# shanjiayao/PTT

Hardware: AMD Instinct MI355X
Metric: tracklet frames/sec (hot path: PointNet++ SA stack + Point-Track-Transformer blocks) (higher is better)
Workload: dtype f32

## Files before the change

include/ptt_hip.h:

```cpp
#ifndef PTT_HIP_H
#define PTT_HIP_H

#include <stddef.h>
#include <stdint.h>

#ifdef __cplusplus
extern "C" {
#endif

#define PTT_ABI_VERSION 30

enum {
    PTT_OK = 0,
    PTT_EINVAL = -1,
    PTT_EUNSUPPORTED = -2,
    PTT_ELAUNCH = -3,
    PTT_EWORKSPACE = -4
};

typedef void* ptt_stream_t;

int ptt_version(void);
const char* ptt_error_name(int code);
const char* ptt_last_error_string(void);

int ptt_fps_f32(const float* xyz, int B, int N, int npoint, int32_t* idx_out,
                ptt_stream_t stream);
int ptt_fps_ws_f32(const float* xyz, int B, int N, int npoint, int32_t* idx_out, float* workspace,
                   size_t workspace_elems, ptt_stream_t stream);

int ptt_ffps_f32(const float* xyz, const float* feat, int64_t feat_sb, int64_t feat_sc, int64_t feat_sn,
                 int B, int N, int C, int npoint, int32_t* idx_out, ptt_stream_t stream);

int ptt_gather_f32(const float* feat, const int32_t* idx, int B, int C, int N, int M,
                   float* out, ptt_stream_t stream);
int ptt_gather_grad_f32(const float* grad_out, const int32_t* idx, int B, int C, int N,
                        int M, float* grad_feat, ptt_stream_t stream);

int ptt_select_centres_f32(const float* xyz, const int32_t* idx, int B, int N, int M, float* new_xyz,
                           int64_t* idx64_out, ptt_stream_t stream);

int ptt_ball_query_f32(const float* new_xyz, const float* xyz, int B, int M, int N,
                       float radius, int nsample, int32_t* idx_out, ptt_stream_t stream);

int ptt_centres_ball_query_f32(const float* xyz, const int32_t* sel, int B, int N, int M, float radius, int nsample,
                               float* new_xyz, int64_t* idx64_out, int32_t* idx_out, ptt_stream_t stream);

int ptt_group_f32(const float* feat, const int32_t* idx, int B, int C, int N, int M,
                  int ns, float* out, ptt_stream_t stream);
int ptt_group_grad_f32(const float* grad_out, const int32_t* idx, int B, int C, int N,
                       int M, int ns, float* grad_feat, ptt_stream_t stream);

size_t ptt_scatter_add_det_workspace(int B, int N, int E);
int ptt_scatter_add_det_f32(const float* src, const int32_t* idx, int B, int C, int N, int E, float* out,
                            void* workspace, size_t workspace_bytes, ptt_stream_t stream);

int ptt_knn_f32(const float* xyz, int B, int N, int k, int32_t* idx_out,
                ptt_stream_t stream);
int ptt_knn_rel_f32(const float* xyz, int B, int N, int k, int32_t* idx_out, float* rel_out,
                    ptt_stream_t stream);

size_t ptt_packed_weight_elems(int Cout, int K);
int ptt_pack_weight_f32(const float* W, int Cout, int K, float* packed,
                        ptt_stream_t stream);
int ptt_pack_weight_rot_f32(const float* W, int Cout, int K, int rot, float* packed,
                            ptt_stream_t stream);

int ptt_linear_f32(const float* X, int rows, int K, int ldx, const float* Wpacked, int Cout,
                   const float* scale, const float* shift, int relu, const float* residual,
                   int ldr, float* out, int ldo, ptt_stream_t stream);

#define PTT_SA_MAX_LAYERS 4

typedef struct ptt_sa_layer {
    const float* Wpacked;
    const float* scale;
    const float* shift;
    int Cin;
    int Cout;
    int relu;
} ptt_sa_layer;

int ptt_rows_mlp_f32(const float* X, int rows, int K, int ldx, const ptt_sa_layer* layers, int n_layers,
                     const float* residual, int ldr, float* out, int ldo, ptt_stream_t stream);

size_t ptt_ball_query_grid_workspace(int B, int N);
int ptt_ball_query_grid_f32(const float* new_xyz, const float* xyz, int B, int M, int N, float radius, int nsample,
                            int32_t* idx_out, void* workspace, size_t workspace_bytes, ptt_stream_t stream);
int ptt_centres_ball_query_grid_f32(const float* xyz, const int32_t* sel, int B, int N, int M, float radius, int nsample,
                                    float* new_xyz, int64_t* idx64_out, int32_t* idx_out, void* workspace, size_t workspace_bytes,
                                    ptt_stream_t stream);
int ptt_fps_ball_knn_f32(const float* xyz, int B, int N, int M, float radius, int nsample, int k, int32_t* inds,
                         int64_t* inds64, float* new_xyz, int32_t* idx, int32_t* knn, float* rel, ptt_stream_t stream);
#define PTT_POINT_JOBS_MAX 4
typedef struct ptt_point_job {
    const float* xyz; const int32_t* centre_sel; const int32_t* point_sel;
    float* new_xyz; int64_t* idx64_out; int32_t* idx_out; float* rel_out;
    int32_t kind, sel_ld, B, Nraw, Npts, M, nsample;
    float radius;
} ptt_point_job;
int ptt_point_jobs_f32(const ptt_point_job* jobs, int n_jobs, ptt_stream_t stream);

#define PTT_ROW_JOBS_MAX 4
typedef struct ptt_row_job {
    const float* X; const float* X2;
    const float* Xmax;
    const float* Wpacked; const float* scale; const float* shift;
    const float* res; const float* res2;
    float* out; float* out2; float* raw;
    const float* rel; const float* w1;
    const float* qkv; const int32_t* knn; const float* pos;
    int32_t rows, K, K1, ldx, ldx2, Cout;
    int32_t act, res_split, ldr, ldr2, out_split, out_col0, ldo, ldo2, ldraw;
    int32_t prologue, epilogue, ldq, q_off, k_off, v_off, ldp, N;
    float sm_scale;
    int32_t col_tiles;
    const int32_t* idx; const float* xyz; const float* centres; const float* wx;
    float radius;
    int32_t ns, M, normalize_xyz, pro_relu;
} ptt_row_job;
int ptt_row_jobs_f32(const ptt_row_job* jobs, int n_jobs, ptt_stream_t stream);

typedef struct ptt_sa_desc {
    const float* xyz;
    const float* new_xyz;
    const int32_t* idx;
    const float* feat;
    int64_t feat_sb, feat_sc, feat_sn;
    float* out;
    int64_t out_sb, out_sc, out_sm;
    int B, N, M, nsample, C;
    float radius;
    int use_xyz;
    int normalize_xyz;
    int n_layers;
    ptt_sa_layer layers[PTT_SA_MAX_LAYERS];
    const float* l0_point_term;
    const float* l0_xyz_weight;
    int l0_channels;
    int l0_relu;
    void* compact_ws;
    size_t compact_ws_bytes;
} ptt_sa_desc;

int ptt_sa_fused_fwd_f32(const ptt_sa_desc* d, ptt_stream_t stream);
size_t ptt_sa_compact_workspace(int B, int M);

typedef struct ptt_xcorr_desc {
    const float* cos_t;
    const float* P;
    const float* w_sim;
    const float* scale0;
    const float* shift0;
    float* out;
    int64_t out_sb, out_sc, out_sn;
    float* sim_out;
    int B, Ns, Nt, C0;
    int n_layers;
    ptt_sa_layer layers[PTT_SA_MAX_LAYERS];
    int32_t split; int64_t out_sh;
    const float* search_feat; const float* templ_feat;
    int64_t s_sb, s_sn, t_sb, t_sn;
    int C; float eps;
} ptt_xcorr_desc;

int ptt_xcorr_fused_fwd_f32(const ptt_xcorr_desc* d, ptt_stream_t stream);

int ptt_cosine_map_f32(const float* search_feat, int64_t s_sb, int64_t s_sn, int64_t s_sc, const float* templ_feat,
                       int64_t t_sb, int64_t t_sn, int64_t t_sc, int B, int Ns, int Nt, int C, float eps,
                       float* cos_t, ptt_stream_t stream);

typedef struct ptt_attn_desc {
    const float* xyz;
    const float* rel;
    const int32_t* knn;
    const float* qkv;
    const float* Wd1p;
    const float* Wd2p;
    const float* bd2;
    const float* Wg1p;
    const float* bg1;
    const float* Wg2p;
    const float* bg2;
    float* res;
    float* attn;
    int B, N, k, D;
    const int32_t* order;
    int heads;
} ptt_attn_desc;

int ptt_pt_attn_pair_f32(const ptt_attn_desc* d, ptt_stream_t stream);
int ptt_spatial_order_f32(const float* xyz, int B, int N, int32_t* order, ptt_stream_t stream);

typedef struct ptt_crop_job {
    const float* points;
    int64_t ld;
    double lo1[3], hi1[3];
    double trans[3];
    double rot[9];
    double lo2[3], hi2[3];
    float* out;
    int32_t* count;
    int32_t n_points;
    int32_t capacity;
    uint8_t* label_out;
    double ltrans[3];
    double lrot[9];
    double llo[3], lhi[3];
    int32_t append;
    int32_t reserved;
} ptt_crop_job;

int ptt_crop_compact_f32(const ptt_crop_job* jobs_device, int n_jobs, ptt_stream_t stream);
#define PTT_CROP_JOBS_BY_VALUE_MAX 8
int ptt_crop_compact_host_f32(const ptt_crop_job* jobs_host, int n_jobs, ptt_stream_t stream);

#define PTT_SCAN_CROP_CHUNK 1024
size_t ptt_crop_scan_workspace(int n_jobs, int max_points);
int ptt_crop_scan_f32(const ptt_crop_job* jobs_device, int n_jobs, int max_points, void* ws, size_t ws_bytes, ptt_stream_t stream);

#define PTT_MAX_SEGMENTS 4
typedef struct ptt_regularize_job {
    const float* seg[PTT_MAX_SEGMENTS];
    const int32_t* seg_count[PTT_MAX_SEGMENTS];
    int32_t seg_capacity[PTT_MAX_SEGMENTS];
    float* out;
    int32_t* info;
    int32_t n_seg;
    int32_t input_size;
} ptt_regularize_job;

int ptt_regularize_f32(const ptt_regularize_job* jobs_device, int n_jobs, const uint32_t* draws, int n_draws,
                       ptt_stream_t stream);
int ptt_crop_regularize_f32(const ptt_crop_job* crop_jobs, const ptt_regularize_job* reg_jobs_device, int n_jobs,
                            const uint32_t* draws, int n_draws, ptt_stream_t stream);

int ptt_mt19937_fill(uint32_t seed, uint32_t* out_host, int n);

typedef struct ptt_track_box {
    double center[3];
    double wlh[3];
    double quat[4];
} ptt_track_box;

int ptt_track_crop_bounds(const ptt_track_box* boxes, int n, double offset, double scale, const double* extra2,
                          ptt_crop_job* jobs_host, int job_stride);
int ptt_track_box_by_offset(ptt_track_box* boxes, int n, float* offsets, int offset_stride, int use_z,
                            const int32_t* active, int64_t* rng_pos);
int ptt_track_select_update(const float* proposals_host, int P, const int32_t* info_host, ptt_track_box* boxes, int n, int use_z,
                            const int32_t* active, int64_t* rng_pos, float* est_out);

int ptt_select_box_f32(const float* pred_box_data, int B, int P, float* out, int32_t* idx_out, ptt_stream_t stream);

#define PTT_REF_CAMERA 0
#define PTT_REF_LIDAR 1
int ptt_box_overlap_f64(const double* gt, const double* pred, int n, int ref_coord, int dims, double* overlap, double* accuracy,
                        ptt_stream_t stream);

#define PTT_TRAIN_MAX_CANDS 1024
typedef struct ptt_train_cand {
    const float* search;
    const uint8_t* label;
    const float* first;
    const float* prev;
    const int32_t* counts;
    float reg[4];
    uint32_t index;
    uint32_t epoch;
    int32_t capacity;
    int32_t reserved;
} ptt_train_cand;

typedef struct ptt_train_batch_desc {
    float* search_points;
    float* template_points;
    float* cls_label;
    float* reg_label;
    int32_t* src_out;
    int32_t* idx_search_out;
    int32_t* idx_template_out;
    int32_t* info;
    int64_t* totals;
    int32_t B, n_cand;
    int32_t search_size, template_size;
    int32_t min_points;
    uint32_t seed_lo, seed_hi;
    int32_t reserved;
} ptt_train_batch_desc;

int ptt_train_batch_f32(const ptt_train_cand* cands_device, const ptt_train_batch_desc* desc_host, ptt_stream_t stream);
int ptt_philox4x32_10(const uint32_t* counter4, const uint32_t* key2, uint32_t* out4);

size_t ptt_bn_stats_workspace(int R, int C);
int ptt_bn_stats_f32(const float* X, int R, int C, int ldx, float eps, float* mean, float* var, float* invstd,
                     void* workspace, size_t workspace_bytes, ptt_stream_t stream);
int ptt_bn_apply_f32(const float* Z, int ldz, const float* mean, const float* invstd, const float* gamma,
                     const float* beta, int R, int C, int relu, float* X, int ldx, ptt_stream_t stream);
int ptt_bn_bwd_f32(const float* G, int ldg, const float* Act, int lda, const float* Z, int ldz, const float* mean,
                   const float* invstd, const float* gamma, int R, int C, int relu, float* dZ, int ldd,
                   float* dgamma, float* dbeta, void* workspace, size_t workspace_bytes, const float* act_scale,
                   const float* act_shift, ptt_stream_t stream);
int ptt_bn_sums_f64(const float* X, int R, int C, int ldx, double* sums, void* workspace, size_t workspace_bytes,
                    ptt_stream_t stream);
int ptt_bn_finish_f64(const double* sums, int C, float eps, float* mean, float* var, float* invstd,
                      ptt_stream_t stream);
int ptt_bn_bwd_sums_f64(const float* G, int ldg, const float* Act, int lda, const float* Z, int ldz, const float* mean,
                        const float* invstd, int R, int C, double* sums, void* workspace, size_t workspace_bytes,
                        const float* act_scale, const float* act_shift, ptt_stream_t stream);
int ptt_bn_bwd_apply_f32(const float* G, int ldg, const float* Act, int lda, const float* Z, int ldz, const float* mean,
                         const float* invstd, const float* gamma, const float* sum_dy, const float* sum_dy_xhat,
                         const double* count, int R, int C, float* dZ, int ldd, const float* act_scale, const float* act_shift,
                         ptt_stream_t stream);
int ptt_pool_rows_f32(const float* X, int ldx, int G, int ns, int C, float* out, int ldo, int32_t* arg,
                      const float* act_scale, const float* act_shift, ptt_stream_t stream);
int ptt_pool_rows_bwd_f32(const float* dOut, int ldo, const int32_t* arg, int G, int ns, int C, float* dX, int ldx,
                          ptt_stream_t stream);
int ptt_pt_pair_input_f32(const float* q, const float* kf, const int32_t* knn, const float* pos, int B, int N, int k, int D,
                          float* t, ptt_stream_t stream);
int ptt_pt_attn_train_fwd_f32(const float* a, const float* vf, const int32_t* knn, const float* pos, int B, int N, int k, int D,
                              float scale, float* attn, float* res, ptt_stream_t stream);
int ptt_pt_attn_train_bwd_f32(const float* attn, const float* vf, const int32_t* knn, const float* pos, const float* dres, int B,
                              int N, int k, int D, float scale, float* da, float* dvp, ptt_stream_t stream);

int ptt_pt_pair_input_ld_f32(const float* q, int ldq, const float* kf, int ldk, const int32_t* knn, const float* pos, int B, int N,
                             int k, int D, float* t, ptt_stream_t stream);
int ptt_pt_attn_fwd_ld_f32(const float* a, const float* vf, int ldv, const int32_t* knn, const float* pos, int B, int N, int k, int D,
                           float scale, float* attn, float* res, ptt_stream_t stream);

int ptt_gather_rows_f32(const float* src, const int32_t* idx, int B, int N, int E, int C, float* out, ptt_stream_t stream);
int ptt_scatter_csr_i32(const int32_t* idx, int B, int N, int E, int32_t* order, int32_t* start, ptt_stream_t stream);
int ptt_scatter_rows_csr_f32(const float* g, const int32_t* order, const int32_t* start, int B, int N, int E, int C,
                             float* out, ptt_stream_t stream);
int ptt_rows_gemm_pool_supported(int rows, int K, int N, int ldx, int ns);
int ptt_rows_gemm_pool_f32(const float* X, int rows, int K, int ldx, const float* in_scale, const float* in_shift,
                           const float* Wpacked, int N, float* out, int ldo, double* stats, size_t stats_elems, int ns,
                           float* pmax, float* pmin, int32_t* amax, int32_t* amin, ptt_stream_t stream);
int ptt_pool_select_f32(const float* pmax, const float* pmin, const int32_t* amax, const int32_t* amin, const float* act_scale,
                        const float* act_shift, int G, int C, float* out, int32_t* arg, ptt_stream_t stream);
size_t ptt_colsum_workspace(int R, int C);
int ptt_colsum_f32(const float* X, int R, int C, int ldx, float* out, void* workspace, size_t workspace_bytes, ptt_stream_t stream);
size_t ptt_linear_wgrad_workspace(int R, int Cout, int Cin);
int ptt_linear_wgrad_f32(const float* dZ, int ldz, const float* X, int ldx, int R, int Cout, int Cin, float* dW,
                         int accumulate, void* workspace, size_t workspace_bytes, const float* x_scale, const float* x_shift,
                         ptt_stream_t stream);
int ptt_linear_act_in_f32(const float* X, int rows, int K, int ldx, const float* in_scale, const float* in_shift,
                          const float* Wpacked, int Cout, float* out, int ldo, ptt_stream_t stream);

int ptt_pack_weight_strided_f32(const float* W, int Cout, int K, int64_t stride_out, int64_t stride_k, int batch,
                                int64_t stride_batch, float* packed, ptt_stream_t stream);
int ptt_linear_batched_f32(const float* X, int rows, int K, int ldx, int64_t x_batch_stride, const float* Wpacked,
                           int64_t w_batch_stride, int Cout, const float* scale, const float* shift, int relu,
                           const float* residual, int ldr, int64_t r_batch_stride, float* out, int ldo,
                           int64_t o_batch_stride, int batch, ptt_stream_t stream);
int ptt_softmax_rows_f32(float* X, int64_t rows, int n, int ld, float scale, ptt_stream_t stream);
int ptt_layernorm_f32(const float* x, int rows, int C, int ldx, const float* weight, const float* bias, float eps,
                      const float* residual, int ldr, float* out, int ldo, ptt_stream_t stream);

int ptt_rows_gemm_supported(int rows, int K, int N, int ldx, int ldo);
int ptt_rows_gemm_stat_chunks(int rows, int K, int N);
int ptt_rows_gemm_f32(const float* X, int rows, int K, int ldx, const float* in_scale, const float* in_shift,
                      const float* Wpacked, int N, const float* bias, int relu, const float* residual, int ldr,
                      float* out, int ldo, double* stats, size_t stats_elems, ptt_stream_t stream);
int ptt_rows_gemm_masked_f32(const float* X, int rows, int K, int ldx, const float* Wpacked, int N, const float* mask, int ldm,
                             float* out, int ldo, double* stats, size_t stats_elems, ptt_stream_t stream);
int ptt_rows_gemm_bnbwd_f32(const float* X, int rows, int K, int ldx, const float* Wpacked, int N, const float* Z, int ldz,
                            const float* mean, const float* invstd, const float* act_scale, const float* act_shift, float* out,
                            int ldo, double* sums_partial, size_t partial_elems, ptt_stream_t stream);
int ptt_bn_bwd_from_partials_f32(const double* partial, int chunks, const float* G, int ldg, const float* Z, int ldz, const float* mean,
                                 const float* invstd, const float* gamma, int R, int C, float* dZ, int ldd, float* dgamma, float* dbeta,
                                 const float* act_scale, const float* act_shift, ptt_stream_t stream);
int ptt_bn_bwd_sums_partials_f64(const double* partial, int chunks, int C, double* sums, ptt_stream_t stream);
typedef struct ptt_bn_bwd_input {
    const float* g; int ldg;
    const int32_t* arg; int ns;
    const float* z; int ldz;
    const float* k1; const float* c0; const float* c1; const float* mean;
    const float* act_a; const float* act_b;
    float* dz_out; int ldd;
} ptt_bn_bwd_input;
int ptt_bn_bwd_consts_f32(const double* partial, int chunks, const float* mean, const float* invstd, const float* gamma, int R, int C,
                          float* dgamma, float* dbeta, float* k1, float* c0, float* c1, ptt_stream_t stream);
int ptt_bn_bwd_pooled_consts_f32(const float* dPooled, int ldp, const int32_t* arg, int ns, const float* Z, int ldz, const float* mean,
                                 const float* invstd, const float* gamma, int R, int C, float* dgamma, float* dbeta, float* k1,
                                 float* c0, float* c1, void* workspace, size_t workspace_bytes, const float* act_scale,
                                 const float* act_shift, ptt_stream_t stream);
int ptt_rows_gemm_bnbwd_fused_supported(int rows, int K, int N, int ns);
int ptt_rows_gemm_bnbwd_fused_f32(const ptt_bn_bwd_input* in, int rows, int K, const float* Wpacked, int N, const float* Z, int ldz,
                                  const float* mean, const float* invstd, const float* act_scale, const float* act_shift, float* out,
                                  int ldo, double* sums_partial, size_t partial_elems, ptt_stream_t stream);
int ptt_bn_finish_partials_f32(const double* partial, int chunks, int C, int R, float eps, float* mean, float* var, float* invstd,
                               ptt_stream_t stream);
int ptt_bn_sums_partials_f64(const double* partial, int chunks, int C, int R, double* sums, ptt_stream_t stream);
int ptt_bn_bwd_pooled_f32(const float* dPooled, int ldp, const int32_t* arg, int ns, const float* Z, int ldz, const float* mean,
                          const float* invstd, const float* gamma, int R, int C, float* dZ, int ldd, float* dgamma, float* dbeta,
                          void* workspace, size_t workspace_bytes, const float* act_scale, const float* act_shift, ptt_stream_t stream);
int ptt_bn_bwd_pooled_sums_f64(const float* dPooled, int ldp, const int32_t* arg, int ns, const float* Z, int ldz, const float* mean,
                               const float* invstd, int R, int C, double* sums, void* workspace, size_t workspace_bytes,
                               const float* act_scale, const float* act_shift, ptt_stream_t stream);
int ptt_bn_bwd_pooled_apply_f32(const float* dPooled, int ldp, const int32_t* arg, int ns, const float* Z, int ldz, const float* mean,
                                const float* invstd, const float* gamma, const float* sum_dy, const float* sum_dy_xhat,
                                const double* count, int R, int C, float* dZ, int ldd, const float* act_scale,
                                const float* act_shift, ptt_stream_t stream);
int ptt_bn_update_running_f32(const float* mean, const float* var, const double* count, float momentum, int C, float* running_mean,
                              float* running_var, int64_t* num_batches_tracked, ptt_stream_t stream);
int ptt_xcorr_z0_f32(const float* P, const float* cos_t, const float* w_sim, int B, int n2, int n1, int C, float* z0, ptt_stream_t stream);
int ptt_xcorr_z0_stat_chunks(int B, int n2, int n1, int C);
int ptt_xcorr_z0_stats_f32(const float* P, const float* cos_t, const float* w_sim, int B, int n2, int n1, int C, float* z0,
                           double* stats_partial, size_t partial_elems, ptt_stream_t stream);
size_t ptt_xcorr_z0_bwd_workspace(int B, int n1, int C);
int ptt_xcorr_z0_bnbwd_f32(const double* partial, int chunks, const float* G, const float* P, const float* cos_t, const float* w_sim,
                           const float* mean, const float* invstd, const float* gamma, const float* act_scale, const float* act_shift,
                           int B, int n2, int n1, int C, float* dP, float* dcos, float* dw, float* dgamma, float* dbeta, void* workspace,
                           size_t workspace_bytes, ptt_stream_t stream);
int ptt_xcorr_z0_bwd_f32(const float* dz0, const float* cos_t, const float* w_sim, int B, int n2, int n1, int C, float* dP, float* dcos,
                         float* dw, void* workspace, size_t workspace_bytes, ptt_stream_t stream);
int ptt_sa_z0_rows_f32(const float* xyz, const float* new_xyz, const int32_t* idx, const float* term, const float* wx, int ldw, int B,
                       int N, int M, int ns, int C, float radius, int normalize_xyz, float* z0, float* rel_rows, ptt_stream_t stream);
int ptt_sa_z0_rows_stat_chunks(int B, int M, int ns, int C);
int ptt_sa_z0_rows_stats_f32(const float* xyz, const float* new_xyz, const int32_t* idx, const float* term, const float* wx, int ldw, int B,
                             int N, int M, int ns, int C, float radius, int normalize_xyz, float* z0, float* rel_rows,
                             double* stats_partial, size_t partial_elems, ptt_stream_t stream);
typedef struct ptt_bn_train_tail {
    const float* gamma; const float* beta;
    float* act_a; float* act_b;
    float* running_mean; float* running_var;
    int64_t* num_batches_tracked;
    float momentum;
} ptt_bn_train_tail;
int ptt_bn_stats_train_f32(const float* X, int R, int C, int ldx, float eps, float* mean, float* var, float* invstd,
                           void* workspace, size_t workspace_bytes, const ptt_bn_train_tail* tail, ptt_stream_t stream);
int ptt_bn_finish_partials_train_f32(const double* partial, int chunks, int C, int R, float eps, float* mean, float* var,
                                     float* invstd, const ptt_bn_train_tail* tail, ptt_stream_t stream);
typedef struct ptt_pack_job {
    const float* W;
    int64_t out_offset, stride_out, stride_k;
    int32_t Cout, K;
} ptt_pack_job;
int ptt_pack_weights_f32(const ptt_pack_job* jobs_device, int n_jobs, float* arena, ptt_stream_t stream);
size_t ptt_linear_wgrad2_workspace(int R, int Cout, int Cin);
int ptt_linear_wgrad2_f32(const float* dZ, int ldz, const float* X, int ldx, int R, int Cout, int Cin, float* dW,
                          int accumulate, void* workspace, size_t workspace_bytes, const float* x_scale, const float* x_shift,
                          ptt_stream_t stream);

typedef struct ptt_track_loss_desc {
    const float* seed_cls;
// ... 81 lines not shown
```

ptt_amd/_lib.py:

```python
import ctypes
import os
import re
from ctypes import Structure, c_char_p, c_double, c_float, c_int, c_int32, c_int64, c_longlong, c_size_t, c_uint32, c_void_p

from .build import HEADER as HEADER_PATH, LIB as LIB_PATH


def _strip_comments(text):
    return re.sub(r"/\*.*?\*/|//[^\n]*", " ", text, flags=re.S)


def parse_defines(text):
    return {n: int(v) for n, v in re.findall(r"^[ \t]*#[ \t]*define[ \t]+(PTT_\w+)[ \t]+(-?\d+)[ \t]*$", _strip_comments(text), re.M)}


CTYPES = {"int": c_int, "int32_t": c_int32, "uint32_t": c_uint32, "int64_t": c_int64, "long long": c_longlong, "size_t": c_size_t,
          "float": c_float, "double": c_double, "ptt_stream_t": c_void_p}


def _ctype(decl, name, is_return=False):
    words = decl.replace("*", " * ").split()
    if not is_return and len(words) > 1 and words[-1] != "*":
        words.pop()
    if "*" in words:
        if not is_return:
            return c_void_p
        if words == ["const", "char", "*"]:
            return c_char_p
    base = " ".join(w for w in words if w != "const")
    if base not in CTYPES:
        raise RuntimeError("ptt_amd: %s of %s in include/ptt_hip.h has the type '%s', which ptt_amd/_lib.py does not map to ctypes"
                           % ("the return value" if is_return else "parameter '%s'" % decl.strip(), name, base))
    return CTYPES[base]


def parse_prototypes(text):
    text = re.sub(r"^[ \t]*#.*$", " ", _strip_comments(text), flags=re.M).replace('extern "C" {', " ")
    text = re.sub(r"\{[^{}]*\}", " ", text)
    protos = {}
    for stmt in text.split(";"):
        stmt = " ".join(stmt.split()).lstrip("} ")
        if not stmt or stmt.split()[0] in ("typedef", "enum", "struct"):
            continue
        m = re.fullmatch(r"(.+?)\b(\w+) ?\((.*)\)", stmt)
        if m is None:
            raise RuntimeError("ptt_amd: cannot read '%s' in include/ptt_hip.h as a function prototype" % stmt)
        ret, name, params = m.groups()
        params = [] if params.strip() == "void" else params.split(",")
        protos[name] = (_ctype(ret, name, is_return=True), [_ctype(p, name) for p in params])
    return protos


def _read_header():
    if not os.path.exists(HEADER_PATH):
        raise RuntimeError("ptt_amd: %s is missing — the Python binding takes every prototype and constant of the C ABI from it" % HEADER_PATH)
    with open(HEADER_PATH) as fh:
        return fh.read()


_header = _read_header()
PROTOTYPES = parse_prototypes(_header)
EXPORTS = list(PROTOTYPES)
DEFINES = parse_defines(_header)
ABI_VERSION = DEFINES["PTT_ABI_VERSION"]
PTT_SA_MAX_LAYERS = DEFINES["PTT_SA_MAX_LAYERS"]
PTT_MAX_SEGMENTS = DEFINES["PTT_MAX_SEGMENTS"]
PTT_CROP_JOBS_BY_VALUE_MAX = DEFINES["PTT_CROP_JOBS_BY_VALUE_MAX"]
PTT_TRAIN_MAX_CANDS = DEFINES["PTT_TRAIN_MAX_CANDS"]


class CropJob(Structure):
    _fields_ = [("points", c_void_p), ("ld", c_int64),
                ("lo1", c_double * 3), ("hi1", c_double * 3), ("trans", c_double * 3), ("rot", c_double * 9),
                ("lo2", c_double * 3), ("hi2", c_double * 3),
                ("out", c_void_p), ("count", c_void_p), ("n_points", c_int32), ("capacity", c_int32),
                ("label_out", c_void_p), ("ltrans", c_double * 3), ("lrot", c_double * 9), ("llo", c_double * 3), ("lhi", c_double * 3),
                ("append", c_int32), ("reserved", c_int32)]


class RegularizeJob(Structure):
    _fields_ = [("seg", c_void_p * PTT_MAX_SEGMENTS), ("seg_count", c_void_p * PTT_MAX_SEGMENTS),
                ("seg_capacity", c_int32 * PTT_MAX_SEGMENTS), ("out", c_void_p), ("info", c_void_p),
                ("n_seg", c_int32), ("input_size", c_int32)]


class TrackBox(Structure):
    _fields_ = [("center", c_double * 3), ("wlh", c_double * 3), ("quat", c_double * 4)]


class TrainCand(Structure):
    _fields_ = [("search", c_void_p), ("label", c_void_p), ("first", c_void_p), ("prev", c_void_p), ("counts", c_void_p),
                ("reg", c_float * 4), ("index", c_uint32), ("epoch", c_uint32), ("capacity", c_int32), ("reserved", c_int32)]


class TrainBatchDesc(Structure):
    _fields_ = [("search_points", c_void_p), ("template_points", c_void_p), ("cls_label", c_void_p), ("reg_label", c_void_p),
                ("src_out", c_void_p), ("idx_search_out", c_void_p), ("idx_template_out", c_void_p), ("info", c_void_p), ("totals", c_void_p),
                ("B", c_int32), ("n_cand", c_int32), ("search_size", c_int32), ("template_size", c_int32), ("min_points", c_int32),
                ("seed_lo", c_uint32), ("seed_hi", c_uint32), ("reserved", c_int32)]


class BnTrainTail(Structure):
    _fields_ = [("gamma", c_void_p), ("beta", c_void_p), ("act_a", c_void_p), ("act_b", c_void_p),
                ("running_mean", c_void_p), ("running_var", c_void_p), ("num_batches_tracked", c_void_p), ("momentum", c_float)]


class BnBwdInput(Structure):
    _fields_ = [("g", c_void_p), ("ldg", c_int), ("arg", c_void_p), ("ns", c_int), ("z", c_void_p), ("ldz", c_int),
                ("k1", c_void_p), ("c0", c_void_p), ("c1", c_void_p), ("mean", c_void_p), ("act_a", c_void_p), ("act_b", c_void_p),
                ("dz_out", c_void_p), ("ldd", c_int)]


class PackJob(Structure):
    _fields_ = [("W", c_void_p), ("out_offset", c_int64), ("stride_out", c_int64), ("stride_k", c_int64),
                ("Cout", c_int32), ("K", c_int32)]


class RowJob(Structure):
    _fields_ = [("X", c_void_p), ("X2", c_void_p), ("Xmax", c_void_p), ("Wpacked", c_void_p), ("scale", c_void_p), ("shift", c_void_p),
                ("res", c_void_p), ("res2", c_void_p), ("out", c_void_p), ("out2", c_void_p), ("raw", c_void_p),
                ("rel", c_void_p), ("w1", c_void_p), ("qkv", c_void_p), ("knn", c_void_p), ("pos", c_void_p),
                ("rows", c_int32), ("K", c_int32), ("K1", c_int32), ("ldx", c_int32), ("ldx2", c_int32), ("Cout", c_int32),
                ("act", c_int32), ("res_split", c_int32), ("ldr", c_int32), ("ldr2", c_int32), ("out_split", c_int32),
                ("out_col0", c_int32), ("ldo", c_int32), ("ldo2", c_int32), ("ldraw", c_int32),
                ("prologue", c_int32), ("epilogue", c_int32), ("ldq", c_int32), ("q_off", c_int32), ("k_off", c_int32),
                ("v_off", c_int32), ("ldp", c_int32), ("N", c_int32), ("sm_scale", c_float), ("col_tiles", c_int32),
                ("idx", c_void_p), ("xyz", c_void_p), ("centres", c_void_p), ("wx", c_void_p), ("radius", c_float),
                ("ns", c_int32), ("M", c_int32), ("normalize_xyz", c_int32), ("pro_relu", c_int32)]


class PointJob(Structure):
    _fields_ = [("xyz", c_void_p), ("centre_sel", c_void_p), ("point_sel", c_void_p), ("new_xyz", c_void_p), ("idx64_out", c_void_p),
                ("idx_out", c_void_p), ("rel_out", c_void_p), ("kind", c_int32), ("sel_ld", c_int32), ("B", c_int32),
                ("Nraw", c_int32), ("Npts", c_int32), ("M", c_int32), ("nsample", c_int32), ("radius", c_float)]


class TrackLossDesc(Structure):
    _fields_ = [("seed_cls", c_void_p), ("cls_label", c_void_p), ("search_inds", c_void_p), ("votes", c_void_p), ("reg_label", c_void_p),
                ("box_data", c_void_p), ("centres", c_void_p), ("pos_weight_seed", c_void_p), ("pos_weight_box", c_void_p),
                ("B", c_int32), ("N", c_int32), ("Ns", c_int32), ("M", c_int32), ("ld_reg", c_int32),
                ("w_seed_cls", c_float), ("w_seed_reg", c_float), ("w_box_cls", c_float), ("w_box_reg", c_float)]


class AdamTensor(Structure):
    _fields_ = [("param", c_void_p), ("grad", c_void_p), ("exp_avg", c_void_p), ("exp_avg_sq", c_void_p), ("n", c_int64)]


class GradJob(Structure):
    _fields_ = [("partial", c_void_p), ("nchunks", c_int32), ("reserved", c_int32)]


class GradSegment(Structure):
    _fields_ = [("dst", c_int64), ("n", c_int32), ("cols", c_int32), ("ld", c_int32), ("job0", c_int32), ("njobs", c_int32), ("out", c_int32),
                ("vec", c_int32), ("reserved", c_int32)]


class AdamHyper(Structure):
    _fields_ = [("beta1", c_float), ("beta2", c_float), ("one_minus_beta1", c_float), ("one_minus_beta2", c_float), ("eps", c_float), ("step_size", c_float), ("bias2_sqrt", c_float),
                ("weight_decay", c_float), ("max_norm", c_float), ("write_clipped", c_int32)]


class SaLayer(Structure):
    _fields_ = [("Wpacked", c_void_p), ("scale", c_void_p), ("shift", c_void_p),
                ("Cin", c_int), ("Cout", c_int), ("relu", c_int)]


class SaDesc(Structure):
    _fields_ = [("xyz", c_void_p), ("new_xyz", c_void_p), ("idx", c_void_p), ("feat", c_void_p),
                ("feat_sb", c_int64), ("feat_sc", c_int64), ("feat_sn", c_int64),
                ("out", c_void_p), ("out_sb", c_int64), ("out_sc", c_int64), ("out_sm", c_int64),
                ("B", c_int), ("N", c_int), ("M", c_int), ("nsample", c_int), ("C", c_int),
                ("radius", c_float), ("use_xyz", c_int), ("normalize_xyz", c_int), ("n_layers", c_int),
                ("layers", SaLayer * PTT_SA_MAX_LAYERS),
                ("l0_point_term", c_void_p), ("l0_xyz_weight", c_void_p), ("l0_channels", c_int), ("l0_relu", c_int),
                ("compact_ws", c_void_p), ("compact_ws_bytes", c_size_t)]


class XcorrDesc(Structure):
    _fields_ = [("cos_t", c_void_p), ("P", c_void_p), ("w_sim", c_void_p), ("scale0", c_void_p), ("shift0", c_void_p),
                ("out", c_void_p), ("out_sb", c_int64), ("out_sc", c_int64), ("out_sn", c_int64),
                ("sim_out", c_void_p),
                ("B", c_int), ("Ns", c_int), ("Nt", c_int), ("C0", c_int),
                ("n_layers", c_int), ("layers", SaLayer * PTT_SA_MAX_LAYERS),
                ("split", c_int32), ("out_sh", c_int64), ("search_feat", c_void_p), ("templ_feat", c_void_p),
                ("s_sb", c_int64), ("s_sn", c_int64), ("t_sb", c_int64), ("t_sn", c_int64), ("C", c_int), ("eps", c_float)]


class AttnDesc(Structure):
    _fields_ = [("xyz", c_void_p), ("rel", c_void_p), ("knn", c_void_p), ("qkv", c_void_p),
                ("Wd1p", c_void_p), ("Wd2p", c_void_p), ("bd2", c_void_p),
                ("Wg1p", c_void_p), ("bg1", c_void_p), ("Wg2p", c_void_p), ("bg2", c_void_p),
                ("res", c_void_p), ("attn", c_void_p),
                ("B", c_int), ("N", c_int), ("k", c_int), ("D", c_int), ("order", c_void_p), ("heads", c_int)]


_lib = None


def lib():
    global _lib
    if _lib is None:
        if not os.path.exists(LIB_PATH):
            raise RuntimeError(
                "ptt_amd: %s is missing — build it with `python -m ptt_amd.build` "
                "(hipcc --offload-arch=gfx950); there is no CPU fallback" % LIB_PATH)
        import torch
        try:
            loaded = ctypes.CDLL(LIB_PATH)
        except OSError as e:
            raise RuntimeError("ptt_amd: cannot load %s: %s" % (LIB_PATH, e))
        for name, (restype, argtypes) in PROTOTYPES.items():
            fn = getattr(loaded, name)
            fn.restype, fn.argtypes = restype, argtypes
        if loaded.ptt_version() != ABI_VERSION:
            raise RuntimeError("ptt_amd: %s has ABI version %d, this package expects %d — rebuild it with "
                               "`python -m ptt_amd.build`" % (LIB_PATH, loaded.ptt_version(), ABI_VERSION))
        _lib = loaded
    return _lib


def check(rc, what):
    if rc != 0:
        l = lib()
        raise RuntimeError("%s failed: %s (%s)" % (what, l.ptt_error_name(rc).decode(),
                                                   l.ptt_last_error_string().decode()))
```

ptt_amd/csrc/mfma_ops.hip:

```cpp
#include <math.h>
#include <stdlib.h>
#include <string.h>
#include "common.h"
#include "mfma_common.h"

#ifndef PTT_PAIR_PF
#define PTT_PAIR_PF 1
#endif
#ifndef PTT_GATHER_BATCH
#define PTT_GATHER_BATCH 16
#endif
#ifndef PTT_SA_WAVES
#define PTT_SA_WAVES 2
#endif

namespace ptt {

#ifdef PTT_DEV
#define PTT_STAMP(i) do { if (p.dbg && threadIdx.x == 0 && blockIdx.x < 4096) p.dbg[blockIdx.x * 8 + (i)] = __builtin_readcyclecounter(); } while (0)
#else
#define PTT_STAMP(i) do { } while (0)
#endif

__device__ __forceinline__ void stagger_second_slot(int first_wave_blocks, int quanta) {
// ... 950 lines not shown
        if (it > 0) store_pooled(prev);
        if (!(PTT_SAS_EXP & 1)) lds_barrier();

        {
            const float* arow = Q + (lane & 31) * SAS_LDK + 4 * half;
            f32x4 a0[2], a1[2], bc[2][2], bn[2][2];
#define SAS_A2(A, KB)                                                                           \
            {                                                                                   \
                A[0] = *reinterpret_cast<const f32x4*>(arow + (KB) * 8);                        \
                A[1] = *reinterpret_cast<const f32x4*>(arow + 32 * SAS_LDK + (KB) * 8);         \
            }
#pragma unroll
            for (int k = 0; k < 2; ++k) { bc[k][0] = pre2[k][0]; bc[k][1] = pre2[k][1]; }
            SAS_A2(a0, 0)
            f32x4 mc = *reinterpret_cast<const f32x4*>(meta + (w * 16 + sub) * 4), mn = mc;
#pragma unroll
            for (int i = 0; i < 8; ++i) {
                if (i < 7) {
#pragma unroll
                    for (int k = 0; k < 2; ++k) {
                        bn[k][0] = weight_load(wr2, wvoff, (2 * i + 2 + k) * WK2);
                        bn[k][1] = weight_load(wr2, wvoff, (2 * i + 2 + k) * WK2 + 4 * 1024);
                    }
                } else {
                    pre1[0] = weight_load(wr1, wvoff, 0);
                    pre1[1] = weight_load(wr1, wvoff, WK1);
                }
                SAS_A2(a1, 2 * i + 1)
                f32x4 v = wx0;
                if (!(PTT_SAS_EXP & 2)) v = weight_load(rf, __builtin_bit_cast(int, mc[0]) + q * 16, 0);
                __builtin_amdgcn_sched_barrier(0);
                if (i == 0) {
#pragma unroll
                    for (int u = 0; u < 2; ++u)
#pragma unroll
                        for (int rt = 0; rt < 2; ++rt)
                            acc[rt][u] = __builtin_amdgcn_mfma_f32_32x32x2f32(a0[rt][0], bc[0][u][0], zero16, 0, 0, 0);
#pragma unroll
                    for (int j = 1; j < 4; ++j)
#pragma unroll
                        for (int u = 0; u < 2; ++u)
#pragma unroll
                            for (int rt = 0; rt < 2; ++rt)
                                acc[rt][u] = __builtin_amdgcn_mfma_f32_32x32x2f32(a0[rt][j], bc[0][u][j], acc[rt][u], 0, 0, 0);
                } else {
                    gemm_mfma_block<2, 2, 2>(a0, bc[0], acc);
                }
                __builtin_amdgcn_sched_barrier(0);
                if (i < 7) {
                    SAS_A2(a0, 2 * i + 2)
                    mn = *reinterpret_cast<const f32x4*>(meta + (w * 16 + 2 * (i + 1) + sub) * 4);
                }
                __builtin_amdgcn_sched_barrier(0);
                gemm_mfma_block<2, 2, 2>(a1, bc[1], acc);
                if (!(PTT_SAS_EXP & 2)) sas_pair_store(P, w, i, sub, q, v, mc, wx0, wx1, wx2, floor0);
#if PTT_SAS_INTERLEAVE
#pragma unroll
                for (int k = 0; k < 16; ++k) {
                    __builtin_amdgcn_sched_group_barrier(0x008, 1, 0);
                    __builtin_amdgcn_sched_group_barrier(0x002, 1, 0);
                }
                __builtin_amdgcn_sched_group_barrier(0x200, 1, 0);
#endif
                __builtin_amdgcn_sched_barrier(0);
                mc = mn;
#pragma unroll
                for (int k = 0; k < 2; ++k) { bc[k][0] = bn[k][0]; bc[k][1] = bn[k][1]; }
            }
#undef SAS_A2
        }
        prev = first;
        if (more) { first.advance(2, M); own = own_next; }
    }
#pragma unroll
    for (int i = 0; i < 4; ++i) pv[i >> 1][i & 1] = sas_pool(acc[i >> 1][i & 1], (i & 1) ? sh2b : sh2a, L2.relu);
    store_pooled(prev);
}

struct XcorrParams {
    const float* P; const float* wsim; const float* scale0; const float* shift0;
    float* sim_out;
    const float* cos_t;
    int C0, Nt;
    SaParams sa;
    const float* sfeat; const float* tfeat; long long s_sb, s_sn, t_sb, t_sn; int C; float eps;
    long long out_sh;
};

struct CosParams {
    const float* sfeat; const float* tfeat; float* cos_t;
    long long s_sb, s_sn, s_sc, t_sb, t_sn, t_sc;
    int B, Ns, Nt, C;
    float eps;
};
__global__ __launch_bounds__(256) void cos_map_kernel(CosParams q) {
    const int lane = threadIdx.x & 63;
    const int j = blockIdx.x * 4 + (threadIdx.x >> 6);
    if (j >= q.B * q.Ns) return;
    const int b = j / q.Ns, jj = j - b * q.Ns;
    const float* s = q.sfeat + (long long)b * q.s_sb + (long long)jj * q.s_sn;
    for (int i0 = 0; i0 < q.Nt; i0 += 64) {
        const int i = i0 + lane;
        const float* a = q.tfeat + (long long)b * q.t_sb + (long long)(i < q.Nt ? i : q.Nt - 1) * q.t_sn;
        float dot = 0.f, na = 0.f, ns = 0.f;
        if (q.t_sc == 1 && q.s_sc == 1 && (q.C & 3) == 0 && ((q.t_sn | q.t_sb | q.s_sn | q.s_sb) & 3) == 0 &&
            ((reinterpret_cast<uintptr_t>(q.tfeat) | reinterpret_cast<uintptr_t>(q.sfeat)) & 15) == 0) {
            for (int c = 0; c < q.C; c += 4) {
                const f32x4 av = *reinterpret_cast<const f32x4*>(a + c), sv = *reinterpret_cast<const f32x4*>(s + c);
#pragma unroll
                for (int k = 0; k < 4; ++k) { dot += av[k] * sv[k]; na += av[k] * av[k]; ns += sv[k] * sv[k]; }
            }
        } else {
            for (int c = 0; c < q.C; ++c) {
                const float av = a[(long long)c * q.t_sc], sv = s[(long long)c * q.s_sc];
                dot += av * sv; na += av * av; ns += sv * sv;
            }
        }
        if (i < q.Nt) q.cos_t[((long long)b * q.Ns + jj) * q.Nt + i] = dot / (fmaxf(sqrtf(na), q.eps) * fmaxf(sqrtf(ns), q.eps));
    }
}

template <int RT, bool SPLIT>
__global__ __launch_bounds__(256, 2) void xcorr_fused_kernel(XcorrParams q) {
    constexpr int ROWS = 32 * RT;
    extern __shared__ __attribute__((aligned(16))) float smem[];
    const SaParams& p = q.sa;
    float* Xs = smem;
    float* simv = smem + ROWS * p.ldk;
    const int t = threadIdx.x, lane = t & 63, w = t >> 6, half = lane >> 5;
    const int npts = p.B * p.M;
    const int j = SPLIT ? (int)blockIdx.x % npts : logical_block();
    const int hsel = SPLIT ? (int)blockIdx.x / npts : 0;
    const int b = j / p.M, jj = j - b * p.M;
    stagger_second_slot(p.first_wave, p.stagger);
    SaPre pre;
    pre.w[0] = pre.w[1] = f32x4{0.f, 0.f, 0.f, 0.f};
    float run[2] = {-__builtin_inff(), -__builtin_inff()};
    const int nlast = p.n_layers - 1;
    const SaLayerDev& LL = p.L[nlast];

    const int ibeg = SPLIT ? hsel * (q.Nt >> 1) : 0, iend = SPLIT ? ibeg + (q.Nt >> 1) : q.Nt;
    for (int i0 = ibeg; i0 < iend; i0 += ROWS) {
        prefetch_first_block(p.L[0].Wp, p.L[0].scale, p.L[0].shift, p.L[0].NT, w, lane, pre);
        if (i0 != ibeg) __syncthreads();
        if constexpr (SPLIT) {
            const int i = t >> 3, sub = t & 7;
            const float* a = q.tfeat + (long long)b * q.t_sb + (long long)(i0 + i) * q.t_sn;
            const float* sv_ = q.sfeat + (long long)b * q.s_sb + (long long)jj * q.s_sn;
            float dot = 0.f, na = 0.f, ns = 0.f;
            for (int c = sub * 4; c < q.C; c += 32) {
                const f32x4 av = *reinterpret_cast<const f32x4*>(a + c), sv = *reinterpret_cast<const f32x4*>(sv_ + c);
#pragma unroll
                for (int k = 0; k < 4; ++k) { dot += av[k] * sv[k]; na += av[k] * av[k]; ns += sv[k] * sv[k]; }
            }
#pragma unroll
            for (int m = 1; m < 8; m <<= 1) { dot += __shfl_xor(dot, m, 64); na += __shfl_xor(na, m, 64); ns += __shfl_xor(ns, m, 64); }
            if (sub == 0) simv[i] = dot / (fmaxf(sqrtf(na), q.eps) * fmaxf(sqrtf(ns), q.eps));
        } else {
            if (t < ROWS) {
                const float cs = q.cos_t[(unsigned)((b * p.M + jj) * q.Nt + i0 + t)];
                simv[t] = cs;
                if (q.sim_out) q.sim_out[(unsigned)((b * q.Nt + i0 + t) * p.M + jj)] = cs;
            }
        }
        __syncthreads();

        const int nq = q.C0 >> 2;
        if (!q.scale0 && !q.shift0 && (q.C0 & 3) == 0 && (256 % nq) == 0) {
            typedef float f32x2 __attribute__((ext_vector_type(2)));
            const int c4 = t % nq, step = 256 / nq;
            const f32x4 w4 = *reinterpret_cast<const f32x4*>(q.wsim + c4 * 4);
            const float* prow = q.P + ((size_t)(b * q.Nt + i0) * q.C0 + c4 * 4);
            for (int i = t / nq; i < ROWS; i += step) {
                const f32x4 pv = *reinterpret_cast<const f32x4*>(prow + (unsigned)(i * q.C0));
                const float cs = simv[i];
                const f32x2 c2 = {cs, cs};
                f32x2 lo = __builtin_elementwise_fma(f32x2{w4[0], w4[1]}, c2, f32x2{pv[0], pv[1]});
                f32x2 hi = __builtin_elementwise_fma(f32x2{w4[2], w4[3]}, c2, f32x2{pv[2], pv[3]});
                *reinterpret_cast<f32x4*>(Xs + i * p.ldk + c4 * 4) =
                    f32x4{fmaxf(lo[0], 0.f), fmaxf(lo[1], 0.f), fmaxf(hi[0], 0.f), fmaxf(hi[1], 0.f)};
            }
        } else {
            for (int c = t; c < q.C0; c += 256) {
                const float wsim = q.wsim[c], sc = q.scale0 ? q.scale0[c] : 1.f, sh = q.shift0 ? q.shift0[c] : 0.f;
                const float* pr = q.P + ((long long)b * q.Nt + i0) * q.C0 + c;
#pragma unroll 8
                for (int i = 0; i < ROWS; ++i) {
                    const float v = (pr[(long long)i * q.C0] + wsim * simv[i]) * sc + sh;
                    Xs[i * p.ldk + c] = fmaxf(v, 0.f);
                }
            }
        }
        __syncthreads();

        for (int l = 0; l < nlast; ++l) {
            const SaLayerDev& L = p.L[l];
            const int ctw = (L.NT + 3) >> 2;
            if (ctw <= 1) sa_layer<32 * RT, 1, RT>(p, L, false, Xs, lane, w, j, 1, pre, &p.L[l + 1]);
            else sa_layer<32 * RT, 2, RT>(p, L, false, Xs, lane, w, j, 1, pre, &p.L[l + 1]);
        }
        {
            const bool affine = LL.scale != nullptr;
            f32x16 acc[RT][2];
#pragma unroll
            for (int rt = 0; rt < RT; ++rt)
#pragma unroll
                for (int u = 0; u < 2; ++u)
#pragma unroll
                    for (int r = 0; r < 16; ++r) acc[rt][u][r] = pre.sh[u];
            int nvalid = 0;
#pragma unroll
            for (int u = 0; u < 2; ++u)
                if (w + 4 * u < LL.NT) nvalid = u + 1;
            gemm_tiles<RT, 2, 0>(Xs, p.ldk, LL.nkb, reinterpret_cast<const f32x4*>(LL.Wp), LL.NT, w, nvalid, lane, acc, pre.w);
#pragma unroll
            for (int u = 0; u < 2; ++u) {
                if (u >= nvalid) break;
                const int col = (w + 4 * u) * 32 + (lane & 31);
                float sc = 1.f, sh = 0.f;
                if (affine) { sc = LL.scale[col]; sh = LL.shift ? LL.shift[col] : 0.f; }
#pragma unroll
                for (int rt = 0; rt < RT; ++rt) {
                    float m = affine ? acc[rt][u][0] * sc + sh : acc[rt][u][0];
#pragma unroll
                    for (int r = 1; r < 16; ++r) m = fmaxf(m, affine ? acc[rt][u][r] * sc + sh : acc[rt][u][r]);
                    run[u] = fmaxf(run[u], max_halves(m));
                }
            }
        }
    }
    if (half == 0) {
#pragma unroll
        for (int u = 0; u < 2; ++u) {
            if (w + 4 * u >= LL.NT) break;
            const int col = (w + 4 * u) * 32 + (lane & 31);
            p.out[(SPLIT ? hsel * q.out_sh : 0) + b * p.osb + col * p.osc + jj * p.osm] = LL.relu ? fmaxf(run[u], 0.f) : run[u];
        }
    }
}

template <int NS, int CT, bool AFFINE, int RT>
__device__ __forceinline__ void sa_wave_layer(const SaParams& p, const SaLayerDev& L, bool last, float* Xw, int lane,
                                              int centre0, int ncentres) {
    f32x16 acc[RT][CT];
#pragma unroll
    for (int u = 0; u < CT; ++u) {
        const float s0 = (!AFFINE && L.shift) ? L.shift[u * 32 + (lane & 31)] : 0.f;
#pragma unroll
        for (int rt = 0; rt < RT; ++rt)
#pragma unroll
            for (int r = 0; r < 16; ++r) acc[rt][u][r] = s0;
    }
    gemm_core<RT, CT, CT, 1>(Xw, p.ldk, L.nkb, reinterpret_cast<const f32x4*>(L.Wp), L.NT, 0, lane, acc);
    __builtin_amdgcn_wave_barrier();
    const int half = lane >> 5;
#pragma unroll
    for (int u = 0; u < CT; ++u) {
        const int col = u * 32 + (lane & 31);
        float sc = 1.f, sv = 0.f;
        if constexpr (AFFINE) { sc = L.scale[col]; sv = L.shift ? L.shift[col] : 0.f; }
#pragma unroll
        for (int rt = 0; rt < RT; ++rt) {
            float y[16];
#pragma unroll
            for (int r = 0; r < 16; ++r) y[r] = AFFINE ? acc[rt][u][r] * sc + sv : acc[rt][u][r];
            if (!last) {
#pragma unroll
                for (int r = 0; r < 16; ++r)
                    Xw[(rt * 32 + tile_row(r, half)) * p.ldk + col] = L.relu ? fmaxf(y[r], 0.f) : y[r];
            } else if (NS == 32) {
                float m = y[0];
#pragma unroll
                for (int r = 1; r < 16; ++r) m = fmaxf(m, y[r]);
                m = max_halves(m);
                if (L.relu) m = fmaxf(m, 0.f);
                if (half == 0 && rt < ncentres) {
                    const int c = centre0 + rt; const int b = c / p.M, mm = c - b * p.M;
                    p.out[b * p.osb + col * p.osc + mm * p.osm] = m;
                }
            } else {
                float m0 = y[0], m1 = y[8];
#pragma unroll
                for (int r = 1; r < 8; ++r) { m0 = fmaxf(m0, y[r]); m1 = fmaxf(m1, y[8 + r]); }
                m0 = max_halves(m0);
                m1 = max_halves(m1);
                if (L.relu) { m0 = fmaxf(m0, 0.f); m1 = fmaxf(m1, 0.f); }
                if (half == 0) {
                    if (2 * rt < ncentres) {
                        const int c = centre0 + 2 * rt; const int b = c / p.M, mm = c - b * p.M;
                        p.out[b * p.osb + col * p.osc + mm * p.osm] = m0;
                    }
                    if (2 * rt + 1 < ncentres) {
                        const int c = centre0 + 2 * rt + 1; const int b = c / p.M, mm = c - b * p.M;
                        p.out[b * p.osb + col * p.osc + mm * p.osm] = m1;
                    }
                }
            }
        }
    }
    __builtin_amdgcn_wave_barrier();
}

constexpr int SAC_HDR = 16;
struct SacTable {
    int32_t* ws; int T;
    __host__ __device__ int32_t* ndist() const { return ws + SAC_HDR; }
    __host__ __device__ int32_t* list(int k) const { return ws + SAC_HDR + (size_t)(1 + k) * T; }
    __host__ __device__ int32_t* rows(int k) const { return ws + SAC_HDR + 5 * (size_t)T + (size_t)((4 << k) - 4) * T; }
    static size_t words(size_t T) { return SAC_HDR + 65 * T; }
};
constexpr int SAC_PASSES = 4;

__global__ __launch_bounds__(64) void sa_compact_zero_kernel(int32_t* ws) {
    if (threadIdx.x < 4) ws[threadIdx.x] = 0;
}

template <bool XYZ>
__global__ __launch_bounds__(256) void sa_compact_kernel(const float* __restrict__ xyz, const int32_t* __restrict__ idx, int N, int M,
                                                         SacTable tab) {
    __shared__ int s_cnt[4], s_base[4], s_cls[32], s_pos[32], s_nd[32];
    __shared__ int s_row[32][32];
    const int t = threadIdx.x, lane = t & 63, half = lane >> 5, s = lane & 31, w = t >> 6;
    const int g0 = blockIdx.x * 32, T = tab.T;
    if (t < 4) s_cnt[t] = 0;
    __syncthreads();
    int iv[SAC_PASSES];
    uint32_t x[SAC_PASSES], y[SAC_PASSES], z[SAC_PASSES];
#pragma unroll
    for (int q = 0; q < SAC_PASSES; ++q) iv[q] = idx[(size_t)min(g0 + q * 8 + w * 2 + half, T - 1) * 32 + s];
    if constexpr (XYZ) {
#pragma unroll
        for (int q = 0; q < SAC_PASSES; ++q) {
            const int b = min(g0 + q * 8 + w * 2 + half, T - 1) / M;
            const uint32_t* pt = reinterpret_cast<const uint32_t*>(xyz) + ((size_t)b * N + iv[q]) * 3;
            x[q] = pt[0]; y[q] = pt[1]; z[q] = pt[2];
        }
    }
#pragma unroll
    for (int q = 0; q < SAC_PASSES; ++q) {
        const int lc = q * 8 + w * 2 + half;
        const int i0a = __builtin_amdgcn_readlane(iv[q], 0), i0b = __builtin_amdgcn_readlane(iv[q], 32);
        const int i0 = half ? i0b : i0a;
        const bool real = s == 0 || iv[q] != i0;
        int dup = 0;
        if constexpr (XYZ) {
            const unsigned long long rm = __ballot(real);
            const int J = 31 - __builtin_clz((uint32_t)rm | (uint32_t)(rm >> 32));
            for (int j = 0; j < J; ++j) {
                const uint32_t xa = __builtin_amdgcn_readlane(x[q], j), xb = __builtin_amdgcn_readlane(x[q], 32 + j);
                const uint32_t ya = __builtin_amdgcn_readlane(y[q], j), yb = __builtin_amdgcn_readlane(y[q], 32 + j);
                const uint32_t za = __builtin_amdgcn_readlane(z[q], j), zb = __builtin_amdgcn_readlane(z[q], 32 + j);
                dup |= (int)(j < s) & (int)(x[q] == (half ? xb : xa)) & (int)(y[q] == (half ? yb : ya)) & (int)(z[q] == (half ? zb : za));
            }
        }
        const bool keep = real && !dup;
        const unsigned long long km = __ballot(keep);
        const uint32_t m = half ? (uint32_t)(km >> 32) : (uint32_t)km;
        const int nd = __popc(m);
        if (keep) s_row[lc][__popc(m & ((1u << s) - 1u))] = iv[q];
        if (s == 0) {
            const int k = nd <= 4 ? 0 : nd <= 8 ? 1 : nd <= 16 ? 2 : 3;
            const bool valid = g0 + lc < T;
            s_cls[lc] = valid ? k : -1;
            s_nd[lc] = nd;
            s_pos[lc] = valid ? atomicAdd(&s_cnt[k], 1) : 0;
            if (valid) tab.ndist()[g0 + lc] = nd;
        }
    }
    __syncthreads();
    if (t < 4) s_base[t] = s_cnt[t] ? atomicAdd(&tab.ws[t], s_cnt[t]) : 0;
    __syncthreads();
    for (int e = t; e < 32 * 32; e += 256) {
        const int lc = e >> 5, j = e & 31, k = s_cls[lc];
        if (k < 0 || j >= (4 << k)) continue;
        const int q = s_base[k] + s_pos[lc];
        tab.rows(k)[(size_t)q * (4 << k) + j] = s_row[lc][j < s_nd[lc] ? j : 0];
        if (j == 0) tab.list(k)[q] = g0 + lc;
    }
}

#ifndef PTT_SAL_WGS
#define PTT_SAL_WGS 1
#endif
#ifndef PTT_SAL_WAVES
#define PTT_SAL_WAVES 12
#endif

template <int ROWS>
struct SacTileT {
    static constexpr int LG = ROWS == 32 ? 3 : 4;
    static_assert(ROWS == 32 || ROWS == 64, "32- or 64-row tiles");
    int k, first, n;
    __device__ __forceinline__ static void count(const int32_t* ws, int total, int (&cnt)[4], int (&tiles)[4]) {
#pragma unroll
        for (int k = 0; k < 4; ++k) {
            cnt[k] = min(max(ws[k], 0), total);
            tiles[k] = (k ? tiles[k - 1] : 0) + ((cnt[k] + ((1 << LG) >> k) - 1) >> (LG - k));
        }
    }
    __device__ __forceinline__ void at(int j, const int (&tiles)[4], const int (&cnt)[4]) {
        k = j < tiles[0] ? 0 : j < tiles[1] ? 1 : j < tiles[2] ? 2 : 3;
        const int j0 = k == 0 ? 0 : k == 1 ? tiles[0] : k == 2 ? tiles[1] : tiles[2];
        const int nk = k == 0 ? cnt[0] : k == 1 ? cnt[1] : k == 2 ? cnt[2] : cnt[3];
        first = (j - j0) << (LG - k);
        n = min((1 << LG) >> k, nk - first);
    }
    __device__ __forceinline__ void row(const SacTable& tab, int s, int& n_out, int& ball) const {
        const int cl = s >> (2 + k), inb = cl < n;
        n_out = tab.rows(k)[(size_t)first * (4 << k) + (inb ? s : (s & ((4 << k) - 1)))];
        ball = tab.list(k)[first + (inb ? cl : 0)];
    }
};
using SacTile = SacTileT<32>;

template <int NU>
__device__ __forceinline__ void sac_store(int k, int n, int ball, int M, const f32x16 (&acc)[NU], const float (&sh)[NU],
                                          float* const (&o)[NU], int relu, int half, int osb, int osm) {
    int ob[8];
#pragma unroll
    for (int g = 0; g < 8; ++g) {
        if (g >= (8 >> k)) break;
        const int id = __builtin_amdgcn_readlane(ball, g << (2 + k)), b = id / M;
        ob[g] = b * osb + (id - b * M) * osm;
    }
#pragma unroll
    for (int u = 0; u < NU; ++u) {
        const f32x16& a = acc[u];
        if (k == 3) {
            const float mx = sas_pool(a, sh[u], relu);
            if (half == 0) o[u][ob[0]] = mx;
        } else if (k == 2) {
            float m0 = a[0], m1 = a[8];
#pragma unroll
            for (int r = 1; r < 8; ++r) { m0 = fmaxf(m0, a[r]); m1 = fmaxf(m1, a[8 + r]); }
            m0 = max_halves(m0) + sh[u]; m1 = max_halves(m1) + sh[u];
            if (relu) { m0 = fmaxf(m0, 0.f); m1 = fmaxf(m1, 0.f); }
            if (half < n) o[u][half ? ob[1] : ob[0]] = half ? m1 : m0;
        } else {
            float m[4];
#pragma unroll
            for (int q = 0; q < 4; ++q) m[q] = fmaxf(fmaxf(a[4 * q], a[4 * q + 1]), fmaxf(a[4 * q + 2], a[4 * q + 3]));
            if (k == 1) {
#pragma unroll
                for (int q = 0; q < 4; ++q) m[q] = max_halves(m[q]) + sh[u];
#pragma unroll
                for (int i = 0; i < 2; ++i) {
                    const int g = 2 * half + i;
                    float v = half ? m[2 + i] : m[i];
                    if (relu) v = fmaxf(v, 0.f);
                    if (g < n) o[u][half ? ob[2 + i] : ob[i]] = v;
                }
            } else {
#pragma unroll
                for (int q = 0; q < 4; ++q) {
                    const int g = 2 * q + half;
                    float v = m[q] + sh[u];
                    if (relu) v = fmaxf(v, 0.f);
                    if (g < n) o[u][half ? ob[2 * q + 1] : ob[2 * q]] = v;
                }
            }
        }
    }
}

template <bool COMPACT>
__global__ __launch_bounds__(64 * PTT_SAL_WAVES) __attribute__((amdgpu_waves_per_eu(PTT_SAL_WAVES * PTT_SAL_WGS / 4)))
void sa_lds_kernel(SaParams p) {
    extern __shared__ __attribute__((aligned(16))) float smem[];
    float* W1 = smem;
    float* W2 = smem + 4096;
    const int t = threadIdx.x, lane = t & 63, half = lane >> 5, col = lane & 31;
    const int w = __builtin_amdgcn_readfirstlane(t >> 6);
    const int total = p.B * p.M, M = p.M, N = p.N;
    const int nw = (int)blockDim.x >> 6;
    SacTable tab{p.cws, total};
    int cnt[4], tiles[4];
    if constexpr (COMPACT) {
        SacTile::count(p.cws, total, cnt, tiles);
        if (logical_block() >= tiles[3]) return;
    }
    {
        const f32x4* g1 = reinterpret_cast<const f32x4*>(p.L[1].Wp);
        const f32x4* g2 = reinterpret_cast<const f32x4*>(p.L[2].Wp);
        f32x4* s1 = reinterpret_cast<f32x4*>(W1);
        f32x4* s2 = reinterpret_cast<f32x4*>(W2);
        const int nthr = (int)blockDim.x;
        for (int i = t; i < 1024; i += nthr) s1[i] = g1[i];
        for (int i = t; i < 2048; i += nthr) s2[i] = g2[i];
    }
    float* cst = smem + 4096 + 8192 + w * 640 + lane;
#pragma unroll
    for (int u = 0; u < 2; ++u) {
        const f32x4 f = reinterpret_cast<const f32x4*>(p.L[0].Wp)[u * 64 + col];
        const float s0 = p.L[0].shift ? p.L[0].shift[u * 32 + col] : 0.f;
        cst[(0 + u) * 64] = half ? f[1] : f[0];
        cst[(2 + u) * 64] = half ? s0 : f[2];
        cst[(4 + u) * 64] = p.L[1].shift ? p.L[1].shift[u * 32 + col] : 0.f;
    }
#pragma unroll
    for (int u = 0; u < 4; ++u) cst[(6 + u) * 64] = p.L[2].shift ? p.L[2].shift[u * 32 + col] : 0.f;
    const float one_zero = half ? 0.f : 1.f, one_hi = 1.f;
    __syncthreads();
    int c0, c1, cstep;
    if constexpr (COMPACT) {
        c0 = logical_block() + (int)gridDim.x * w; c1 = tiles[3]; cstep = (int)gridDim.x * nw;
    } else {
        const int gw = logical_block() * nw + w;
        c0 = gw * p.chunk; c1 = min(total, c0 + p.chunk); cstep = 1;
    }
    if (c0 >= c1) return;
    const float rdiv = p.normalize ? p.radius : 1.0f;
    const int osb = (int)p.osb, osm = (int)p.osm, osc = (int)p.osc;
    const f32x16 zero16 = {0.f, 0.f, 0.f, 0.f, 0.f, 0.f, 0.f, 0.f, 0.f, 0.f, 0.f, 0.f, 0.f, 0.f, 0.f, 0.f};
    const float* a1p = W1 + lane * 4;
    const float* b2p = W2 + lane * 4;
    const __amdgpu_buffer_rsrc_t rx = weight_rsrc(p.xyz);

    SasCentre ce{0, 0, 0};
    SacTile tc{0, 0, 0};
    float px, py, pz, cx, cy, cz;
    int g_cur = 0;
    if constexpr (COMPACT) {
        tc.at(c0, tiles, cnt);
        int n_cur;
        tc.row(tab, col, n_cur, g_cur);
        const size_t flat = (size_t)(g_cur / M) * N + n_cur;
        px = p.xyz[flat * 3]; py = p.xyz[flat * 3 + 1]; pz = p.xyz[flat * 3 + 2];
        cx = p.new_xyz[(size_t)g_cur * 3]; cy = p.new_xyz[(size_t)g_cur * 3 + 1]; cz = p.new_xyz[(size_t)g_cur * 3 + 2];
    } else {
        ce.c = c0; ce.b = c0 / M; ce.m = c0 - ce.b * M;
        const int n_cur = p.idx[(size_t)c0 * 32 + col];
        const size_t flat = (size_t)ce.b * N + n_cur;
        px = p.xyz[flat * 3]; py = p.xyz[flat * 3 + 1]; pz = p.xyz[flat * 3 + 2];
        cx = p.new_xyz[(size_t)c0 * 3]; cy = p.new_xyz[(size_t)c0 * 3 + 1]; cz = p.new_xyz[(size_t)c0 * 3 + 2];
    }
    for (int c = c0; c < c1; c += cstep) {
        SasCentre nx = ce;
        SacTile tx = tc;
        int n_next, g_next;
        if constexpr (COMPACT) {
            if (c + cstep < c1) tx.at(c + cstep, tiles, cnt);
            tx.row(tab, col, n_next, g_next);
        } else {
            if (c + 1 < c1) nx.advance(1, M);
            n_next = p.idx[(size_t)nx.c * 32 + col];
        }
        f32x4 wa[2], wn[2];
#pragma unroll
        for (int u = 0; u < 2; ++u) wa[u] = *reinterpret_cast<const f32x4*>(a1p + u * 256);
        const float dx = (px - cx) / rdiv, dy = (py - cy) / rdiv, dz = (pz - cz) / rdiv;
        __builtin_amdgcn_sched_barrier(0);
        f32x16 h0[2];
        {
            const float k0 = half ? dy : dx, k1 = half ? one_hi : dz;
#pragma unroll
            for (int u = 0; u < 2; ++u) h0[u] = __builtin_amdgcn_mfma_f32_32x32x2f32(cst[(0 + u) * 64], k0, zero16, 0, 0, 0);
#pragma unroll
            for (int u = 0; u < 2; ++u) h0[u] = __builtin_amdgcn_mfma_f32_32x32x2f32(cst[(2 + u) * 64], k1, h0[u], 0, 0, 0);
#pragma unroll
            for (int u = 0; u < 2; ++u)
#pragma unroll
                for (int r = 0; r < 16; ++r) h0[u][r] = fmaxf(h0[u][r], 0.f);
        }
        f32x16 h1[2];
        f32x4 wb[4], wm[4];
        {
#pragma unroll
            for (int u = 0; u < 2; ++u) h1[u] = __builtin_amdgcn_mfma_f32_32x32x2f32(cst[(4 + u) * 64], one_zero, zero16, 0, 0, 0);
#pragma unroll
            for (int kb = 0; kb < 8; ++kb) {
                if (kb < 7) {
#pragma unroll
                    for (int u = 0; u < 2; ++u) wn[u] = *reinterpret_cast<const f32x4*>(a1p + ((kb + 1) * 2 + u) * 256);
                } else {
#pragma unroll
                    for (int u = 0; u < 4; ++u) wb[u] = *reinterpret_cast<const f32x4*>(b2p + u * 256);
                }
                __builtin_amdgcn_sched_barrier(0);
#pragma unroll
                for (int j = 0; j < 4; ++j)
#pragma unroll
                    for (int u = 0; u < 2; ++u)
                        h1[u] = __builtin_amdgcn_mfma_f32_32x32x2f32(wa[u][j], h0[kb >> 2][(kb & 3) * 4 + j], h1[u], 0, 0, 0);
                __builtin_amdgcn_sched_barrier(0);
#pragma unroll
                for (int u = 0; u < 2; ++u) wa[u] = wn[u];
            }
#pragma unroll
            for (int u = 0; u < 2; ++u)
#pragma unroll
                for (int r = 0; r < 16; ++r) h1[u][r] = fmaxf(h1[u][r], 0.f);
        }
        {
            const int g = COMPACT ? g_next : nx.c;
            const int off = ((COMPACT ? g_next / M : nx.b) * N + n_next) * 12;
            px = __builtin_bit_cast(float, __builtin_amdgcn_raw_buffer_load_b32(rx, off, 0, 0));
            py = __builtin_bit_cast(float, __builtin_amdgcn_raw_buffer_load_b32(rx, off + 4, 0, 0));
            pz = __builtin_bit_cast(float, __builtin_amdgcn_raw_buffer_load_b32(rx, off + 8, 0, 0));
            cx = p.new_xyz[(size_t)g * 3]; cy = p.new_xyz[(size_t)g * 3 + 1]; cz = p.new_xyz[(size_t)g * 3 + 2];
        }
        __builtin_amdgcn_sched_barrier(0);
        {
            f32x16 acc[4];
#pragma unroll
            for (int kb = 0; kb < 8; ++kb) {
                if (kb < 7) {
#pragma unroll
                    for (int u = 0; u < 4; ++u) wm[u] = *reinterpret_cast<const f32x4*>(b2p + ((kb + 1) * 4 + u) * 256);
                }
                __builtin_amdgcn_sched_barrier(0);
#pragma unroll
                for (int j = 0; j < 4; ++j)
#pragma unroll
                    for (int u = 0; u < 4; ++u)
                        acc[u] = __builtin_amdgcn_mfma_f32_32x32x2f32(h1[kb >> 2][(kb & 3) * 4 + j], wb[u][j],
                                                                       (kb == 0 && j == 0) ? zero16 : acc[u], 0, 0, 0);
                __builtin_amdgcn_sched_barrier(0);
#pragma unroll
                for (int u = 0; u < 4; ++u) wb[u] = wm[u];
            }
            if constexpr (COMPACT) {
                const float sh2[4] = {cst[6 * 64], cst[7 * 64], cst[8 * 64], cst[9 * 64]};
                float* const o[4] = {p.out + col * osc, p.out + (32 + col) * osc, p.out + (64 + col) * osc, p.out + (96 + col) * osc};
                sac_store<4>(tc.k, tc.n, g_cur, M, acc, sh2, o, p.L[2].relu, half, osb, osm);
            } else {
                float* o = p.out + (ce.b * osb + ce.m * osm);
#pragma unroll
                for (int u = 0; u < 4; ++u) {
                    const float mx = sas_pool(acc[u], cst[(6 + u) * 64], p.L[2].relu);
                    if (half == 0) o[(u * 32 + col) * osc] = mx;
                }
            }
        }
        if constexpr (COMPACT) { tc = tx; g_cur = g_next; } else ce = nx;
    }
}

__global__ __launch_bounds__(256, 2) void sa_stream_compact_kernel(SaParams p) {
    extern __shared__ __attribute__((aligned(16))) float smem[];
    float* const P = smem;
    float* const Q = smem + SAS_TILE;
    float* const meta = smem + 2 * SAS_TILE;
    int* const sball = reinterpret_cast<int*>(meta + 64 * 4);
    const int t = threadIdx.x, lane = t & 63, half = lane >> 5, sub = half, q = lane & 31, col = q;
    const int w = __builtin_amdgcn_readfirstlane(t >> 6);
    const int total = p.B * p.M, M = p.M, N = p.N;
    const SacTable tab{p.cws, total};
    int cnt[4], tiles[4];
    SacTileT<64>::count(p.cws, total, cnt, tiles);
    if ((int)blockIdx.x >= tiles[3]) return;
    const SaLayerDev& L1 = p.L[0];
    const SaLayerDev& L2 = p.L[1];
    const __amdgpu_buffer_rsrc_t rf = weight_rsrc(p.feat);
    const __amdgpu_buffer_rsrc_t wr1 = weight_rsrc(L1.Wp), wr2 = weight_rsrc(L2.Wp);
    const int wvoff = (w * 64 + lane) * 16;
    constexpr int WK1 = 4 * 1024, WK2 = 8 * 1024;
    const f32x4 wx0 = *reinterpret_cast<const f32x4*>(p.wx + q * 4);
    const f32x4 wx1 = *reinterpret_cast<const f32x4*>(p.wx + 128 + q * 4);
    const f32x4 wx2 = *reinterpret_cast<const f32x4*>(p.wx + 256 + q * 4);
    const float sh1 = L1.shift ? L1.shift[w * 32 + col] : 0.f;
    const float sh2[2] = {L2.shift ? L2.shift[w * 32 + col] : 0.f, L2.shift ? L2.shift[(w + 4) * 32 + col] : 0.f};
    f32x16 sh1v;
#pragma unroll
    for (int r = 0; r < 16; ++r) sh1v[r] = sh1;
    const f32x16 zero16 = {0.f, 0.f, 0.f, 0.f, 0.f, 0.f, 0.f, 0.f, 0.f, 0.f, 0.f, 0.f, 0.f, 0.f, 0.f, 0.f};
    const float floor0 = p.l0_relu ? 0.f : -__builtin_inff();
    const float rdiv = p.normalize ? p.radius : 1.0f;
    const int osb = (int)p.osb, osm = (int)p.osm;
    float* const o[2] = {p.out + (w * 32 + col) * (int)p.osc, p.out + ((w + 4) * 32 + col) * (int)p.osc};

    for (int j = blockIdx.x; j < tiles[3]; j += (int)gridDim.x) {
        SacTileT<64> tc;
        tc.at(j, tiles, cnt);
        if (t < 64) {
            int n, ball;
            tc.row(tab, t, n, ball);
            const int flat = (ball / M) * N + n;
            const float x = p.xyz[(size_t)flat * 3 + 0], y = p.xyz[(size_t)flat * 3 + 1], z = p.xyz[(size_t)flat * 3 + 2];
            const float cx = p.new_xyz[(size_t)ball * 3 + 0], cy = p.new_xyz[(size_t)ball * 3 + 1], cz = p.new_xyz[(size_t)ball * 3 + 2];
            const float dx = (x - cx) / rdiv, dy = (y - cy) / rdiv, dz = (z - cz) / rdiv;
            const int off = flat * (128 * (int)sizeof(float));
            *reinterpret_cast<f32x4*>(meta + t * 4) = f32x4{__builtin_bit_cast(float, off), dx, dy, dz};
            sball[t] = ball;
        }
        __syncthreads();
#pragma unroll
        for (int i = 0; i < 8; ++i) {
            f32x4 m;
            const f32x4 v = sas_pair_load(meta, rf, w, i, sub, q, m);
            sas_pair_store(P, w, i, sub, q, v, m, wx0, wx1, wx2, floor0);
        }
        const int ballr[2] = {sball[col], sball[32 + col]};
        __syncthreads();
        {
            f32x16 acc1[2] = {sh1v, sh1v};
            const float* arow = P + (lane & 31) * SAS_LDK + 4 * half;
#pragma unroll
            for (int kb = 0; kb < 16; ++kb) {
                const f32x4 b = weight_load(wr1, wvoff, kb * WK1);
                const f32x4 a[2] = {*reinterpret_cast<const f32x4*>(arow + kb * 8),
                                    *reinterpret_cast<const f32x4*>(arow + 32 * SAS_LDK + kb * 8)};
#pragma unroll
                for (int jj = 0; jj < 4; ++jj)
#pragma unroll
                    for (int rt = 0; rt < 2; ++rt) acc1[rt] = __builtin_amdgcn_mfma_f32_32x32x2f32(a[rt][jj], b[jj], acc1[rt], 0, 0, 0);
            }
#pragma unroll
            for (int rt = 0; rt < 2; ++rt)
#pragma unroll
                for (int r = 0; r < 16; ++r) Q[(rt * 32 + tile_row(r, half)) * SAS_LDK + w * 32 + col] = fmaxf(acc1[rt][r], 0.f);
        }
        __syncthreads();
        {
            f32x16 acc[2][2] = {{zero16, zero16}, {zero16, zero16}};
            const float* arow = Q + (lane & 31) * SAS_LDK + 4 * half;
#pragma unroll
            for (int kb = 0; kb < 16; ++kb) {
                const f32x4 b[2] = {weight_load(wr2, wvoff, kb * WK2), weight_load(wr2, wvoff, kb * WK2 + 4 * 1024)};
                const f32x4 a[2] = {*reinterpret_cast<const f32x4*>(arow + kb * 8),
                                    *reinterpret_cast<const f32x4*>(arow + 32 * SAS_LDK + kb * 8)};
                gemm_mfma_block<2, 2, 2>(a, b, acc);
            }
#pragma unroll
            for (int rt = 0; rt < 2; ++rt) {
                const int n = tc.n - rt * (8 >> tc.k);
                if (n <= 0) continue;
                sac_store<2>(tc.k, n, ballr[rt], M, acc[rt], sh2, o, L2.relu, half, osb, osm);
            }
        }
    }
}

template <int NS, int RT>
__global__ __launch_bounds__(256, 2) void sa_wave_kernel(SaParams p) {
    extern __shared__ __attribute__((aligned(16))) float smem[];
    constexpr int CPW = 32 * RT / NS;
    const int t = threadIdx.x, lane = t & 63, w = t >> 6;
    float* Xw = smem + w * 32 * RT * p.ldk;
    const int total_centres = p.B * p.M;
    const int centre0 = (logical_block() * 4 + w) * CPW;
    if (centre0 >= total_centres) return;
    const int ncentres = min(CPW, total_centres - centre0);

#pragma unroll
    for (int rt = 0; rt < RT; ++rt) sa_gather_rows<NS, 32>(p, Xw, rt * 32, centre0, lane);
    __builtin_amdgcn_wave_barrier();

    for (int l = 0; l < p.n_layers; ++l) {
        const SaLayerDev& L = p.L[l];
        const bool last = (l == p.n_layers - 1);
#define PTT_WAVE_LAYER(CTV)                                                                         \
        { if (L.scale) sa_wave_layer<NS, CTV, true, RT>(p, L, last, Xw, lane, centre0, ncentres);       \
          else sa_wave_layer<NS, CTV, false, RT>(p, L, last, Xw, lane, centre0, ncentres); }
        if (L.NT == 1) PTT_WAVE_LAYER(1)
        else if (L.NT == 2) PTT_WAVE_LAYER(2)
        else PTT_WAVE_LAYER(4)
#undef PTT_WAVE_LAYER
    }
}

struct AttnParams {
    const float* xyz; const float* rel; const int32_t* knn; const float* qkv; const float* Wd1p;
    const float* Wd2p; const float* bd2; const float* Wg1p; const float* bg1; const float* Wg2p; const float* bg2;
    float* res; float* attn;
    const int32_t* order;
    int BN, N, first_wave, stagger;
    long long* dbg;
};

template <int D, int HEADS>
__device__ __forceinline__ void gemm_heads(const float* Xs, int ldk, const float* Wp, int w, int lane, f32x16 (&acc)[1][4],
                                           const f32x4 (&pre)[4]) {
    static_assert(D == 512 && (HEADS == 2 || HEADS == 4 || HEADS == 8 || HEADS == 16), "4 waves x 4 column tiles of D = 512");
    constexpr int HD = D / HEADS, TPH = HD / 32, NKB = HD / 8;
    constexpr int NA = HEADS == 2 ? 2 : 4;
    constexpr int NB = HEADS == 2 ? 2 : 1;
    const int row = lane & 31, half = lane >> 5;
    const float* arow[NA];
#pragma unroll
    for (int i = 0; i < NA; ++i) arow[i] = Xs + row * ldk + 4 * half + ((w + 4 * i * (4 / NA)) / TPH) * HD;
    const __amdgpu_buffer_rsrc_t wr = weight_rsrc(Wp);
    int wvoff[NB];
#pragma unroll
    for (int i = 0; i < NB; ++i) wvoff[i] = (((w + 4 * i) % TPH) * 64 + lane) * 16;
    constexpr int wkstep = TPH * 1024;
    f32x4 bcur[NB], bnxt[NB];
#pragma unroll
    for (int i = 0; i < NB; ++i) { bcur[i] = pre[i]; bnxt[i] = bcur[i]; }
    auto block = [&](int kb) {
        f32x4 a[NA];
#pragma unroll
        for (int i = 0; i < NA; ++i) a[i] = *reinterpret_cast<const f32x4*>(arow[i] + kb * 8);
#pragma unroll
        for (int j = 0; j < 4; ++j)
#pragma unroll
            for (int u = 0; u < 4; ++u)
                acc[0][u] = __builtin_amdgcn_mfma_f32_32x32x2f32(a[u / (4 / NA)][j], bcur[u % NB][j], acc[0][u], 0, 0, 0);
    };
    for (int kb = 0; kb + 1 < NKB; ++kb) {
#pragma unroll
        for (int i = 0; i < NB; ++i) bnxt[i] = weight_load(wr, wvoff[i], (kb + 1) * wkstep);
        block(kb);
#pragma unroll
        for (int i = 0; i < NB; ++i) bcur[i] = bnxt[i];
    }
    block(NKB - 1);
}

template <int D, int HEADS>
__device__ __forceinline__ void prefetch_first_block_heads(const float* Wp, int w, int lane, f32x4 (&pre)[4]) {
    constexpr int TPH = D / HEADS / 32, NB = HEADS == 2 ? 2 : 1;
    const f32x4* bp = reinterpret_cast<const f32x4*>(Wp) + lane;
#pragma unroll
    for (int i = 0; i < NB; ++i) pre[i] = bp[(size_t)((w + 4 * i) % TPH) * 64];
}

template <int D>
__global__ __launch_bounds__(256, 2) void pt_attn_pair_kernel(AttnParams p) {
    constexpr int HEADS = 1;
#include "pt_attn_pair_body.h"
}

template <int HEADS>
__global__ __launch_bounds__(256, 2) void pt_attn_pair_heads_kernel(AttnParams p) {
    constexpr int D = 512;
#include "pt_attn_pair_body.h"
}

__global__ __launch_bounds__(256) void softmax_rows_kernel(float* __restrict__ X, long long rows, int n, int ld, float scale) {
    const int lane = threadIdx.x & 63;
    const long long r = (long long)blockIdx.x * 4 + (threadIdx.x >> 6);
    if (r >= rows) return;
    float* x = X + r * ld;
    float m = -3.0e38f;
    for (int c = lane; c < n; c += 64) m = fmaxf(m, x[c] * scale);
    m = wave_max_f32(m);
    float sum = 0.f;
    for (int c = lane; c < n; c += 64) {
        const float e = __expf(x[c] * scale - m);
        x[c] = e;
        sum += e;
    }
#pragma unroll
    for (int o = 32; o > 0; o >>= 1) sum += __shfl_xor(sum, o, 64);
    const float inv = 1.0f / sum;
    for (int c = lane; c < n; c += 64) x[c] *= inv;
}

constexpr int LN_VPL = 16;
__global__ __launch_bounds__(256) void layernorm_rows_kernel(const float* __restrict__ X, int rows, int C, int ldx,
                                                             const float* __restrict__ weight, const float* __restrict__ bias,
                                                             float eps, const float* __restrict__ R, int ldr,
                                                             float* __restrict__ Y, int ldy) {
    const int lane = threadIdx.x & 63;
    const int r = blockIdx.x * 4 + (threadIdx.x >> 6);
    if (r >= rows) return;
    const float* x = X + (size_t)r * ldx;
    float v[LN_VPL];
    float sum = 0.f;
#pragma unroll
    for (int i = 0; i < LN_VPL; ++i) {
        const int c = lane + 64 * i;
        v[i] = c < C ? x[c] : 0.f;
        sum += v[i];
    }
#pragma unroll
    for (int o = 32; o > 0; o >>= 1) sum += __shfl_xor(sum, o, 64);
    const float mean = sum / (float)C;
    float sq = 0.f;
#pragma unroll
    for (int i = 0; i < LN_VPL; ++i) {
        const float d = (lane + 64 * i) < C ? v[i] - mean : 0.f;
        v[i] = d;
        sq += d * d;
    }
#pragma unroll
    for (int o = 32; o > 0; o >>= 1) sq += __shfl_xor(sq, o, 64);
    const float rstd = 1.0f / sqrtf(sq / (float)C + eps);
    float* y = Y + (size_t)r * ldy;
    const float* res = R ? R + (size_t)r * ldr : nullptr;
#pragma unroll
    for (int i = 0; i < LN_VPL; ++i) {
        const int c = lane + 64 * i;
        if (c < C) {
            float o = v[i] * rstd;
            if (weight) o *= weight[c];
            if (bias) o += bias[c];
            if (res) o += res[c];
            y[c] = o;
        }
    }
}

}

using namespace ptt;

extern "C" int ptt_layernorm_f32(const float* x, int rows, int C, int ldx, const float* weight, const float* bias, float eps,
                                 const float* residual, int ldr, float* out, int ldo, ptt_stream_t stream) {
    if (rows < 0 || C <= 0 || C > 64 * LN_VPL || ldx < C || ldo < C || (residual && ldr < C))
        return fail(PTT_EINVAL, "ptt_layernorm_f32: rows=%d C=%d ldx=%d ldr=%d ldo=%d (C <= %d)", rows, C, ldx, ldr, ldo, 64 * LN_VPL);
    if (rows == 0) return PTT_OK;
    if (!x || !out) return fail(PTT_EINVAL, "ptt_layernorm_f32: null pointer");
    hipLaunchKernelGGL(layernorm_rows_kernel, dim3((unsigned)((rows + 3) / 4)), dim3(256), 0, as_stream(stream), x, rows, C, ldx,
                       weight, bias, eps, residual, ldr, out, ldo);
    return check_launch("layernorm_rows_kernel");
}

extern "C" int ptt_softmax_rows_f32(float* X, int64_t rows, int n, int ld, float scale, ptt_stream_t stream) {
    if (rows < 0 || n <= 0 || ld < n) return fail(PTT_EINVAL, "ptt_softmax_rows_f32: rows=%lld n=%d ld=%d", (long long)rows, n, ld);
    if (rows == 0) return PTT_OK;
    if (!X) return fail(PTT_EINVAL, "ptt_softmax_rows_f32: null pointer");
    hipLaunchKernelGGL(softmax_rows_kernel, dim3((unsigned)((rows + 3) / 4)), dim3(256), 0, as_stream(stream), X, (long long)rows, n, ld,
                       scale);
    return check_launch("softmax_rows_kernel");
}

extern "C" size_t ptt_packed_weight_elems(int Cout, int K) {
    if (Cout <= 0 || K <= 0) return 0;
    const size_t NT = (size_t)(Cout + 31) / 32, NKB = (size_t)(K + 7) / 8;
    return NT * NKB * 256;
}

extern "C" int ptt_pack_weight_rot_f32(const float* W, int Cout, int K, int rot, float* packed, ptt_stream_t stream) {
    if (Cout <= 0 || K <= 0 || rot < 0 || rot >= K)
        return fail(PTT_EINVAL, "ptt_pack_weight_rot_f32: Cout=%d K=%d rot=%d", Cout, K, rot);
    if (!W || !packed) return fail(PTT_EINVAL, "ptt_pack_weight_rot_f32: null pointer");
    const size_t total = ptt_packed_weight_elems(Cout, K);
    const int NT = (Cout + 31) / 32;
    size_t g = (total + 255) / 256;
    if (g > 4096) g = 4096;
    hipLaunchKernelGGL(pack_weight_kernel, dim3((unsigned)g), dim3(256), 0, as_stream(stream), W, Cout, K, NT, rot, total,
                       packed, (long long)K, 1LL, 0LL);
    return check_launch("pack_weight_kernel");
}

extern "C" int ptt_pack_weight_strided_f32(const float* W, int Cout, int K, int64_t stride_out, int64_t stride_k, int batch,
                                           int64_t stride_batch, float* packed, ptt_stream_t stream) {
    if (Cout <= 0 || K <= 0 || batch < 0) return fail(PTT_EINVAL, "ptt_pack_weight_strided_f32: Cout=%d K=%d batch=%d", Cout, K, batch);
    if (batch == 0) return PTT_OK;
    if (!W || !packed) return fail(PTT_EINVAL, "ptt_pack_weight_strided_f32: null pointer");
    const size_t total = ptt_packed_weight_elems(Cout, K);
    const int NT = (Cout + 31) / 32;
    size_t g = (total + 255) / 256;
    if (g > 1024) g = 1024;
    hipLaunchKernelGGL(pack_weight_kernel, dim3((unsigned)g, (unsigned)batch), dim3(256), 0, as_stream(stream), W, Cout, K, NT, 0,
                       total, packed, (long long)stride_out, (long long)stride_k, (long long)stride_batch);
    return check_launch("pack_weight_kernel");
}

extern "C" int ptt_pack_weights_f32(const ptt_pack_job* jobs_device, int n_jobs, float* arena, ptt_stream_t stream) {
    if (n_jobs < 0) return fail(PTT_EINVAL, "ptt_pack_weights_f32: n_jobs=%d", n_jobs);
    if (n_jobs == 0) return PTT_OK;
    if (!jobs_device || !arena) return fail(PTT_EINVAL, "ptt_pack_weights_f32: null pointer");
    if (n_jobs > 65535) return fail(PTT_EUNSUPPORTED, "ptt_pack_weights_f32: n_jobs=%d exceeds one launch (65535)", n_jobs);
    hipLaunchKernelGGL(pack_weights_kernel, dim3(32, (unsigned)n_jobs), dim3(256), 0, as_stream(stream), jobs_device, arena);
    return check_launch("pack_weights_kernel");
}

extern "C" int ptt_pack_weight_f32(const float* W, int Cout, int K, float* packed, ptt_stream_t stream) {
    return ptt_pack_weight_rot_f32(W, Cout, K, 0, packed, stream);
}

static int linear_launch(const float* X, int rows, int K, int ldx, const float* Wpacked, int Cout, const float* scale,
                         const float* shift, int relu, const float* residual, int ldr, float* out, int ldo, int batch,
                         long long xb, long long wb, long long ob, long long rb, ptt_stream_t stream,
                         const float* in_a = nullptr, const float* in_b = nullptr);

extern "C" int ptt_linear_act_in_f32(const float* X, int rows, int K, int ldx, const float* in_scale, const float* in_shift,
                                     const float* Wpacked, int Cout, float* out, int ldo, ptt_stream_t stream) {
    if (!in_scale || !in_shift || (K & 3) || (ldx & 3) || ((reinterpret_cast<uintptr_t>(X) | reinterpret_cast<uintptr_t>(in_scale) |
                                                             reinterpret_cast<uintptr_t>(in_shift)) & 15))
        return fail(PTT_EINVAL, "ptt_linear_act_in_f32: needs K %% 4 == 0, ldx %% 4 == 0 and 16-byte aligned X / in_scale / in_shift");
    return linear_launch(X, rows, K, ldx, Wpacked, Cout, nullptr, nullptr, 0, nullptr, 0, out, ldo, 1, 0, 0, 0, 0, stream, in_scale,
                         in_shift);
}

extern "C" int ptt_linear_f32(const float* X, int rows, int K, int ldx, const float* Wpacked, int Cout,
                              const float* scale, const float* shift, int relu, const float* residual, int ldr,
                              float* out, int ldo, ptt_stream_t stream) {
    return linear_launch(X, rows, K, ldx, Wpacked, Cout, scale, shift, relu, residual, ldr, out, ldo, 1, 0, 0, 0, 0, stream);
}

extern "C" int ptt_linear_batched_f32(const float* X, int rows, int K, int ldx, int64_t x_batch_stride, const float* Wpacked,
                                      int64_t w_batch_stride, int Cout, const float* scale, const float* shift, int relu,
                                      const float* residual, int ldr, int64_t r_batch_stride, float* out, int ldo,
                                      int64_t o_batch_stride, int batch, ptt_stream_t stream) {
    if (batch < 0 || batch > 65535) return fail(PTT_EINVAL, "ptt_linear_batched_f32: batch=%d", batch);
    if (batch == 0) return PTT_OK;
    return linear_launch(X, rows, K, ldx, Wpacked, Cout, scale, shift, relu, residual, ldr, out, ldo, batch, x_batch_stride,
                         w_batch_stride, o_batch_stride, r_batch_stride, stream);
}

static int linear_launch(const float* X, int rows, int K, int ldx, const float* Wpacked, int Cout, const float* scale,
                         const float* shift, int relu, const float* residual, int ldr, float* out, int ldo, int batch,
                         long long xb, long long wb, long long ob, long long rb, ptt_stream_t stream, const float* in_a,
                         const float* in_b) {
    if (rows < 0 || K <= 0 || Cout <= 0 || ldx < K || ldo < Cout || (residual && ldr < Cout))
        return fail(PTT_EINVAL, "ptt_linear_f32: rows=%d K=%d Cout=%d ldx=%d ldo=%d ldr=%d", rows, K, Cout, ldx, ldo,
                    ldr);
    if (rows == 0) return PTT_OK;
    if (!X || !Wpacked || !out) return fail(PTT_EINVAL, "ptt_linear_f32: null pointer");
    LinearParams p;
    p.X = X; p.Wp = Wpacked; p.scale = scale; p.shift = shift; p.residual = residual; p.out = out;
    p.rows = rows; p.K = K; p.ldx = ldx; p.Cout = Cout; p.relu = relu; p.ldr = ldr; p.ldo = ldo;
    p.nkb = (K + 7) / 8; p.NT = (Cout + 31) / 32;
    p.vec_ok = ((ldx & 3) == 0 && (xb & 3) == 0 && (reinterpret_cast<uintptr_t>(X) & 15) == 0) ? 1 : 0;
    p.xb = xb; p.wb = wb; p.ob = ob; p.rb = rb;
    p.in_a = in_a; p.in_b = in_b;
    const bool vec = p.vec_ok && (K & 3) == 0;
    hipStream_t s = as_stream(stream);
    if (dev_switches().linear_small && vec && batch == 1 && !in_a && rows <= 8192 && K <= 520 && K >= 32) {
        const int hb = ((p.nkb + 1) / 2 + LS_PD - 1) / LS_PD * LS_PD;
        const int lds = (32 * (2 * hb * 8 + 4) + 4 * 16 * 64) * (int)sizeof(float);
        if (int rc = set_lds_limit(reinterpret_cast<const void*>(linear_small_kernel), lds)) return rc;
        hipLaunchKernelGGL(linear_small_kernel, dim3((rows + 31) / 32, (p.NT + 3) / 4), dim3(512), lds, s, p);
        return check_launch("linear_small_kernel");
    }
    const int rt64 = (rows + 63) / 64, rt32 = (rows + 31) / 32, cg256 = (p.NT + 7) / 8, cg128 = (p.NT + 3) / 4;
    int RT = dev_switches().linear_rt, CT = dev_switches().linear_ct;
    if (rows >= 32768 && Cout >= 256 && RT == 1 && CT == 1) CT = 2;
    const int lds = 2 * (RT * 32) * LIN_LDK * (int)sizeof(float);
    const dim3 grid(RT == 2 ? rt64 : rt32, CT == 2 ? cg256 : cg128, batch);
    int rc = PTT_OK;
#define PTT_LIN_CASE(R, V, C)                                                                                  \
    if (RT == R && vec == V && CT == C) {                                                                      \
        if ((rc = set_lds_limit(reinterpret_cast<const void*>(linear_kernel<R, V, C>), lds))) return rc;       \
        hipLaunchKernelGGL((linear_kernel<R, V, C>), grid, dim3(256), lds, s, p);                              \
    }
    PTT_LIN_CASE(1, true, 1) PTT_LIN_CASE(1, true, 2) PTT_LIN_CASE(1, false, 1) PTT_LIN_CASE(1, false, 2)
#ifdef PTT_DEV
    PTT_LIN_CASE(2, true, 1) PTT_LIN_CASE(2, true, 2) PTT_LIN_CASE(2, false, 1) PTT_LIN_CASE(2, false, 2)
#endif
#undef PTT_LIN_CASE
    return check_launch("linear_kernel");
}

extern "C" int ptt_rows_mlp_f32(const float* X, int rows, int K, int ldx, const ptt_sa_layer* layers, int n_layers,
                                const float* residual, int ldr, float* out, int ldo, ptt_stream_t stream) {
    if (rows < 0 || K <= 0 || ldx < K || n_layers < 1 || n_layers > PTT_SA_MAX_LAYERS || !layers)
        return fail(PTT_EINVAL, "ptt_rows_mlp_f32: rows=%d K=%d ldx=%d layers=%d", rows, K, ldx, n_layers);
    if (rows == 0) return PTT_OK;
    if (!X || !out) return fail(PTT_EINVAL, "ptt_rows_mlp_f32: null pointer");
    if (K > 264) return fail(PTT_EUNSUPPORTED, "ptt_rows_mlp_f32: K=%d (at most 264 input channels)", K);
    RowsMlpParams p;
    p.X = X; p.residual = residual; p.out = out; p.rows = rows; p.K0 = K; p.ldx = ldx; p.ldr = ldr; p.ldo = ldo;
    p.n_layers = n_layers;
    int maxk = 0, cin = K;
    for (int l = 0; l < n_layers; ++l) {
        const ptt_sa_layer& s = layers[l];
        const bool last = l == n_layers - 1;
        if (s.Cin != cin) return fail(PTT_EINVAL, "ptt_rows_mlp_f32: layer %d Cin=%d, expected %d", l, s.Cin, cin);
        if (s.Cout <= 0 || s.Cout > (last ? 384 : 256))
            return fail(PTT_EUNSUPPORTED, "ptt_rows_mlp_f32: layer %d Cout=%d (inner layers <= 256, the last <= 384)", l, s.Cout);
        if (!s.Wpacked) return fail(PTT_EINVAL, "ptt_rows_mlp_f32: layer %d has no weights", l);
        SaLayerDev& L = p.L[l];
        L.Wp = s.Wpacked; L.scale = s.scale; L.shift = s.shift; L.Cin = s.Cin; L.Cout = s.Cout; L.relu = s.relu;
        L.nkb = (s.Cin + 7) / 8; L.NT = (s.Cout + 31) / 32;
        if (L.nkb * 8 > maxk) maxk = L.nkb * 8;
        if (!last && L.NT * 32 > maxk) maxk = L.NT * 32;
        cin = s.Cout;
    }
    if (ldo < cin || (residual && ldr < cin)) return fail(PTT_EINVAL, "ptt_rows_mlp_f32: ldo=%d ldr=%d Cout=%d", ldo, ldr, cin);
    p.ldk = maxk + 4;
    p.vec_in = ((K & 3) == 0 && (ldx & 3) == 0 && (reinterpret_cast<uintptr_t>(X) & 15) == 0) ? 1 : 0;
    const int lds = 32 * p.ldk * (int)sizeof(float);
    int rc = set_lds_limit(reinterpret_cast<const void*>(rows_mlp_kernel), lds);
    if (rc) return rc;
    hipLaunchKernelGGL(rows_mlp_kernel, dim3((rows + 31) / 32), dim3(256), lds, as_stream(stream), p);
    return check_launch("rows_mlp_kernel");
}

extern "C" size_t ptt_sa_compact_workspace(int B, int M) {
    const long long T = (long long)(B > 0 ? B : 0) * (M > 0 ? M : 0);
    return SacTable::words((size_t)T) * sizeof(int32_t);
}

extern "C" int ptt_sa_fused_fwd_f32(const ptt_sa_desc* d, ptt_stream_t stream) {
    if (!d) return fail(PTT_EINVAL, "ptt_sa_fused_fwd_f32: null descriptor");
    if (d->B < 0 || d->N <= 0 || d->M < 0 || d->C < 0 || d->n_layers < 1 || d->n_layers > PTT_SA_MAX_LAYERS)
        return fail(PTT_EINVAL, "ptt_sa_fused_fwd_f32: B=%d N=%d M=%d C=%d layers=%d", d->B, d->N, d->M, d->C,
                    d->n_layers);
    if (d->nsample != 16 && d->nsample != 32 && d->nsample != 64)
        return fail(PTT_EUNSUPPORTED, "ptt_sa_fused_fwd_f32: nsample=%d (16, 32 and 64 are instantiated)", d->nsample);
    if (d->B == 0 || d->M == 0) return PTT_OK;
    const bool hoist = d->l0_point_term != nullptr;
    if (!d->xyz || !d->new_xyz || !d->idx || !d->out || (!hoist && d->C > 0 && !d->feat))
        return fail(PTT_EINVAL, "ptt_sa_fused_fwd_f32: null pointer");
    if (!d->use_xyz && d->C == 0) return fail(PTT_EINVAL, "ptt_sa_fused_fwd_f32: no xyz and no features");
    if (hoist) {
        const int c0 = d->l0_channels;
        if (!d->use_xyz || !d->l0_xyz_weight || c0 <= 0 || (c0 % 32) != 0 || c0 > 256 ||
            (reinterpret_cast<uintptr_t>(d->l0_point_term) & 15) != 0 ||
            (reinterpret_cast<uintptr_t>(d->l0_xyz_weight) & 15) != 0)
            return fail(PTT_EINVAL, "ptt_sa_fused_fwd_f32: hoisted layer 0 needs use_xyz, 16-byte aligned (B,N,C0) and "
                        "(3,C0) arrays and C0 a multiple of 32 <= 256 (C0=%d)", c0);
    }

    SaParams p;
    p.xyz = d->xyz; p.new_xyz = d->new_xyz; p.idx = d->idx; p.feat = d->feat; p.out = d->out;
    p.fsb = d->feat_sb; p.fsc = d->feat_sc; p.fsn = d->feat_sn;
    p.osb = d->out_sb; p.osc = d->out_sc; p.osm = d->out_sm;
    p.B = d->B; p.N = d->N; p.M = d->M; p.C = d->C; p.use_xyz = d->use_xyz ? 1 : 0;
    p.normalize = d->normalize_xyz ? 1 : 0; p.n_layers = d->n_layers; p.radius = d->radius;
    p.K0 = (d->use_xyz ? 3 : 0) + d->C;
    p.hoist = hoist ? 1 : 0; p.l0_relu = d->l0_relu ? 1 : 0; p.wx = d->l0_xyz_weight;
    if (hoist && d->l0_channels == 128 && (unsigned long long)d->B * d->N * 128ull * sizeof(float) < 0x7fffffffull &&
        !dev_switches().sa_gather1)
        p.hoist = 2;
    if (hoist) {
        p.feat = d->l0_point_term; p.C = d->l0_channels; p.K0 = p.C;
        p.fsc = 1; p.fsn = p.C; p.fsb = (long long)d->N * p.C;
    }
    int maxk = 0, cin = p.K0;
    for (int l = 0; l < d->n_layers; ++l) {
        const ptt_sa_layer& s = d->layers[l];
        if (s.Cin != cin) return fail(PTT_EINVAL, "ptt_sa_fused_fwd_f32: layer %d Cin=%d, expected %d", l, s.Cin, cin);
        if (s.Cout <= 0 || (s.Cout % 32) != 0 || s.Cout > 256)
            return fail(PTT_EUNSUPPORTED, "ptt_sa_fused_fwd_f32: layer %d Cout=%d must be a multiple of 32 <= 256", l,
                        s.Cout);
        if (!s.Wpacked) return fail(PTT_EINVAL, "ptt_sa_fused_fwd_f32: layer %d has no weights", l);
        SaLayerDev& L = p.L[l];
        L.Wp = s.Wpacked; L.scale = s.scale; L.shift = s.shift; L.Cin = s.Cin; L.Cout = s.Cout; L.relu = s.relu;
        L.nkb = (s.Cin + 7) / 8; L.NT = s.Cout / 32;
        if (L.nkb * 8 > maxk) maxk = L.nkb * 8;
        if (l + 1 < d->n_layers && s.Cout > maxk) maxk = s.Cout;
        cin = s.Cout;
    }
    {
        const unsigned long long lim = 0x7fffffffull, B = (unsigned long long)d->B;
        if (B * d->N * 12ull >= lim || B * d->M * d->nsample * 4ull >= lim || B * d->M * (unsigned long long)cin * 4ull >= lim ||
            B * d->N * (unsigned long long)(p.C > 0 ? p.C : 1) * 4ull >= lim)
            return fail(PTT_EUNSUPPORTED, "ptt_sa_fused_fwd_f32: B=%d N=%d M=%d: an array of this launch exceeds 2 GiB "
                        "(32-bit offsets) — split the batch", d->B, d->N, d->M);
    }
    p.ldk = maxk + 4;
    p.vec_gather = (p.C > 0 && p.fsc == 1 && (p.C & 3) == 0 && p.C <= 256 && (p.fsn & 3) == 0 &&
                    (p.fsb & 3) == 0 && (reinterpret_cast<uintptr_t>(p.feat) & 15) == 0) ? 1 : 0;
    p.first_wave = 1024; p.stagger = dev_switches().sa_stagger;
    p.dbg = dev_switches().stamps;
    p.cws = nullptr;
    const int total_centres = d->B * d->M;
    hipStream_t s = as_stream(stream);
    int rc;
    if (d->C == 0 && d->use_xyz && !hoist && d->nsample == 32 && d->n_layers == 3 && p.L[0].Cout == 64 && p.L[1].Cout == 64 &&
        p.L[2].Cout == 128 && !p.L[0].scale && !p.L[1].scale && !p.L[2].scale && p.L[0].relu && p.L[1].relu &&
        dev_switches().sa_lds) {
        const int waves = 256 * PTT_SAL_WAVES * PTT_SAL_WGS;
        p.chunk = (total_centres + waves - 1) / waves;
        if (dev_switches().sa_lds_chunk > 0 && p.chunk > dev_switches().sa_lds_chunk) p.chunk = dev_switches().sa_lds_chunk;
        const int nw = total_centres * 3 <= 256 * PTT_SAL_WAVES ? 4 : PTT_SAL_WAVES;
        int wgs = (total_centres + p.chunk * nw - 1) / (p.chunk * nw);
        const int lds = (4096 + 8192 + PTT_SAL_WAVES * 640) * (int)sizeof(float);
        if (d->compact_ws) {
            if (d->compact_ws_bytes < ptt_sa_compact_workspace(d->B, d->M) || (reinterpret_cast<uintptr_t>(d->compact_ws) & 15))
                return fail(PTT_EWORKSPACE, "ptt_sa_fused_fwd_f32: compact_ws needs %zu bytes, 16-byte aligned (got %zu)",
                            ptt_sa_compact_workspace(d->B, d->M), d->compact_ws_bytes);
            p.cws = static_cast<int32_t*>(d->compact_ws);
            hipLaunchKernelGGL(sa_compact_zero_kernel, dim3(1), dim3(64), 0, s, p.cws);
            if ((rc = check_launch("sa_compact_zero_kernel"))) return rc;
            hipLaunchKernelGGL(sa_compact_kernel<true>, dim3((total_centres + 31) / 32), dim3(256), 0, s, d->xyz, d->idx, d->N, d->M,
                               SacTable{p.cws, total_centres});
            if ((rc = check_launch("sa_compact_kernel"))) return rc;
            if (wgs > 256 * PTT_SAL_WGS) wgs = 256 * PTT_SAL_WGS;
            if ((rc = set_lds_limit(reinterpret_cast<const void*>(sa_lds_kernel<true>), lds))) return rc;
            hipLaunchKernelGGL(sa_lds_kernel<true>, dim3(wgs), dim3(64 * nw), lds, s, p);
            return check_launch("sa_lds_kernel");
        }
        if ((rc = set_lds_limit(reinterpret_cast<const void*>(sa_lds_kernel<false>), lds))) return rc;
        hipLaunchKernelGGL(sa_lds_kernel<false>, dim3(wgs), dim3(64 * nw), lds, s, p);
        return check_launch("sa_lds_kernel");
    }
    size_t wbytes = 0;
    bool wave_ok = true;
    for (int l = 0; l < d->n_layers; ++l) {
        wbytes += (size_t)d->layers[l].Cin * d->layers[l].Cout * sizeof(float);
        const int nt = d->layers[l].Cout / 32;
        if (!(nt == 1 || nt == 2 || nt == 4)) wave_ok = false;
    }
    wave_ok = wave_ok && dev_switches().sa_wave;
    if (wave_ok && wbytes <= 64 * 1024 && d->nsample <= 32) {
        const int lds = 4 * 32 * p.ldk * (int)sizeof(float);
        const int cpw = 32 / d->nsample, per_wg = 4 * cpw;
        const dim3 grid((total_centres + per_wg - 1) / per_wg);
        if (d->nsample == 32) {
            if ((rc = set_lds_limit(reinterpret_cast<const void*>(sa_wave_kernel<32, 1>), lds))) return rc;
            hipLaunchKernelGGL((sa_wave_kernel<32, 1>), grid, dim3(256), lds, s, p);
        } else {
            if ((rc = set_lds_limit(reinterpret_cast<const void*>(sa_wave_kernel<16, 1>), lds))) return rc;
            hipLaunchKernelGGL((sa_wave_kernel<16, 1>), grid, dim3(256), lds, s, p);
        }
        return check_launch("sa_wave_kernel");
    }
    if (p.hoist == 2 && d->nsample == 32 && d->n_layers == 2 && p.L[0].Cin == 128 && p.L[0].Cout == 128 &&
        p.L[1].Cout == 256 && !p.L[0].scale && !p.L[1].scale && p.L[0].relu && dev_switches().sa_stream) {
        p.tiles = (total_centres + 1) / 2;
        int wgs = p.tiles < 512 ? p.tiles : 512;
        p.chunk = (p.tiles + wgs - 1) / wgs;
        if (dev_switches().sa_chunk > 0 && p.chunk > dev_switches().sa_chunk) p.chunk = dev_switches().sa_chunk;
        wgs = (p.tiles + p.chunk - 1) / p.chunk;
        if (d->compact_ws) {
            if (d->compact_ws_bytes < ptt_sa_compact_workspace(d->B, d->M) || (reinterpret_cast<uintptr_t>(d->compact_ws) & 15))
                return fail(PTT_EWORKSPACE, "ptt_sa_fused_fwd_f32: compact_ws needs %zu bytes, 16-byte aligned (got %zu)",
                            ptt_sa_compact_workspace(d->B, d->M), d->compact_ws_bytes);
            p.cws = static_cast<int32_t*>(d->compact_ws);
            hipLaunchKernelGGL(sa_compact_zero_kernel, dim3(1), dim3(64), 0, s, p.cws);
            if ((rc = check_launch("sa_compact_zero_kernel"))) return rc;
            hipLaunchKernelGGL(sa_compact_kernel<false>, dim3((total_centres + 31) / 32), dim3(256), 0, s, d->xyz, d->idx, d->N, d->M,
                               SacTable{p.cws, total_centres});
            if ((rc = check_launch("sa_compact_kernel"))) return rc;
            const int lds = (2 * SAS_TILE + 64 * 4 + 64) * (int)sizeof(float);
            if ((rc = set_lds_limit(reinterpret_cast<const void*>(sa_stream_compact_kernel), lds))) return rc;
            hipLaunchKernelGGL(sa_stream_compact_kernel, dim3(p.tiles < 512 ? p.tiles : 512), dim3(256), lds, s, p);
            return check_launch("sa_stream_compact_kernel");
        }
        const int lds = (2 * SAS_TILE + 4 * 16 * 4) * (int)sizeof(float);
        if ((rc = set_lds_limit(reinterpret_cast<const void*>(sa_stream_kernel<32>), lds))) return rc;
        hipLaunchKernelGGL((sa_stream_kernel<32>), dim3(wgs), dim3(256), lds, s, p);
        return check_launch("sa_stream_kernel");
    }
    int RT = dev_switches().sa_rt;
    if (d->nsample == 64) RT = 2;
    const int lds = 32 * RT * p.ldk * (int)sizeof(float);
    if (lds > 160 * 1024) return fail(PTT_EUNSUPPORTED, "ptt_sa_fused_fwd_f32: %d B of LDS per workgroup", lds);
    const int cpw = 32 * RT / d->nsample;
    const dim3 grid((total_centres + cpw - 1) / cpw);
#define PTT_SA_CASE(NSV, RTV)                                                                                   \
    if (d->nsample == NSV && RT == RTV) {                                                                       \
        if ((rc = set_lds_limit(reinterpret_cast<const void*>(sa_fused_kernel<NSV, RTV>), lds))) return rc;     \
        hipLaunchKernelGGL((sa_fused_kernel<NSV, RTV>), grid, dim3(256), lds, s, p);                            \
    }
    PTT_SA_CASE(32, 2) PTT_SA_CASE(32, 1) PTT_SA_CASE(16, 2) PTT_SA_CASE(16, 1) PTT_SA_CASE(64, 2)
#undef PTT_SA_CASE
    return check_launch("sa_fused_kernel");
}

extern "C" int ptt_xcorr_fused_fwd_f32(const ptt_xcorr_desc* d, ptt_stream_t stream) {
    if (!d) return fail(PTT_EINVAL, "ptt_xcorr_fused_fwd_f32: null descriptor");
    if (d->B < 0 || d->Ns <= 0 || d->C0 <= 0 || d->n_layers < 1 || d->n_layers > PTT_SA_MAX_LAYERS)
        return fail(PTT_EINVAL, "ptt_xcorr_fused_fwd_f32: B=%d Ns=%d C0=%d layers=%d", d->B, d->Ns, d->C0, d->n_layers);
    if (d->Nt <= 0 || (d->Nt % 64) != 0)
        return fail(PTT_EUNSUPPORTED, "ptt_xcorr_fused_fwd_f32: Nt=%d (the template seeds are walked in chunks of 64)", d->Nt);
    if (d->n_layers < 2) return fail(PTT_EUNSUPPORTED, "ptt_xcorr_fused_fwd_f32: needs at least two MFMA layers after layer 0");
    if ((d->C0 % 8) != 0 || d->C0 > 256) return fail(PTT_EUNSUPPORTED, "ptt_xcorr_fused_fwd_f32: C0=%d", d->C0);
    if (d->B == 0) return PTT_OK;
    if (!d->P || !d->w_sim || !d->out) return fail(PTT_EINVAL, "ptt_xcorr_fused_fwd_f32: null pointer");
    if ((unsigned long long)d->B * d->Ns * d->Nt >= 0x7fffffffull || (unsigned long long)d->B * d->Nt * d->C0 >= 0x7fffffffull)
        return fail(PTT_EUNSUPPORTED, "ptt_xcorr_fused_fwd_f32: B=%d Ns=%d Nt=%d: 32-bit element offsets — split the batch",
                    d->B, d->Ns, d->Nt);
    XcorrParams q;
    q.P = d->P; q.wsim = d->w_sim; q.scale0 = d->scale0;
    q.shift0 = d->shift0; q.sim_out = d->sim_out; q.cos_t = d->cos_t;
    q.C0 = d->C0; q.Nt = d->Nt;
    q.sfeat = q.tfeat = nullptr; q.s_sb = q.s_sn = q.t_sb = q.t_sn = 0; q.C = 0; q.eps = 0.f; q.out_sh = 0;
    SaParams& p = q.sa;
    memset(&p, 0, sizeof(p));
    p.out = d->out; p.osb = d->out_sb; p.osc = d->out_sc; p.osm = d->out_sn;
    p.B = d->B; p.M = d->Ns; p.n_layers = d->n_layers;
    int maxk = d->C0, cin = d->C0;
    for (int l = 0; l < d->n_layers; ++l) {
        const ptt_sa_layer& s = d->layers[l];
        if (s.Cin != cin) return fail(PTT_EINVAL, "ptt_xcorr_fused_fwd_f32: layer %d Cin=%d, expected %d", l, s.Cin, cin);
        if (s.Cout <= 0 || (s.Cout % 32) != 0 || s.Cout > 256)
            return fail(PTT_EUNSUPPORTED, "ptt_xcorr_fused_fwd_f32: layer %d Cout=%d", l, s.Cout);
        if (!s.Wpacked) return fail(PTT_EINVAL, "ptt_xcorr_fused_fwd_f32: layer %d has no weights", l);
        SaLayerDev& L = p.L[l];
        L.Wp = s.Wpacked; L.scale = s.scale; L.shift = s.shift; L.Cin = s.Cin; L.Cout = s.Cout; L.relu = s.relu;
        L.nkb = (s.Cin + 7) / 8; L.NT = s.Cout / 32;
        if (l + 1 < d->n_layers && s.Cout > maxk) maxk = s.Cout;
        cin = s.Cout;
    }
    p.ldk = ((maxk + 7) / 8) * 8 + 4;
    p.first_wave = 1024; p.stagger = 2;
    if (d->split) {
        if (!d->search_feat || !d->templ_feat || d->sim_out || (d->C & 3) || (d->s_sb & 3) || (d->s_sn & 3) ||
            (d->t_sb & 3) || (d->t_sn & 3) || ((reinterpret_cast<uintptr_t>(d->search_feat) | reinterpret_cast<uintptr_t>(d->templ_feat)) & 15) ||
            ((d->B * d->Ns) & 7) || d->C <= 0)
            return fail(PTT_EINVAL, "ptt_xcorr_fused_fwd_f32: the split form needs the features (unit channel stride, C %% 4 == 0, 16-byte "
                                    "aligned rows), B * Ns %% 8 == 0 and no sim_out");
        q.sfeat = d->search_feat; q.tfeat = d->templ_feat; q.s_sb = d->s_sb; q.s_sn = d->s_sn; q.t_sb = d->t_sb; q.t_sn = d->t_sn;
        q.C = d->C; q.eps = d->eps; q.out_sh = d->out_sh;
        const int lds = (32 * p.ldk + 32) * (int)sizeof(float);
        int rc = set_lds_limit(reinterpret_cast<const void*>(xcorr_fused_kernel<1, true>), lds);
        if (rc) return rc;
        hipLaunchKernelGGL((xcorr_fused_kernel<1, true>), dim3(2 * d->B * d->Ns), dim3(256), lds, as_stream(stream), q);
        return check_launch("xcorr_fused_kernel");
    }
    if (!d->cos_t) return fail(PTT_EINVAL, "ptt_xcorr_fused_fwd_f32: null pointer (cos_t comes from ptt_cosine_map_f32)");
    const int lds = (64 * p.ldk + 64) * (int)sizeof(float);
    int rc = set_lds_limit(reinterpret_cast<const void*>(xcorr_fused_kernel<2, false>), lds);
    if (rc) return rc;
    hipLaunchKernelGGL((xcorr_fused_kernel<2, false>), dim3(d->B * d->Ns), dim3(256), lds, as_stream(stream), q);
    return check_launch("xcorr_fused_kernel");
}

extern "C" int ptt_cosine_map_f32(const float* search_feat, int64_t s_sb, int64_t s_sn, int64_t s_sc, const float* templ_feat,
                                  int64_t t_sb, int64_t t_sn, int64_t t_sc, int B, int Ns, int Nt, int C, float eps,
                                  float* cos_t, ptt_stream_t stream) {
    if (B < 0 || Ns <= 0 || Nt <= 0 || C <= 0) return fail(PTT_EINVAL, "ptt_cosine_map_f32: B=%d Ns=%d Nt=%d C=%d", B, Ns, Nt, C);
    if (B == 0) return PTT_OK;
    if (!search_feat || !templ_feat || !cos_t) return fail(PTT_EINVAL, "ptt_cosine_map_f32: null pointer");
    CosParams q;
    q.sfeat = search_feat; q.tfeat = templ_feat; q.cos_t = cos_t;
    q.s_sb = s_sb; q.s_sn = s_sn; q.s_sc = s_sc; q.t_sb = t_sb; q.t_sn = t_sn; q.t_sc = t_sc;
    q.B = B; q.Ns = Ns; q.Nt = Nt; q.C = C; q.eps = eps;
    hipLaunchKernelGGL(cos_map_kernel, dim3((B * Ns + 3) / 4), dim3(256), 0, as_stream(stream), q);
    return check_launch("cos_map_kernel");
}

extern "C" int ptt_pt_attn_pair_f32(const ptt_attn_desc* d, ptt_stream_t stream) {
    if (!d) return fail(PTT_EINVAL, "ptt_pt_attn_pair_f32: null descriptor");
    if (d->B < 0 || d->N <= 0) return fail(PTT_EINVAL, "ptt_pt_attn_pair_f32: B=%d N=%d", d->B, d->N);
    if (d->D != 512 || d->k != 16)
        return fail(PTT_EUNSUPPORTED, "ptt_pt_attn_pair_f32: D=%d k=%d (D=512, k=16 is instantiated)", d->D, d->k);
    if (d->B == 0) return PTT_OK;
    if (!d->xyz || !d->knn || !d->qkv || !d->Wd1p || !d->Wd2p || !d->bd2 || !d->Wg1p || !d->bg1 ||
        !d->Wg2p || !d->res)
        return fail(PTT_EINVAL, "ptt_pt_attn_pair_f32: null pointer");
    AttnParams p;
    p.xyz = d->xyz; p.rel = d->rel; p.knn = d->knn; p.qkv = d->qkv; p.Wd1p = d->Wd1p; p.Wd2p = d->Wd2p; p.bd2 = d->bd2;
    p.Wg1p = d->Wg1p; p.bg1 = d->bg1; p.Wg2p = d->Wg2p; p.bg2 = d->bg2; p.res = d->res; p.attn = d->attn;
    p.order = d->order;
    p.BN = d->B * d->N; p.N = d->N;
    p.first_wave = 512; p.stagger = dev_switches().pair_stagger;
    p.dbg = dev_switches().stamps;
    if ((d->N & 1) != 0)
        return fail(PTT_EUNSUPPORTED, "ptt_pt_attn_pair_f32: N=%d must be even (a tile holds two points of one cloud)",
                    d->N);
    const int heads = d->heads ? d->heads : 1;
    int lds = (32 * (512 + 4) + 32 + 32 * 12) * (int)sizeof(float);
    lds += dev_switches().pair_lds_pad;
    const void* kern;
    switch (heads) {
        case 1: kern = reinterpret_cast<const void*>(pt_attn_pair_kernel<512>); break;
        case 2: kern = reinterpret_cast<const void*>(pt_attn_pair_heads_kernel<2>); break;
        case 4: kern = reinterpret_cast<const void*>(pt_attn_pair_heads_kernel<4>); break;
        case 8: kern = reinterpret_cast<const void*>(pt_attn_pair_heads_kernel<8>); break;
        default: return fail(PTT_EUNSUPPORTED, "ptt_pt_attn_pair_f32: heads=%d (1, 2, 4, 8 are instantiated)", d->heads);
    }
    int rc = set_lds_limit(kern, lds);
    if (rc) return rc;
    const dim3 grid((p.BN + 1) / 2);
    switch (heads) {
        case 1: hipLaunchKernelGGL((pt_attn_pair_kernel<512>), grid, dim3(256), lds, as_stream(stream), p); break;
        case 2: hipLaunchKernelGGL((pt_attn_pair_heads_kernel<2>), grid, dim3(256), lds, as_stream(stream), p); break;
        case 4: hipLaunchKernelGGL((pt_attn_pair_heads_kernel<4>), grid, dim3(256), lds, as_stream(stream), p); break;
        default: hipLaunchKernelGGL((pt_attn_pair_heads_kernel<8>), grid, dim3(256), lds, as_stream(stream), p); break;
    }
    return check_launch(heads == 1 ? "pt_attn_pair_kernel" : "pt_attn_pair_heads_kernel");
}
```

ptt_amd/models/backbones_3d/pointnet2/pointnet2_modules.py:

```python
import os
from typing import List

import torch
import torch.nn as nn
import torch.nn.functional as F

from .... import ops, train_ops
from ....param_cache import (DropsCachesOnModeChange, FoldedLayer, ParamCache, conv_bn_tensors, fold_conv_bn,
                             index_table)
from . import pointnet2_utils
from . import pytorch_utils as pt_utils

STREAM_COMPACT_MIN_BALLS = 2048
STREAM_COMPACT_MAX_POINTS = 1024


class PointnetSAModuleVotes(DropsCachesOnModeChange, nn.Module):
    def __init__(self, *, mlp: List[int], radius: float = None, nsample: int = None, bn: bool = True,
                 use_xyz: bool = True, normalize_xyz: bool = False, sample_uniformly: bool = False,
                 sample_method='fps'):
        super().__init__()
        self.radius = radius
        self.nsample = nsample
        self.mlp_module = None
        self.use_xyz = use_xyz
        self.normalize_xyz = normalize_xyz
        self.sample_uniformly = sample_uniformly
        self.grouper = pointnet2_utils.QueryAndGroup(radius, nsample, use_xyz=use_xyz, ret_grouped_xyz=True,
                                                     normalize_xyz=normalize_xyz, sample_uniformly=sample_uniformly,
                                                     ret_unique_cnt=False)
        mlp_spec = mlp
        if use_xyz and len(mlp_spec) > 0:
            mlp_spec[0] += 3
        self.mlp_module = pt_utils.SharedMLP(mlp_spec, bn=bn)
        self.sample_method = sample_method
        self._fused_cache = ParamCache()
        self.centres_knn_k = 0
        self.centres_knn = None

    def _sample(self, xyz, features, npoint):
        if self.sample_method == 'fps':
            return pointnet2_utils.furthest_point_sample(xyz, npoint)
        if self.sample_method in ('rs', 'sequence'):
            return index_table(xyz.size(0), npoint, xyz.device, torch.int32)
        if self.sample_method == 'ffps':
            if features is None:
                raise ValueError("sample_method 'ffps': a level without point features cannot sample in feature space "
                                 "(use 'fps' for it)")
            return ops.feature_fps(xyz.contiguous(), features.detach(), npoint)
        raise NotImplementedError(self.sample_method)

    def _fusable(self, xyz, features):
        if self.training or not xyz.is_cuda:
            return False
        name = 'PointnetSAModuleVotes(nsample=%s, mlp=%s)' % (self.nsample, [u.conv.weight.shape[0] for u in self.mlp_module
                                                                              if hasattr(u, 'conv')])
        if ops.autograd_recording(self, xyz, features):
            return ops.note_unfused(name, 'autograd is recording (wrap inference in torch.no_grad())')
        if self.sample_uniformly or self.nsample not in (16, 32, 64):
            return ops.note_unfused(name, 'nsample must be 16, 32 or 64 and sample_uniformly off')
        if xyz.dtype != torch.float32 or (features is not None and features.dtype != torch.float32):
            return ops.note_unfused(name, 'inputs must be float32')
        if len(self.mlp_module) > 4:
            return ops.note_unfused(name, 'more than 4 SharedMLP layers')
        for unit in self.mlp_module:
            conv = getattr(unit, 'conv', None)
            if conv is None or conv.kernel_size != (1, 1) or conv.weight.shape[0] % 32 != 0 or conv.weight.shape[0] > 256:
                return ops.note_unfused(name, 'layer widths must be multiples of 32, at most 256, 1x1 convolutions')
            if list(unit._modules.keys())[0] != 'conv':
                return ops.note_unfused(name, 'pre-activation units')
        return True

    def _fused_params(self, device):
        return self._fused_cache.get(conv_bn_tensors(self.mlp_module), device, self._fold)

    def _fold(self):
        layers, scale0 = [], None
        for li, unit in enumerate(self.mlp_module):
            w = unit.conv.weight
            cout, cin = w.shape[0], w.shape[1]
            rot = 3 if (li == 0 and self.use_xyz and cin > 3) else 0
            scale, shift = fold_conv_bn(unit)
            scale0 = scale if li == 0 else scale0
            wq = w if scale is None else w * scale.view(-1, 1, 1, 1)
            layers.append(FoldedLayer(ops.pack_weight(wq, rot), None, shift, cin, cout, hasattr(unit, 'activation')))
        hoist = None
        w0 = self.mlp_module[0].conv.weight
        if (self.use_xyz and len(layers) >= 2 and w0.shape[1] > 3 and layers[0].cout <= 256
                and os.environ.get('PTT_SA_HOIST', '1') != '0'):
            w2 = w0.reshape(w0.shape[0], w0.shape[1]).float()
            wx = w2[:, 0:3] if scale0 is None else w2[:, 0:3] * scale0[:, None]
            wf = w2[:, 3:] if scale0 is None else w2[:, 3:] * scale0[:, None]
            hoist = (ops.pack_weight(wf.contiguous()), wx.t().contiguous(), layers[0].cout, layers[0].relu)
        return layers, hoist

    def forward(self, xyz: torch.Tensor, features: torch.Tensor, npoint: int, inds: torch.Tensor = None, pre=None,
                compact: bool = False):
        self.centres_knn = None
        if self._fusable(xyz, features):
            return self._forward_fused(xyz, features, npoint, inds, pre, compact)
        return self._forward_train(xyz, features, npoint, inds)

    def _forward_fused(self, xyz, features, npoint, inds, pre, compact):
        if (pre is None and inds is None and self.sample_method == 'fps' and xyz.shape[1] <= 256 and npoint <= 128
                and xyz.shape[0] * npoint * self.nsample <= ops.ONE_FRAME_MAX_SA_ROWS and self.centres_knn_k <= npoint):
            xyz = xyz.contiguous()
            inds, inds64, new_xyz, idx, self.centres_knn = ops.fps_ball_knn(xyz, npoint, self.radius, self.nsample, self.centres_knn_k)
            pre = (new_xyz, idx, inds64)
        prefix = inds is None and self.sample_method in ('rs', 'sequence')
        if pre is not None:
            pass
        elif prefix:
            inds64 = index_table(xyz.size(0), npoint, xyz.device, torch.int64)
        elif inds is None:
            inds = self._sample(xyz, features, npoint)
        else:
            assert inds.shape[1] == npoint
            inds = inds.to(torch.int32)

        xyz = xyz.contiguous()
        if pre is not None:
            new_xyz, idx, inds64 = pre
        elif prefix:
            new_xyz, _, idx = ops.centres_ball_query(xyz, None, npoint, self.radius, self.nsample)
        else:
            new_xyz, inds64, idx = ops.centres_ball_query(xyz, inds.contiguous(), npoint, self.radius, self.nsample)
        layers, hoist = self._fused_params(xyz.device)
        if hoist is not None and features is not None:
            wf_packed, wx, c0, relu0 = hoist
            rows = features.transpose(1, 2)
            uniform = rows.stride(2) == 1 and rows.stride(0) == rows.shape[1] * rows.stride(1)
            term = ops.linear(rows if uniform else rows.contiguous(), wf_packed, c0, None, layers[0].shift, relu=False)
            B, M, ns = xyz.shape[0], npoint, self.nsample
            if (B * M * ns <= ops.ONE_FRAME_MAX_SA_ROWS and ns in (16, 32) and len(layers) == 3 and c0 % 4 == 0 and c0 >= 192):
                L1, L2 = layers[1], layers[2]
                h = torch.empty((B * M * ns, L1.cout), dtype=torch.float32, device=xyz.device)
                ops.row_jobs([pt_utils.layer_job(L1, prologue=3, x=term, idx=idx, xyz=xyz, centres=new_xyz, wx=wx,
                                                 radius=self.radius, ns=ns, M=M, N=xyz.shape[1], normalize_xyz=self.normalize_xyz,
                                                 pro_relu=relu0, out=h)])
                pooled = torch.empty((B, M, L2.cout), dtype=torch.float32, device=xyz.device)
                ops.row_jobs([pt_utils.layer_job(L2, x=h, epilogue=2, ns=ns, M=M, out=pooled)])
                return new_xyz, pooled.transpose(1, 2), inds64
            new_features = ops.sa_fused_forward(xyz, new_xyz, idx, None, layers[1:], self.radius, True,
                                                self.normalize_xyz, point_major_out=True, l0=(term, wx, relu0),
                                                compact=(bool(compact) and B * M >= STREAM_COMPACT_MIN_BALLS
                                                         and xyz.shape[1] <= STREAM_COMPACT_MAX_POINTS))
        else:
            new_features = ops.sa_fused_forward(xyz, new_xyz, idx, features, layers, self.radius,
                                                self.use_xyz, self.normalize_xyz, point_major_out=True,
                                                compact=features is None)
        return new_xyz, new_features, inds64

    def _forward_train(self, xyz, features, npoint, inds):
        if inds is None:
            inds = self._sample(xyz, features, npoint)
        else:
            assert inds.shape[1] == npoint
            inds = inds.to(torch.int32)
        hoist = (self.use_xyz and not self.sample_uniformly and self.nsample * npoint <= 16384
                 and train_ops.usable(self.mlp_module, xyz if features is None else features)
                 and self.mlp_module[0].conv.weight.shape[0] % 4 == 0)
        if hoist and not xyz.requires_grad and inds.dtype == torch.int32:
            new_xyz, inds64, idx = ops.centres_ball_query(xyz.contiguous(), inds.contiguous(), npoint, self.radius, self.nsample)
            y = train_ops.sa_level_hoisted(xyz, new_xyz, features, idx, self.mlp_module, self.radius, self.normalize_xyz)
            return new_xyz, y, inds64
        xyz_flipped = xyz.transpose(1, 2).contiguous()
        new_xyz = pointnet2_utils.gather_operation(xyz_flipped, inds).transpose(1, 2).contiguous()
        if hoist and features is not None:
            idx = pointnet2_utils.ball_query(self.radius, self.nsample, xyz, new_xyz)
            y = train_ops.sa_level_hoisted(xyz, new_xyz, features, idx, self.mlp_module, self.radius, self.normalize_xyz)
            return new_xyz, y, inds.to(torch.int64)
        grouped_features, grouped_xyz = self.grouper(xyz, new_xyz, features)
        if train_ops.usable(self.mlp_module, grouped_features):
            return new_xyz, train_ops.shared_mlp_pool(grouped_features, self.mlp_module, pool_dim=3), inds.to(torch.int64)
        y = self.mlp_module(grouped_features)
        y = y.max(dim=3)[0]
        return new_xyz, y, inds.to(torch.int64)
```

ptt_amd/models/backbones_3d/pointnet2_backbone.py:

```python
from typing import List

import torch
import torch.nn as nn

from ... import graph_policy, ops, train_ops
from ...param_cache import ParamCache, index_table
from .pointnet2 import pointnet2_modules


class PointNet2BackboneLight(nn.Module):
    def __init__(self, model_cfg, input_channels, **kwargs):
        super().__init__()
        self.model_cfg = model_cfg
        input_channels -= 3
        self.num_points_each_layer = []
        self.SA_modules = nn.ModuleList()
        sa = self.model_cfg.SA_CONFIG
        for k in range(len(sa.RADIUS)):
            mlps = list(sa.MLPS[k])
            if k == 0:
                mlps[0] = input_channels
            self.SA_modules.append(pointnet2_modules.PointnetSAModuleVotes(
                radius=sa.RADIUS[k], nsample=sa.NSAMPLE[k], mlp=mlps,
                use_xyz=sa.get('USE_XYZ', True), normalize_xyz=sa.get('NORMALIZE_XYZ', True),
                sample_method=sa.SAMPLE_METHOD[k]))
        self.cov_final = nn.Conv1d(256, 256, kernel_size=1)
        self.num_point_features = sa.MLPS[-1][-1]
        self._cov_cache = ParamCache()
        self.seed_knn = 16
        self.overlap_branches = True
        self._side_stream = None

    @staticmethod
    def _break_up_pc(pc):
        xyz = pc[..., 0:3].contiguous()
        features = pc[..., 3:].contiguous() if pc.size(-1) > 3 else None
        return xyz, features

    def _cov_final(self, features):
        if not features.is_cuda:
            return self.cov_final(features)
        if self.training:
            if features.dtype != torch.float32:
                return self.cov_final(features)
            return train_ops.rows_linear(self.cov_final, features.transpose(1, 2)).transpose(1, 2)
        if ops.autograd_recording(self.cov_final, features) or features.dtype != torch.float32:
            ops.note_unfused('PointNet2BackboneLight.cov_final', 'autograd is recording or input is not float32')
            return self.cov_final(features)
        w, b = self.cov_final.weight, self.cov_final.bias
        wpacked, bias = self._cov_cache.get([w, b], w.device, lambda: (ops.pack_weight(w), b.detach().float().contiguous()))
        rows = features.transpose(1, 2)
        out = ops.linear(rows, wpacked, w.shape[0], None, bias)
        return out.transpose(1, 2)

    def branch_forward(self, pts, npoints: List, inds0=None, want_knn=0, compact_levels=()):
        xyz, features = self._break_up_pc(pts)
        sa = self.model_cfg.SA_CONFIG
        one_frame = (not self.training and xyz.is_cuda and features is None and len(self.SA_modules) == 3
                     and xyz.shape[0] * npoints[0] <= 4 * ops.ONE_FRAME_MAX_POINTS
                     and self.SA_modules[0].sample_method == 'fps'
                     and all(m.sample_method in ('rs', 'sequence') for m in self.SA_modules[1:])
                     and npoints[0] >= npoints[1] >= npoints[2] and (not want_knn or npoints[2] <= 128)
                     and all(m._fusable(xyz, None) for m in self.SA_modules[:1]))
        knn = None
        if one_frame:
            from .pointnet2 import pointnet2_utils
            xyz = xyz.contiguous()
            if inds0 is None:
                inds0 = pointnet2_utils.furthest_point_sample(xyz, npoints[0])
            inds0 = inds0.to(torch.int32).contiguous()
            levels, inds64, knn = ops.sa_levels_point_jobs(xyz, inds0, list(npoints), list(sa.RADIUS), list(sa.NSAMPLE),
                                                           knn_k=want_knn)
            seq = [None] + [index_table(xyz.size(0), n, xyz.device, torch.int64) for n in npoints[1:3]]
            xyz, features, inds0 = self.SA_modules[0](xyz=xyz, features=features, npoint=npoints[0], inds=inds0,
                                                      pre=(levels[0][0], levels[0][1], inds64))
            xyz, features, inds1 = self.SA_modules[1](xyz=xyz, features=features, npoint=npoints[1],
                                                      pre=(levels[1][0], levels[1][1], seq[1]))
            xyz, features, inds2 = self.SA_modules[2](xyz=xyz, features=features, npoint=npoints[2],
                                                      pre=(levels[2][0], levels[2][1], seq[2]))
        else:
            xyz, features, inds0 = self.SA_modules[0](xyz=xyz, features=features, npoint=npoints[0], inds=inds0)
            xyz, features, inds1 = self.SA_modules[1](xyz=xyz, features=features, npoint=npoints[1], compact=1 in compact_levels)
            xyz, features, inds2 = self.SA_modules[2](xyz=xyz, features=features, npoint=npoints[2], compact=2 in compact_levels)
        point_features = self._cov_final(features)
        assert inds1.dtype == inds2.dtype == torch.int64, 'index type must be int64, not {}'.format(inds2.dtype)
        if all(m.sample_method in ('rs', 'sequence') for m in self.SA_modules[1:]) and inds0.shape[1] >= npoints[2]:
            inds = inds0[:, :npoints[2]]
        else:
            inds = inds0.gather(1, inds1).gather(1, inds2)
        if want_knn:
            return xyz, point_features, inds, knn
        return xyz, point_features, inds

    def sample(self, search_points, template_points):
        from .pointnet2 import pointnet2_utils
        sa = self.model_cfg.SA_CONFIG
        assert sa.SAMPLE_METHOD[0] == 'fps'
        return (pointnet2_utils.furthest_point_sample(search_points[..., 0:3].contiguous(), sa.NPOINTS_SEARCH[0]),
                pointnet2_utils.furthest_point_sample(template_points[..., 0:3].contiguous(), sa.NPOINTS_TEMPLATE[0]))

    def forward_branches(self, search_points, template_points, inds=None):
        sa = self.model_cfg.SA_CONFIG
        i_s, i_t = inds if inds is not None else (None, None)
        last = (len(self.SA_modules) - 1,) if (search_points.is_cuda and not self.training) else ()
        if not (self.overlap_branches and search_points.is_cuda and not self.training):
            r = self.branch_forward(search_points, sa.NPOINTS_SEARCH, i_s, want_knn=self.seed_knn, compact_levels=last)
            t_seeds, t_feats, t_inds = self.branch_forward(template_points, sa.NPOINTS_TEMPLATE, i_t)
        else:
            if self._side_stream is None or self._side_stream.device != search_points.device:
                self._side_stream = torch.cuda.Stream(device=search_points.device)
            main = torch.cuda.current_stream(search_points.device)
            side = graph_policy.branch(main, self._side_stream)
            with torch.cuda.stream(side):
                t_seeds, t_feats, t_inds = self.branch_forward(template_points, sa.NPOINTS_TEMPLATE, i_t)
            r = self.branch_forward(search_points, sa.NPOINTS_SEARCH, i_s, want_knn=self.seed_knn, compact_levels=last)
            graph_policy.join(main, side)
            if side is not main:
                for t in (t_seeds, t_feats, t_inds, template_points):
                    t.record_stream(main)
        s_seeds, s_feats, s_inds = r[:3]
        s_knn = r[3] if len(r) > 3 else None
        out = {'search_seeds': s_seeds, 'search_feats': s_feats, 'search_inds': s_inds,
               'template_seeds': t_seeds, 'template_feats': t_feats, 'template_inds': t_inds}
        if s_knn is not None:
            out['search_seeds_knn'] = s_knn
        return out

    def forward(self, batch_dict):
        batch_dict.update(self.forward_branches(batch_dict['search_points'], batch_dict['template_points'],
                                                batch_dict.pop('fps_inds', None)))
        batch_dict.pop('search_points')
        batch_dict.pop('template_points')
        return batch_dict
```

ptt_amd/models/trackers/ptt.py:

```python
import torch.nn as nn

from ... import train_ops
from .tracker3d_template import Tracker3DTemplate


class PTT(Tracker3DTemplate):
    def __init__(self, model_cfg, num_class, dataset):
        super().__init__(model_cfg=model_cfg, num_class=num_class, dataset=dataset)
        self.module_list = self.build_networks()

    def forward(self, batch_dict):
        for module in self.module_list:
            batch_dict = module(batch_dict)
        if self.training:
            loss, tb_dict, disp_dict = self.get_training_loss()
            return {'loss': loss.float()}, tb_dict, disp_dict
        return batch_dict

    def _one_launch_losses(self):
        c, b = self.centroid_voting_head, self.box_voting_head
        dc, db = c.forward_ret_dict or {}, b.forward_ret_dict or {}
        if not all(k in dc for k in ('cls_label_points', 'search_inds')) or not all(k in db for k in ('pred_box_data', 'centres')):
            return None
        for head, reduction in ((c, 'mean'), (b, 'none')):
            f, r = head.cls_loss_func, head.reg_loss_func
            if not (type(f) is nn.BCEWithLogitsLoss and f.reduction == reduction and f.weight is None and f.pos_weight is not None
                    and f.pos_weight.numel() == 1 and type(r) is nn.SmoothL1Loss and r.reduction == 'none' and r.beta == 1.0):
                return None
        t = (dc['pred_centroids_cls'], dc['pred_centroids_votes'], db['pred_box_data'], db['centres'], dc['cls_label_points'], dc['reg_label'],
             c.cls_loss_func.pos_weight, b.cls_loss_func.pos_weight)
        if dc['pred_centroids_cls'].dim() != 2 or db['pred_box_data'].shape[-1] != 5 or not train_ops.track_losses_usable(
                *t, search_inds=dc['search_inds'], seeds_shape=dc['pred_centroids_cls'].shape):
            return None
        wc, wb = c.model_cfg.LOSS_CONFIG.LOSS_WEIGHTS, b.model_cfg.LOSS_CONFIG.LOSS_WEIGHTS
        total, vals = train_ops.track_losses(t[0], t[1], t[2], t[3], t[4], dc['search_inds'], t[5], t[6], t[7],
                                             (wc['centroids_cls_weight'], wc['centroids_reg_weight'], wb['boxes_cls_weight'], wb['boxes_reg_weight']))
        tb_dict = {'centroids_cls_loss': vals[1], 'centroids_reg_loss': vals[2], 'boxes_cls_loss': vals[3], 'boxes_reg_loss': vals[4]}
        return total, tb_dict, dict(tb_dict)

    def get_training_loss(self):
        fused = self._one_launch_losses()
        if fused is not None:
            return fused
        disp_dict = {}
        loss_centroids, tb_dict = self.centroid_voting_head.get_loss()
        loss_boxes, tb_dict = self.box_voting_head.get_loss(tb_dict)
        disp_dict.update(tb_dict)
        return loss_centroids + loss_boxes, tb_dict, disp_dict
```

ptt_amd/ops.py:

```python
import contextlib
import ctypes
import os

import torch

from . import _lib
from ._lib import AttnDesc, SaDesc, SaLayer, XcorrDesc


def _stream():
    return ctypes.c_void_p(torch.cuda.current_stream().cuda_stream)


_timing = None


def start_kernel_timing(names):
    global _timing
    _timing = {n: [] for n in names}


def stop_kernel_timing():
    global _timing
    t, _timing = _timing, None
# ... 53 lines not shown

def drop_params():
    global param_generation
    param_generation += 1


class StateWatch(object):

    def __init__(self, module):
        self.tensors = list(module.parameters()) + list(module.buffers())
        self.mark()

    def _key(self):
        return list(map(torch.Tensor.data_ptr, self.tensors)), [t._version for t in self.tensors]

    def mark(self):
        self.generation, self.key = param_generation, self._key()

    def changed(self):
        return param_generation != self.generation or self._key() != self.key


def require_finite(*tensors):
    bad = [k for k, t in enumerate(tensors) if t is not None and t.is_floating_point() and not bool(torch.isfinite(t).all())]
    if bad:
        raise ValueError("non-finite values in tensor(s) %s" % ", ".join("#%d %s" % (k, tuple(tensors[k].shape)) for k in bad))


def _chk(t, name, dtype, ndim=None):
    if not isinstance(t, torch.Tensor):
        raise TypeError("%s must be a torch.Tensor" % name)
    if not t.is_cuda:
        raise RuntimeError("%s must be a device (HIP) tensor — CPU tensors are not supported" % name)
    if t.dtype != dtype:
        raise RuntimeError("%s must be %s, got %s" % (name, dtype, t.dtype))
    if not t.is_contiguous():
        raise RuntimeError("%s must be contiguous" % name)
    if ndim is not None and t.dim() != ndim:
        raise RuntimeError("%s must have %d dimensions, got %s" % (name, ndim, tuple(t.shape)))
    return t


def _ptr(t):
    return ctypes.c_void_p(t.data_ptr()) if t is not None else ctypes.c_void_p(0)


_UNTIMED = contextlib.nullcontext()


def _launch(name, device, *args, timed=None):
    with torch.cuda.device(device), (_timed(timed) if timed else _UNTIMED):
        rc = getattr(_lib.lib(), name)(*args, _stream())
    if rc:
        _lib.check(rc, name)


def _host(name, *args):
    return getattr(_lib.lib(), name)(*args)


def _host_checked(name, *args):
    _lib.check(_host(name, *args), name)


def _workspace(query, device, *dims):
    ws = _ws(_host(query, *dims), device)
    return ws, (_ptr(ws), ws.numel() * 8)


FPS_RESIDENT_MAX_N, FPS_RESIDENT_MAX_NPOINT = 16384, 15360


def furthest_point_sampling(xyz, npoint):
    _chk(xyz, "xyz", torch.float32, 3)
    B, N, _ = xyz.shape
    out = torch.empty((B, int(npoint)), dtype=torch.int32, device=xyz.device)
    if N <= FPS_RESIDENT_MAX_N and int(npoint) <= FPS_RESIDENT_MAX_NPOINT:
        _launch("ptt_fps_f32", xyz.device, _ptr(xyz), B, N, int(npoint), _ptr(out), timed='ptt_fps_f32')
    else:
        ws = torch.empty((B * N,), dtype=torch.float32, device=xyz.device)
        _launch("ptt_fps_ws_f32", xyz.device, _ptr(xyz), B, N, int(npoint), _ptr(out), _ptr(ws), ws.numel(), timed='ptt_fps_f32')
    return out


FFPS_MAX_N, FFPS_MAX_C, FFPS_MAX_NPOINT = 16384, 1024, 15360


def feature_fps(xyz, features, npoint):
    _chk(xyz, "xyz", torch.float32, 3)
    B, N, _ = xyz.shape
    C = 0
    if features is not None:
        if not isinstance(features, torch.Tensor):
            raise TypeError("features must be a torch.Tensor")
        if not features.is_cuda:
            raise RuntimeError("features must be a device (HIP) tensor — CPU tensors are not supported")
        if features.dtype != torch.float32:
            raise RuntimeError("features must be torch.float32, got %s" % features.dtype)
        if features.dim() != 3 or features.shape[0] != B or features.shape[2] != N:
            raise RuntimeError("features must be (B,C,N) = (%d,C,%d), got %s" % (B, N, tuple(features.shape)))
        C = features.shape[1]
    npoint = int(npoint)
    if N > FFPS_MAX_N or C > FFPS_MAX_C or npoint > FFPS_MAX_NPOINT:
        raise ValueError("feature_fps: N=%d, C=%d, npoint=%d exceed the kernel's limits N <= %d, C <= %d, npoint <= %d"
                         % (N, C, npoint, FFPS_MAX_N, FFPS_MAX_C, FFPS_MAX_NPOINT))
    if N < 1 or npoint < 1:
        raise ValueError("feature_fps: N=%d and npoint=%d must be at least 1" % (N, npoint))
    out = torch.empty((B, npoint), dtype=torch.int32, device=xyz.device)
    if B == 0:
        return out
    sb, sc, sn = features.stride() if C else (0, 0, 0)
    if C and (N - 1) * abs(sn) + (C - 1) * abs(sc) > 2 ** 31 - 1:
        raise ValueError("feature_fps: one cloud's features span more than 2^31 - 1 elements (strides %d, %d)" % (sc, sn))
    _launch("ptt_ffps_f32", xyz.device, _ptr(xyz), _ptr(features if C else None), sb, sc, sn, B, N, C, npoint, _ptr(out),
            timed='ptt_ffps_f32')
    return out


def gather_points(features, idx):
    _chk(features, "features", torch.float32, 3)
    _chk(idx, "idx", torch.int32, 2)
    B, C, N = features.shape
    M = idx.shape[1]
    out = torch.empty((B, C, M), dtype=torch.float32, device=features.device)
    _launch("ptt_gather_f32", features.device, _ptr(features), _ptr(idx), B, C, N, M, _ptr(out))
    return out


def scatter_add_det(src, idx, N):
    B, C, E = src.shape
    out = torch.empty((B, C, int(N)), dtype=torch.float32, device=src.device)
    nbytes = _host("ptt_scatter_add_det_workspace", B, int(N), E)
    ws = torch.empty((max(1, (nbytes + 3) // 4),), dtype=torch.int32, device=src.device)
    _launch("ptt_scatter_add_det_f32", src.device, _ptr(src), _ptr(idx), B, C, int(N), E, _ptr(out), _ptr(ws), ws.numel() * 4)
    return out


_ATOMIC_GRADS = os.environ.get("PTT_ATOMIC_GRADS", "0")


def set_atomic_grads(on):
    global _ATOMIC_GRADS
    prev = _ATOMIC_GRADS == "1"
    _ATOMIC_GRADS = "1" if on else "0"
    return prev


def _det_grads(entries, N):
    if int(N) * 16384 > 0xffffffff:
        return False
    return entries <= 16384 and _ATOMIC_GRADS != "1"


def gather_points_grad(grad_out, idx, N):
    _chk(grad_out, "grad_out", torch.float32, 3)
    _chk(idx, "idx", torch.int32, 2)
    B, C, M = grad_out.shape
    if M > 0 and _det_grads(M, N):
        return scatter_add_det(grad_out, idx, N)
    out = torch.empty((B, C, int(N)), dtype=torch.float32, device=grad_out.device)
    _launch("ptt_gather_grad_f32", grad_out.device, _ptr(grad_out), _ptr(idx), B, C, int(N), M, _ptr(out))
    return out


def select_centres(xyz, idx, npoint, want_idx64=True):
    _chk(xyz, "xyz", torch.float32, 3)
    B, N, _ = xyz.shape
    if idx is not None:
        _chk(idx, "idx", torch.int32, 2)
    new_xyz = torch.empty((B, int(npoint), 3), dtype=torch.float32, device=xyz.device)
    idx64 = torch.empty((B, int(npoint)), dtype=torch.int64, device=xyz.device) if (want_idx64 and idx is not None) else None
    _launch("ptt_select_centres_f32", xyz.device, _ptr(xyz), _ptr(idx), B, N, int(npoint), _ptr(new_xyz), _ptr(idx64))
    return new_xyz, idx64


GRID_BALL_QUERY_MIN_POINTS = 4096


def ball_query(new_xyz, xyz, radius, nsample):
    _chk(new_xyz, "new_xyz", torch.float32, 3)
    _chk(xyz, "xyz", torch.float32, 3)
    B, M, _ = new_xyz.shape
    N = xyz.shape[1]
    out = torch.empty((B, M, int(nsample)), dtype=torch.int32, device=xyz.device)
    if GRID_BALL_QUERY_MIN_POINTS <= N <= 131072:
        ws, ws_arg = _workspace("ptt_ball_query_grid_workspace", xyz.device, B, N)
        _launch("ptt_ball_query_grid_f32", xyz.device, _ptr(new_xyz), _ptr(xyz), B, M, N, float(radius), int(nsample), _ptr(out), *ws_arg,
                timed='ptt_ball_query_f32')
    else:
        _launch("ptt_ball_query_f32", xyz.device, _ptr(new_xyz), _ptr(xyz), B, M, N, float(radius), int(nsample), _ptr(out),
                timed='ptt_ball_query_f32')
    return out


def centres_ball_query(xyz, sel, npoint, radius, nsample, want_idx64=True):
    _chk(xyz, "xyz", torch.float32, 3)
    B, N, _ = xyz.shape
    if sel is not None:
        _chk(sel, "sel", torch.int32, 2)
    M = int(npoint)
    new_xyz = torch.empty((B, M, 3), dtype=torch.float32, device=xyz.device)
    idx64 = torch.empty((B, M), dtype=torch.int64, device=xyz.device) if (want_idx64 and sel is not None) else None
    idx = torch.empty((B, M, int(nsample)), dtype=torch.int32, device=xyz.device)
    if GRID_BALL_QUERY_MIN_POINTS <= N <= 131072:
        ws, ws_arg = _workspace("ptt_ball_query_grid_workspace", xyz.device, B, N)
        _launch("ptt_centres_ball_query_grid_f32", xyz.device, _ptr(xyz), _ptr(sel), B, N, M, float(radius), int(nsample), _ptr(new_xyz), _ptr(idx64),
                _ptr(idx), *ws_arg, timed='ptt_ball_query_f32')
    else:
        _launch("ptt_centres_ball_query_f32", xyz.device, _ptr(xyz), _ptr(sel), B, N, M, float(radius), int(nsample), _ptr(new_xyz), _ptr(idx64),
                _ptr(idx), timed='ptt_ball_query_f32')
    return new_xyz, idx64, idx


def group_points(features, idx):
    _chk(features, "features", torch.float32, 3)
    _chk(idx, "idx", torch.int32, 3)
    B, C, N = features.shape
    _, M, ns = idx.shape
    out = torch.empty((B, C, M, ns), dtype=torch.float32, device=features.device)
    _launch("ptt_group_f32", features.device, _ptr(features), _ptr(idx), B, C, N, M, ns, _ptr(out))
    return out


def group_points_grad(grad_out, idx, N):
    _chk(grad_out, "grad_out", torch.float32, 4)
    _chk(idx, "idx", torch.int32, 3)
    B, C, M, ns = grad_out.shape
    if M * ns > 0 and _det_grads(M * ns, N):
        return scatter_add_det(grad_out.view(B, C, M * ns), idx.view(B, M * ns), N)
    out = torch.empty((B, C, int(N)), dtype=torch.float32, device=grad_out.device)
    _launch("ptt_group_grad_f32", grad_out.device, _ptr(grad_out), _ptr(idx), B, C, int(N), M, ns, _ptr(out))
    return out


def _unreached(name):
    def fn(*a, **k):
        raise NotImplementedError("%s is never reached by PTT (SURVEY.md §2.1) and is not provided" % name)
    fn.__name__ = name
    return fn


three_nn = _unreached("three_nn")
three_interpolate = _unreached("three_interpolate")
three_interpolate_grad = _unreached("three_interpolate_grad")
furthest_point_sampling_with_dist = _unreached("furthest_point_sampling_with_dist")


def knn(xyz, k, want_rel=False):
    _chk(xyz, "xyz", torch.float32, 3)
    B, N, _ = xyz.shape
    out = torch.empty((B, N, int(k)), dtype=torch.int32, device=xyz.device)
    rel = torch.empty((B, N, int(k), 3), dtype=torch.float32, device=xyz.device) if want_rel else None
    _launch("ptt_knn_rel_f32", xyz.device, _ptr(xyz), B, N, int(k), _ptr(out), _ptr(rel), timed='ptt_knn_f32')
    return (out, rel) if want_rel else out


def pack_weight(weight, rot=0):
    w = weight.detach()
    w = w.reshape(w.shape[0], -1).contiguous().float()
    _chk(w, "weight", torch.float32, 2)
    Cout, K = w.shape
    n = _host("ptt_packed_weight_elems", Cout, K)
    out = torch.empty((n,), dtype=torch.float32, device=w.device)
    _launch("ptt_pack_weight_rot_f32", w.device, _ptr(w), Cout, K, int(rot), _ptr(out))
    return out


ONE_FRAME_MAX_SA_ROWS = 4096
ROW_JOB_MAX_ROWS = 1024
ONE_FRAME_MAX_POINTS = int(os.environ.get("PTT_PT_PER_LAYER_MAX", "512"))


def linear(x, wpacked, cout, scale=None, shift=None, relu=False, residual=None, out=None):
    if not x.is_cuda or x.dtype != torch.float32:
        raise RuntimeError("x must be a float32 device tensor")
    K = x.shape[-1]
    x2 = x.reshape(-1, K)
    if x2.stride(1) != 1:
        x2 = x2.contiguous()
    rows = x2.shape[0]
    if out is None:
        out = torch.empty(tuple(x.shape[:-1]) + (int(cout),), dtype=torch.float32, device=x.device)
    o2 = out.view(-1, int(cout))
    r2 = None
    if residual is not None:
        r2 = residual.reshape(-1, int(cout))
        if r2.stride(1) != 1:
            r2 = r2.contiguous()
    if (scale is None and (rows > 8192 or (rows >= 6144 and int(cout) == 256)) and x2.data_ptr() % 16 == 0 and o2.is_contiguous()
            and _host("ptt_rows_gemm_supported", rows, K, int(cout), x2.stride(0), int(cout))):
        _launch("ptt_rows_gemm_f32", x.device, _ptr(x2), rows, K, x2.stride(0), None, None, _ptr(wpacked), int(cout), _ptr(shift), 1 if relu else 0,
                _ptr(r2), r2.stride(0) if r2 is not None else int(cout), _ptr(o2), int(cout), None, 0, timed='ptt_linear_f32')
        return out
    if rows <= ROW_JOB_MAX_ROWS and 192 <= K <= 1024 and o2.stride(1) == 1:
        row_jobs([row_job(wpacked, cout, x=x2, scale=scale, shift=shift, act=1 if relu else 0, res=r2, out=o2)])
        return out
    _launch("ptt_linear_f32", x.device, _ptr(x2), rows, K, x2.stride(0) if rows > 1 else K, _ptr(wpacked), int(cout), _ptr(scale), _ptr(shift),
            1 if relu else 0, _ptr(r2), (r2.stride(0) if (r2 is not None and rows > 1) else int(cout)), _ptr(o2),
            o2.stride(0) if rows > 1 else int(cout), timed='ptt_linear_f32')
    return out


def sa_fused_forward(xyz, new_xyz, idx, features, layers, radius, use_xyz=True, normalize_xyz=False,
                     point_major_out=True, l0=None, compact=False):
    _chk(xyz, "xyz", torch.float32, 3)
    _chk(new_xyz, "new_xyz", torch.float32, 3)
    _chk(idx, "idx", torch.int32, 3)
    B, N, _ = xyz.shape
    _, M, ns = idx.shape
    d = SaDesc()
    d.xyz, d.new_xyz, d.idx = xyz.data_ptr(), new_xyz.data_ptr(), idx.data_ptr()
    if features is not None:
        if not features.is_cuda or features.dtype != torch.float32 or features.dim() != 3:
            raise RuntimeError("features must be a (B,C,N) float32 device tensor")
        d.feat = features.data_ptr()
        d.feat_sb, d.feat_sc, d.feat_sn = features.stride()
        d.C = features.shape[1]
    else:
        d.feat, d.C = None, 0
    cout = layers[-1][4]
    if point_major_out:
        store = torch.empty((B, M, cout), dtype=torch.float32, device=xyz.device)
        out = store.transpose(1, 2)
    else:
        out = torch.empty((B, cout, M), dtype=torch.float32, device=xyz.device)
    d.out = out.data_ptr()
    d.out_sb, d.out_sc, d.out_sm = out.stride()
    d.B, d.N, d.M, d.nsample = B, N, M, ns
    d.radius, d.use_xyz, d.normalize_xyz = float(radius), int(bool(use_xyz)), int(bool(normalize_xyz))
    d.n_layers = len(layers)
    for i, (wp, sc, sh, cin, co, relu) in enumerate(layers):
        L = d.layers[i]
        L.Wpacked = wp.data_ptr()
        L.scale = sc.data_ptr() if sc is not None else None
        L.shift = sh.data_ptr() if sh is not None else None
        L.Cin, L.Cout, L.relu = int(cin), int(co), int(bool(relu))
    if l0 is not None:
        term, wx, l0_relu = l0
        if features is not None:
            raise RuntimeError("with a hoisted layer 0 the point features are already inside l0[0]")
        _chk(term, "l0 point term", torch.float32, 3)
        _chk(wx, "l0 xyz weight", torch.float32, 2)
        if term.shape[0] != B or term.shape[1] != N or wx.shape[0] != 3 or wx.shape[1] != term.shape[2]:
            raise RuntimeError("l0 point term must be (B,N,C0) and the xyz weight (3,C0)")
        d.l0_point_term, d.l0_xyz_weight = term.data_ptr(), wx.data_ptr()
        d.l0_channels, d.l0_relu = term.shape[2], int(bool(l0_relu))
    if isinstance(compact, torch.Tensor):
        if not compact.is_cuda or compact.device != xyz.device or not compact.is_contiguous():
            raise RuntimeError("compact workspace must be a contiguous tensor on %s" % xyz.device)
        d.compact_ws, d.compact_ws_bytes = compact.data_ptr(), compact.numel() * compact.element_size()
    elif compact:
        ws, (_, d.compact_ws_bytes) = _workspace("ptt_sa_compact_workspace", xyz.device, B, M)
        d.compact_ws = ws.data_ptr()
    _launch("ptt_sa_fused_fwd_f32", xyz.device, ctypes.byref(d), timed='ptt_sa_fused_fwd_f32')
    return out


def cosine_map(search_feats, templ_feats, eps=1e-8):
    for t_, n_ in ((search_feats, "search_feats"), (templ_feats, "templ_feats")):
        if not isinstance(t_, torch.Tensor) or not t_.is_cuda or t_.dtype != torch.float32 or t_.dim() != 3:
            raise RuntimeError("%s must be a (B,C,N) float32 device tensor" % n_)
    if search_feats.shape[:2] != templ_feats.shape[:2] or search_feats.device != templ_feats.device:
        raise RuntimeError("search_feats and templ_feats must share batch size, channel count and device")
    B, C, Ns = search_feats.shape
    Nt = templ_feats.shape[2]
    out = torch.empty((B, Ns, Nt), dtype=torch.float32, device=search_feats.device)
    ssb, ssc, ssn = search_feats.stride()
    tsb, tsc, tsn = templ_feats.stride()
    _launch("ptt_cosine_map_f32", out.device, search_feats.data_ptr(), ssb, ssn, ssc, templ_feats.data_ptr(), tsb, tsn, tsc, B, Ns, Nt, C, float(eps),
            out.data_ptr(), timed='ptt_cosine_map_f32')
    return out


def rows_mlp(x, layers, residual=None):
    if not x.is_cuda or x.dtype != torch.float32 or x.stride(-1) != 1:
        raise RuntimeError("rows_mlp: x must be a float32 device tensor with contiguous rows")
    K = x.shape[-1]
    x2 = x.reshape(-1, K)
    rows = x2.shape[0]
    cout = int(layers[-1][4])
    out = torch.empty((rows, cout), dtype=torch.float32, device=x.device)
    res2 = None
    if residual is not None:
        res2 = residual.reshape(-1, cout)
        _chk(res2 if res2.is_contiguous() else res2.contiguous(), "residual", torch.float32, 2)
        res2 = res2 if res2.stride(1) == 1 else res2.contiguous()
    arr = (SaLayer * len(layers))()
    for i, (wp, sc, sh, cin, co, relu) in enumerate(layers):
        arr[i].Wpacked = wp.data_ptr()
        arr[i].scale = sc.data_ptr() if sc is not None else None
        arr[i].shift = sh.data_ptr() if sh is not None else None
        arr[i].Cin, arr[i].Cout, arr[i].relu = int(cin), int(co), int(bool(relu))
    _launch("ptt_rows_mlp_f32", x.device, _ptr(x2), rows, K, x2.stride(0), arr, len(layers), _ptr(res2), res2.stride(0) if res2 is not None else 0,
            _ptr(out), cout, timed='ptt_rows_mlp_f32')
    return out.view(*x.shape[:-1], cout)


def xcorr_fused(search_feats, templ_feats, P, w_sim, scale0, shift0, layers, eps=1e-8, want_sim=False, cos_t=None, split=False):
    for t_, n_ in ((search_feats, "search_feats"), (templ_feats, "templ_feats")):
        if not t_.is_cuda or t_.dtype != torch.float32 or t_.dim() != 3:
            raise RuntimeError("%s must be a (B,C,N) float32 device tensor" % n_)
    _chk(P, "P", torch.float32, 3)
    _chk(w_sim, "w_sim", torch.float32, 1)
    B, C, Ns = search_feats.shape
    Nt = templ_feats.shape[2]
    C0 = P.shape[2]
    if Nt <= 0 or Nt % 64:
        raise RuntimeError("xcorr_fused: Nt=%d (ptt_xcorr_fused_fwd_f32 walks the template seeds in chunks of 64)" % Nt)
    if P.shape[0] != B or P.shape[1] != Nt or w_sim.shape[0] != C0 or templ_feats.shape[:2] != search_feats.shape[:2]:
        raise RuntimeError("xcorr_fused: inconsistent shapes")
    cout = layers[-1][4]
    split = (split and not want_sim and search_feats.stride(1) == 1 and templ_feats.stride(1) == 1 and C % 4 == 0 and (B * Ns) % 8 == 0
             and all(st % 4 == 0 for st in (search_feats.stride(0), search_feats.stride(2), templ_feats.stride(0), templ_feats.stride(2)))
             and search_feats.data_ptr() % 16 == 0 and templ_feats.data_ptr() % 16 == 0 and bool(layers[-1][5]))
    if not split:
        if cos_t is None:
            cos_t = cosine_map(search_feats, templ_feats, eps=eps)
        _chk(cos_t, "cos_t", torch.float32, 3)
        if tuple(cos_t.shape) != (B, Ns, Nt):
            raise RuntimeError("xcorr_fused: cos_t must be (B,Ns,Nt)")
    store = torch.empty(((2, B, Ns, cout) if split else (B, Ns, cout)), dtype=torch.float32, device=P.device)
    out = store.transpose(-1, -2)
    sim = torch.empty((B, Nt, Ns), dtype=torch.float32, device=P.device) if want_sim else None
    d = XcorrDesc()
    if split:
        d.split, d.out_sh = 1, store.stride(0)
        d.search_feat, d.templ_feat = search_feats.data_ptr(), templ_feats.data_ptr()
        d.s_sb, d.s_sn, d.t_sb, d.t_sn = search_feats.stride(0), search_feats.stride(2), templ_feats.stride(0), templ_feats.stride(2)
        d.C, d.eps = int(C), float(eps)
    else:
        d.cos_t = cos_t.data_ptr()
    d.P, d.w_sim = P.data_ptr(), w_sim.data_ptr()
    d.scale0 = scale0.data_ptr() if scale0 is not None else None
    d.shift0 = shift0.data_ptr() if shift0 is not None else None
    d.out = out.data_ptr()
    d.out_sb, d.out_sc, d.out_sn = out.stride()[-3:]
    d.sim_out = sim.data_ptr() if sim is not None else None
    d.B, d.Ns, d.Nt, d.C0 = B, Ns, Nt, C0
    d.n_layers = len(layers)
    for i, (wp, sc, sh, cin, co, relu) in enumerate(layers):
        L = d.layers[i]
        L.Wpacked = wp.data_ptr()
        L.scale = sc.data_ptr() if sc is not None else None
        L.shift = sh.data_ptr() if sh is not None else None
        L.Cin, L.Cout, L.relu = int(cin), int(co), int(bool(relu))
    _launch("ptt_xcorr_fused_fwd_f32", P.device, ctypes.byref(d), timed='ptt_xcorr_fused_fwd_f32')
    return out, sim


def pack_delta0(weight, bias):
    return pack_weight(torch.cat([weight.detach().float().reshape(weight.shape[0], 3),
                                  bias.detach().float().reshape(-1, 1)], dim=1).contiguous())


def spatial_order(xyz):
    _chk(xyz, "xyz", torch.float32, 3)
    B, N, _ = xyz.shape
    order = torch.empty((B, N), dtype=torch.int32, device=xyz.device)
    _launch("ptt_spatial_order_f32", xyz.device, _ptr(xyz), B, N, _ptr(order))
    return order


def pt_attn_pair(xyz, knn_idx, qkv, wd1p, wd2p, bd2, wg1p, bg1, wg2p, bg2, d_model, want_attn=True, rel=None, order=None,
                 heads=1):
    _chk(xyz, "xyz", torch.float32, 3)
    _chk(knn_idx, "knn_idx", torch.int32, 3)
    _chk(qkv, "qkv", torch.float32, 3)
    B, N, _ = xyz.shape
    k = knn_idx.shape[2]
    D = int(d_model)
    res = torch.empty((B, N, D), dtype=torch.float32, device=xyz.device)
    ashape = (B, N, k, D) if heads == 1 else (B * heads, N, k, D // heads)
    attn = torch.empty(ashape, dtype=torch.float32, device=xyz.device) if want_attn else None
    d = AttnDesc()
    d.xyz, d.knn, d.qkv = xyz.data_ptr(), knn_idx.data_ptr(), qkv.data_ptr()
    d.rel = rel.data_ptr() if rel is not None else None
    d.Wd1p, d.Wd2p, d.bd2 = wd1p.data_ptr(), wd2p.data_ptr(), bd2.data_ptr()
    d.Wg1p, d.bg1, d.Wg2p, d.bg2 = wg1p.data_ptr(), bg1.data_ptr(), wg2p.data_ptr(), bg2.data_ptr()
    d.res = res.data_ptr()
    d.attn = attn.data_ptr() if attn is not None else None
    d.B, d.N, d.k, d.D, d.heads = B, N, k, D, int(heads)
    if order is not None:
        _chk(order, "order", torch.int32, 2)
        if tuple(order.shape) != (B, N):
            raise ValueError("order: (B,N) int32 expected")
        d.order = order.data_ptr()
    _launch("ptt_pt_attn_pair_f32", xyz.device, ctypes.byref(d), timed='ptt_pt_attn_pair_f32')
    return res, attn


def layernorm(x, weight, bias, eps, residual=None, out=None):
    if not x.is_cuda or x.dtype != torch.float32:
        raise RuntimeError("x must be a float32 device tensor")
    C = x.shape[-1]
    x2 = x.reshape(-1, C)
    if x2.stride(1) != 1:
        x2 = x2.contiguous()
    if out is None:
        out = torch.empty(x.shape, dtype=torch.float32, device=x.device)
    o2 = out.view(-1, C)
    r2 = None
    if residual is not None:
        r2 = residual.reshape(-1, C)
        if r2.stride(1) != 1:
            r2 = r2.contiguous()
    rows = x2.shape[0]
    _launch("ptt_layernorm_f32", x.device, _ptr(x2), rows, C, x2.stride(0) if rows > 1 else C, _ptr(weight), _ptr(bias), float(eps), _ptr(r2),
            (r2.stride(0) if (r2 is not None and rows > 1) else C), _ptr(o2), o2.stride(0) if rows > 1 else C, timed='ptt_layernorm_f32')
    return out


import numpy as np

CROP_JOB, REGULARIZE_JOB, TRACK_BOX = np.dtype(_lib.CropJob), np.dtype(_lib.RegularizeJob), np.dtype(_lib.TrackBox)


def track_crop_bounds(boxes, offset, scale, extra2, jobs, job_stride=1):
    ex = None if extra2 is None else np.ascontiguousarray(extra2, np.float64)
    _host_checked("ptt_track_crop_bounds", boxes.ctypes.data, len(boxes), float(offset), float(scale), ex.ctypes.data if ex is not None else None,
                  jobs.ctypes.data, int(job_stride))


def track_box_by_offset(boxes, offsets, use_z, active=None, rng_pos=None):
    assert offsets.dtype == np.float32 and offsets.flags['C_CONTIGUOUS'] and offsets.shape[1] >= 4
    _host_checked("ptt_track_box_by_offset", boxes.ctypes.data, len(boxes), offsets.ctypes.data, offsets.shape[1], int(bool(use_z)),
                  active.ctypes.data if active is not None else None, rng_pos.ctypes.data if rng_pos is not None else None)


def track_select_update(proposals, info, boxes, use_z, active, rng_pos, est_out):
    B = len(boxes)
    P = proposals.shape[1] if proposals.ndim == 3 else 1
    assert proposals.dtype == np.float32 and proposals.flags['C_CONTIGUOUS'] and info.dtype == np.int32 and info.flags['C_CONTIGUOUS']
    assert est_out.dtype == np.float32 and est_out.shape == (B, 5) and est_out.flags['C_CONTIGUOUS'] and rng_pos.dtype == np.int64
    _host_checked("ptt_track_select_update", proposals.ctypes.data, P, info.ctypes.data, boxes.ctypes.data, B, int(bool(use_z)),
                  active.ctypes.data if active is not None else None, rng_pos.ctypes.data, est_out.ctypes.data)


_mt_tables = {}


def mt19937_draws(device, n=8192, seed=1):
    key = (str(device), int(n), int(seed))
    if key not in _mt_tables:
        host = np.empty(int(n), np.uint32)
        _host_checked("ptt_mt19937_fill", int(seed), host.ctypes.data, int(n))
        _mt_tables[key] = torch.from_numpy(host.view(np.int32)).to(device)
        publish_params(torch.device(device), replaced=False)
    return _mt_tables[key]


def upload_jobs(jobs, out=None):
    host = torch.from_numpy(np.ascontiguousarray(jobs).view(np.uint8).reshape(-1)).pin_memory()
    if out is None:
        return host.to('cuda', non_blocking=True)
    out.copy_(host, non_blocking=True)
    return out


def crop_compact(jobs_dev, n_jobs):
    _launch("ptt_crop_compact_f32", jobs_dev.device, _ptr(jobs_dev), int(n_jobs), timed='ptt_crop_compact_f32')


CROP_JOBS_BY_VALUE_MAX = _lib.PTT_CROP_JOBS_BY_VALUE_MAX


def crop_compact_host(jobs_np, n_jobs, device):
    _launch("ptt_crop_compact_host_f32", device, ctypes.c_void_p(jobs_np.ctypes.data), int(n_jobs), timed='ptt_crop_compact_f32')


def crop_compact_pinned(jobs_pinned, n_jobs, device):
    _launch("ptt_crop_compact_f32", device, ctypes.c_void_p(jobs_pinned.data_ptr()), int(n_jobs), timed='ptt_crop_compact_f32')


SCAN_CROP_CHUNK = _lib.DEFINES["PTT_SCAN_CROP_CHUNK"]


def crop_scan_check(jobs_np, n_jobs, max_points):
    jobs = jobs_np[:int(n_jobs)]
    if len(jobs) != int(n_jobs) or int(max_points) < 0:
        raise ValueError("crop_scan: the table holds %d jobs, n_jobs=%d, max_points=%d" % (len(jobs_np), n_jobs, max_points))
    if np.any(jobs['label_out'] != 0):
        raise ValueError("crop_scan: label_out is not supported (training crops take ptt_crop_compact_f32)")
    if np.any(jobs['append'] != 0):
        raise ValueError("crop_scan: append jobs are not supported (SHAPE_AGGREGATION = all takes ptt_crop_compact_f32)")
    if len(jobs) and (int(jobs['n_points'].max()) > int(max_points) or int(jobs['n_points'].min()) < 0):
        raise ValueError("crop_scan: n_points must lie in 0..max_points=%d, got %d..%d" % (max_points, jobs['n_points'].min(), jobs['n_points'].max()))


def crop_scan_workspace(n_jobs, max_points):
    return int(_host("ptt_crop_scan_workspace", int(n_jobs), int(max_points)))


def crop_scan_device(jobs_dev, n_jobs, max_points, ws=None):
    if ws is None:
        ws = _ws(crop_scan_workspace(n_jobs, max_points), jobs_dev.device)
    _launch("ptt_crop_scan_f32", jobs_dev.device, _ptr(jobs_dev), int(n_jobs), int(max_points), _ptr(ws), ws.numel() * ws.element_size(),
            timed='ptt_crop_scan_f32')


def crop_scan(jobs_np, n_jobs, max_points, device, out=None):
    crop_scan_check(jobs_np, n_jobs, max_points)
    with torch.cuda.device(device):
        jobs_dev = upload_jobs(jobs_np, out)
    crop_scan_device(jobs_dev, n_jobs, max_points)
    return jobs_dev


def crop_regularize_pinned(crop_jobs_pinned, reg_jobs_dev, n_jobs, draws):
    _launch("ptt_crop_regularize_f32", reg_jobs_dev.device, ctypes.c_void_p(crop_jobs_pinned.data_ptr()), _ptr(reg_jobs_dev), int(n_jobs),
            _ptr(draws), draws.numel(), timed='ptt_crop_compact_f32')


def regularize(jobs_dev, n_jobs, draws):
    _launch("ptt_regularize_f32", jobs_dev.device, _ptr(jobs_dev), int(n_jobs), _ptr(draws), draws.numel(), timed='ptt_regularize_f32')


def select_box(pred_box_data, out=None, idx_out=None):
    _chk(pred_box_data, "pred_box_data", torch.float32, 3)
    B, P, five = pred_box_data.shape
    if five != 5:
        raise RuntimeError("pred_box_data must be (B,P,5)")
    if out is None:
        out = torch.empty((B, 5), dtype=torch.float32, device=pred_box_data.device)
    _launch("ptt_select_box_f32", pred_box_data.device, _ptr(pred_box_data), B, P, _ptr(out), _ptr(idx_out))
    return out


REF_COORDS = {"camera": _lib.DEFINES["PTT_REF_CAMERA"], "lidar": _lib.DEFINES["PTT_REF_LIDAR"]}


def box_overlap(gt, pred, ref_coord, dims=3, out=None):
    _chk(gt, "gt", torch.float64, 2)
    _chk(pred, "pred", torch.float64, 2)
    n = gt.shape[0]
    if gt.shape[1] != 10 or tuple(pred.shape) != (n, 10) or pred.device != gt.device:
        raise RuntimeError("gt and pred must be (n,10) on one device, got %s and %s" % (tuple(gt.shape), tuple(pred.shape)))
    if isinstance(ref_coord, str):
        if ref_coord.lower() not in REF_COORDS:
            raise ValueError("ref_coord must be 'camera' or 'lidar', got %r" % (ref_coord,))
        ref_coord = REF_COORDS[ref_coord.lower()]
    if out is None:
        out = torch.empty((2, n), dtype=torch.float64, device=gt.device)
    elif _chk(out, "out", torch.float64, 2).shape != (2, n) or out.device != gt.device:
        raise RuntimeError("out must be (2,%d) on the boxes' device, got %s" % (n, tuple(out.shape)))
    _launch("ptt_box_overlap_f64", gt.device, _ptr(gt), _ptr(pred), n, int(ref_coord), int(dims), _ptr(out[0]), _ptr(out[1]))
    return out[0], out[1]


TRAIN_CAND, TRAIN_BATCH_DESC = np.dtype(_lib.TrainCand), np.dtype(_lib.TrainBatchDesc)
TRAIN_MAX_CANDS = _lib.PTT_TRAIN_MAX_CANDS


def train_batch(cands_dev, desc, device):
    _launch("ptt_train_batch_f32", device, _ptr(cands_dev), ctypes.c_void_p(desc.ctypes.data), timed='ptt_train_batch_f32')


# ... 1074 lines not shown
```

Before: 17370.

## Add 1- and 2-row distinct-neighbour classes to SA compact path and enable everywhere

```diff
diff --git a/include/ptt_hip.h b/include/ptt_hip.h
--- a/include/ptt_hip.h
+++ b/include/ptt_hip.h
@@ -8,7 +8,7 @@
 extern "C" {
 #endif
 
-#define PTT_ABI_VERSION 30
+#define PTT_ABI_VERSION 31
 
 enum {
     PTT_OK = 0,
@@ -141,6 +141,7 @@
     int l0_relu;
     void* compact_ws;
     size_t compact_ws_bytes;
+    int compact_min_class;
 } ptt_sa_desc;
 
 int ptt_sa_fused_fwd_f32(const ptt_sa_desc* d, ptt_stream_t stream);
diff --git a/ptt_amd/_lib.py b/ptt_amd/_lib.py
--- a/ptt_amd/_lib.py
+++ b/ptt_amd/_lib.py
@@ -173,7 +173,7 @@
                 ("radius", c_float), ("use_xyz", c_int), ("normalize_xyz", c_int), ("n_layers", c_int),
                 ("layers", SaLayer * PTT_SA_MAX_LAYERS),
                 ("l0_point_term", c_void_p), ("l0_xyz_weight", c_void_p), ("l0_channels", c_int), ("l0_relu", c_int),
-                ("compact_ws", c_void_p), ("compact_ws_bytes", c_size_t)]
+                ("compact_ws", c_void_p), ("compact_ws_bytes", c_size_t), ("compact_min_class", c_int)]
 
 
 class XcorrDesc(Structure):
diff --git a/ptt_amd/csrc/mfma_ops.hip b/ptt_amd/csrc/mfma_ops.hip
--- a/ptt_amd/csrc/mfma_ops.hip
+++ b/ptt_amd/csrc/mfma_ops.hip
@@ -1276,27 +1276,39 @@
 }
 
 constexpr int SAC_HDR = 16;
+template <bool C1> struct SacClasses {
+    static constexpr int N = C1 ? 6 : 4;
+    static constexpr int LG0 = C1 ? 0 : 2;
+};
 struct SacTable {
     int32_t* ws; int T;
     __host__ __device__ int32_t* ndist() const { return ws + SAC_HDR; }
     __host__ __device__ int32_t* list(int k) const { return ws + SAC_HDR + (size_t)(1 + k) * T; }
-    __host__ __device__ int32_t* rows(int k) const { return ws + SAC_HDR + 5 * (size_t)T + (size_t)((4 << k) - 4) * T; }
-    static size_t words(size_t T) { return SAC_HDR + 65 * T; }
+    template <bool C1 = false>
+    __host__ __device__ int32_t* rows(int k) const {
+        if constexpr (C1) return ws + SAC_HDR + 7 * (size_t)T + (size_t)((1 << k) - 1) * T;
+        else return ws + SAC_HDR + 5 * (size_t)T + (size_t)((4 << k) - 4) * T;
+    }
+    static size_t words(size_t T) { return SAC_HDR + 70 * T; }
 };
 constexpr int SAC_PASSES = 4;
 
 __global__ __launch_bounds__(64) void sa_compact_zero_kernel(int32_t* ws) {
     if (threadIdx.x < 4) ws[threadIdx.x] = 0;
 }
-
-template <bool XYZ>
+__global__ __launch_bounds__(64) void sa_compact_zero6_kernel(int32_t* ws) {
+    if (threadIdx.x < 6) ws[threadIdx.x] = 0;
+}
+
+template <bool XYZ, bool C1 = false>
 __global__ __launch_bounds__(256) void sa_compact_kernel(const float* __restrict__ xyz, const int32_t* __restrict__ idx, int N, int M,
                                                          SacTable tab) {
-    __shared__ int s_cnt[4], s_base[4], s_cls[32], s_pos[32], s_nd[32];
+    constexpr int NC = SacClasses<C1>::N, LG0 = SacClasses<C1>::LG0;
+    __shared__ int s_cnt[NC], s_base[NC], s_cls[32], s_pos[32], s_nd[32];
     __shared__ int s_row[32][32];
     const int t = threadIdx.x, lane = t & 63, half = lane >> 5, s = lane & 31, w = t >> 6;
     const int g0 = blockIdx.x * 32, T = tab.T;
-    if (t < 4) s_cnt[t] = 0;
+    if (t < NC) s_cnt[t] = 0;
     __syncthreads();
     int iv[SAC_PASSES];
     uint32_t x[SAC_PASSES], y[SAC_PASSES], z[SAC_PASSES];
@@ -1333,7 +1345,8 @@
         const int nd = __popc(m);
         if (keep) s_row[lc][__popc(m & ((1u << s) - 1u))] = iv[q];
         if (s == 0) {
-            const int k = nd <= 4 ? 0 : nd <= 8 ? 1 : nd <= 16 ? 2 : 3;
+            int k = nd <= 4 ? 0 : nd <= 8 ? 1 : nd <= 16 ? 2 : 3;
+            if constexpr (C1) k = nd <= 1 ? 0 : nd <= 2 ? 1 : k + 2;
             const bool valid = g0 + lc < T;
             s_cls[lc] = valid ? k : -1;
             s_nd[lc] = nd;
@@ -1342,13 +1355,13 @@
         }
     }
     __syncthreads();
-    if (t < 4) s_base[t] = s_cnt[t] ? atomicAdd(&tab.ws[t], s_cnt[t]) : 0;
+    if (t < NC) s_base[t] = s_cnt[t] ? atomicAdd(&tab.ws[t], s_cnt[t]) : 0;
     __syncthreads();
     for (int e = t; e < 32 * 32; e += 256) {
         const int lc = e >> 5, j = e & 31, k = s_cls[lc];
-        if (k < 0 || j >= (4 << k)) continue;
+        if (k < 0 || j >= ((1 << LG0) << k)) continue;
         const int q = s_base[k] + s_pos[lc];
-        tab.rows(k)[(size_t)q * (4 << k) + j] = s_row[lc][j < s_nd[lc] ? j : 0];
+        tab.rows<C1>(k)[(size_t)q * ((1 << LG0) << k) + j] = s_row[lc][j < s_nd[lc] ? j : 0];
         if (j == 0) tab.list(k)[q] = g0 + lc;
     }
 }
@@ -1360,36 +1373,66 @@
 #define PTT_SAL_WAVES 12
 #endif
 
-template <int ROWS>
+template <int ROWS, bool C1 = false>
 struct SacTileT {
-    static constexpr int LG = ROWS == 32 ? 3 : 4;
+    static constexpr int NC = SacClasses<C1>::N, LG0 = SacClasses<C1>::LG0;
+    static constexpr int LG = (ROWS == 32 ? 5 : 6) - LG0;
     static_assert(ROWS == 32 || ROWS == 64, "32- or 64-row tiles");
     int k, first, n;
-    __device__ __forceinline__ static void count(const int32_t* ws, int total, int (&cnt)[4], int (&tiles)[4]) {
-#pragma unroll
-        for (int k = 0; k < 4; ++k) {
+    __device__ __forceinline__ static void count(const int32_t* ws, int total, int (&cnt)[NC], int (&tiles)[NC]) {
+#pragma unroll
+        for (int k = 0; k < NC; ++k) {
             cnt[k] = min(max(ws[k], 0), total);
             tiles[k] = (k ? tiles[k - 1] : 0) + ((cnt[k] + ((1 << LG) >> k) - 1) >> (LG - k));
         }
     }
-    __device__ __forceinline__ void at(int j, const int (&tiles)[4], const int (&cnt)[4]) {
-        k = j < tiles[0] ? 0 : j < tiles[1] ? 1 : j < tiles[2] ? 2 : 3;
-        const int j0 = k == 0 ? 0 : k == 1 ? tiles[0] : k == 2 ? tiles[1] : tiles[2];
-        const int nk = k == 0 ? cnt[0] : k == 1 ? cnt[1] : k == 2 ? cnt[2] : cnt[3];
+    __device__ __forceinline__ void at(int j, const int (&tiles)[NC], const int (&cnt)[NC]) {
+        int j0, nk;
+        if constexpr (C1) {
+            k = j < tiles[0] ? 0 : j < tiles[1] ? 1 : j < tiles[2] ? 2 : j < tiles[3] ? 3 : j < tiles[4] ? 4 : 5;
+            j0 = k == 0 ? 0 : k == 1 ? tiles[0] : k == 2 ? tiles[1] : k == 3 ? tiles[2] : k == 4 ? tiles[3] : tiles[4];
+            nk = k == 0 ? cnt[0] : k == 1 ? cnt[1] : k == 2 ? cnt[2] : k == 3 ? cnt[3] : k == 4 ? cnt[4] : cnt[5];
+        } else {
+            k = j < tiles[0] ? 0 : j < tiles[1] ? 1 : j < tiles[2] ? 2 : 3;
+            j0 = k == 0 ? 0 : k == 1 ? tiles[0] : k == 2 ? tiles[1] : tiles[2];
+            nk = k == 0 ? cnt[0] : k == 1 ? cnt[1] : k == 2 ? cnt[2] : cnt[3];
+        }
         first = (j - j0) << (LG - k);
         n = min((1 << LG) >> k, nk - first);
     }
     __device__ __forceinline__ void row(const SacTable& tab, int s, int& n_out, int& ball) const {
-        const int cl = s >> (2 + k), inb = cl < n;
-        n_out = tab.rows(k)[(size_t)first * (4 << k) + (inb ? s : (s & ((4 << k) - 1)))];
+        const int cl = s >> (LG0 + k), inb = cl < n;
+        n_out = tab.rows<C1>(k)[(size_t)first * ((1 << LG0) << k) + (inb ? s : (s & (((1 << LG0) << k) - 1)))];
         ball = tab.list(k)[first + (inb ? cl : 0)];
     }
 };
-using SacTile = SacTileT<32>;
 
 template <int NU>
-__device__ __forceinline__ void sac_store(int k, int n, int ball, int M, const f32x16 (&acc)[NU], const float (&sh)[NU],
+__device__ __forceinline__ void sac_store_small(int k, int n, int ball, int M, const f32x16 (&acc)[NU], const float (&sh)[NU],
+                                                float* const (&o)[NU], int relu, int half, int osb, int osm) {
+    const int b = ball / M;
+    const int off = b * osb + (ball - b * M) * osm;
+#pragma unroll
+    for (int r = 0; r < 16; ++r) {
+        if (k == 1 && (r & 1)) continue;
+        const int oa = __builtin_amdgcn_readlane(off, tile_row(r, 0)), ob = __builtin_amdgcn_readlane(off, tile_row(r, 1));
+        const int g = tile_row(r, half) >> k;
+#pragma unroll
+        for (int u = 0; u < NU; ++u) {
+            float v = (k == 1 ? fmaxf(acc[u][r], acc[u][r | 1]) : acc[u][r]) + sh[u];
+            if (relu) v = fmaxf(v, 0.f);
+            if (g < n) o[u][half ? ob : oa] = v;
+        }
+    }
+}
+
+template <int NU, bool C1 = false>
+__device__ __forceinline__ void sac_store(int kc, int n, int ball, int M, const f32x16 (&acc)[NU], const float (&sh)[NU],
                                           float* const (&o)[NU], int relu, int half, int osb, int osm) {
+    if constexpr (C1) {
+        if (kc < 2) { sac_store_small<NU>(kc, n, ball, M, acc, sh, o, relu, half, osb, osm); return; }
+    }
+    const int k = C1 ? kc - 2 : kc;
     int ob[8];
 #pragma unroll
     for (int g = 0; g < 8; ++g) {
@@ -1437,9 +1480,11 @@
     }
 }
 
-template <bool COMPACT>
+template <bool COMPACT, bool C1 = false>
 __global__ __launch_bounds__(64 * PTT_SAL_WAVES) __attribute__((amdgpu_waves_per_eu(PTT_SAL_WAVES * PTT_SAL_WGS / 4)))
 void sa_lds_kernel(SaParams p) {
+    using SacTile = SacTileT<32, C1>;
+    constexpr int NC = SacTile::NC;
     extern __shared__ __attribute__((aligned(16))) float smem[];
     float* W1 = smem;
     float* W2 = smem + 4096;
@@ -1448,10 +1493,10 @@
     const int total = p.B * p.M, M = p.M, N = p.N;
     const int nw = (int)blockDim.x >> 6;
     SacTable tab{p.cws, total};
-    int cnt[4], tiles[4];
+    int cnt[NC], tiles[NC];
     if constexpr (COMPACT) {
         SacTile::count(p.cws, total, cnt, tiles);
-        if (logical_block() >= tiles[3]) return;
+        if (logical_block() >= tiles[NC - 1]) return;
     }
     {
         const f32x4* g1 = reinterpret_cast<const f32x4*>(p.L[1].Wp);
@@ -1477,7 +1522,7 @@
     __syncthreads();
     int c0, c1, cstep;
     if constexpr (COMPACT) {
-        c0 = logical_block() + (int)gridDim.x * w; c1 = tiles[3]; cstep = (int)gridDim.x * nw;
+        c0 = logical_block() + (int)gridDim.x * w; c1 = tiles[NC - 1]; cstep = (int)gridDim.x * nw;
     } else {
         const int gw = logical_block() * nw + w;
         c0 = gw * p.chunk; c1 = min(total, c0 + p.chunk); cstep = 1;
@@ -1596,7 +1641,7 @@
             if constexpr (COMPACT) {
                 const float sh2[4] = {cst[6 * 64], cst[7 * 64], cst[8 * 64], cst[9 * 64]};
                 float* const o[4] = {p.out + col * osc, p.out + (32 + col) * osc, p.out + (64 + col) * osc, p.out + (96 + col) * osc};
-                sac_store<4>(tc.k, tc.n, g_cur, M, acc, sh2, o, p.L[2].relu, half, osb, osm);
+                sac_store<4, C1>(tc.k, tc.n, g_cur, M, acc, sh2, o, p.L[2].relu, half, osb, osm);
             } else {
                 float* o = p.out + (ce.b * osb + ce.m * osm);
 #pragma unroll
@@ -1610,7 +1655,10 @@
     }
 }
 
+template <bool C1 = false>
 __global__ __launch_bounds__(256, 2) void sa_stream_compact_kernel(SaParams p) {
+    using Tile = SacTileT<64, C1>;
+    constexpr int NC = Tile::NC;
     extern __shared__ __attribute__((aligned(16))) float smem[];
     float* const P = smem;
     float* const Q = smem + SAS_TILE;
@@ -1620,9 +1668,9 @@
     const int w = __builtin_amdgcn_readfirstlane(t >> 6);
     const int total = p.B * p.M, M = p.M, N = p.N;
     const SacTable tab{p.cws, total};
-    int cnt[4], tiles[4];
-    SacTileT<64>::count(p.cws, total, cnt, tiles);
-    if ((int)blockIdx.x >= tiles[3]) return;
+    int cnt[NC], tiles[NC];
+    Tile::count(p.cws, total, cnt, tiles);
+    if ((int)blockIdx.x >= tiles[NC - 1]) return;
     const SaLayerDev& L1 = p.L[0];
     const SaLayerDev& L2 = p.L[1];
     const __amdgpu_buffer_rsrc_t rf = weight_rsrc(p.feat);
@@ -1643,8 +1691,8 @@
     const int osb = (int)p.osb, osm = (int)p.osm;
     float* const o[2] = {p.out + (w * 32 + col) * (int)p.osc, p.out + ((w + 4) * 32 + col) * (int)p.osc};
 
-    for (int j = blockIdx.x; j < tiles[3]; j += (int)gridDim.x) {
-        SacTileT<64> tc;
+    for (int j = blockIdx.x; j < tiles[NC - 1]; j += (int)gridDim.x) {
+        Tile tc;
         tc.at(j, tiles, cnt);
         if (t < 64) {
             int n, ball;
@@ -1697,9 +1745,9 @@
             }
 #pragma unroll
             for (int rt = 0; rt < 2; ++rt) {
-                const int n = tc.n - rt * (8 >> tc.k);
+                const int n = tc.n - rt * ((C1 ? 32 : 8) >> tc.k);
                 if (n <= 0) continue;
-                sac_store<2>(tc.k, n, ballr[rt], M, acc[rt], sh2, o, L2.relu, half, osb, osm);
+                sac_store<2, C1>(tc.k, n, ballr[rt], M, acc[rt], sh2, o, L2.relu, half, osb, osm);
             }
         }
     }
@@ -2114,6 +2162,9 @@
     p.first_wave = 1024; p.stagger = dev_switches().sa_stagger;
     p.dbg = dev_switches().stamps;
     p.cws = nullptr;
+    if (d->compact_min_class != 0 && d->compact_min_class != 1 && d->compact_min_class != 4)
+        return fail(PTT_EINVAL, "ptt_sa_fused_fwd_f32: compact_min_class=%d (0 or 4: classes from 4 rows, 1: from 1 row)", d->compact_min_class);
+    const bool c1 = d->compact_min_class == 1;
     const int total_centres = d->B * d->M;
     hipStream_t s = as_stream(stream);
     int rc;
@@ -2131,12 +2182,22 @@
                 return fail(PTT_EWORKSPACE, "ptt_sa_fused_fwd_f32: compact_ws needs %zu bytes, 16-byte aligned (got %zu)",
                             ptt_sa_compact_workspace(d->B, d->M), d->compact_ws_bytes);
             p.cws = static_cast<int32_t*>(d->compact_ws);
+            if (wgs > 256 * PTT_SAL_WGS) wgs = 256 * PTT_SAL_WGS;
+            if (c1) {
+                hipLaunchKernelGGL(sa_compact_zero6_kernel, dim3(1), dim3(64), 0, s, p.cws);
+                if ((rc = check_launch("sa_compact_zero6_kernel"))) return rc;
+                hipLaunchKernelGGL((sa_compact_kernel<true, true>), dim3((total_centres + 31) / 32), dim3(256), 0, s, d->xyz, d->idx,
+                                   d->N, d->M, SacTable{p.cws, total_centres});
+                if ((rc = check_launch("sa_compact_kernel"))) return rc;
+                if ((rc = set_lds_limit(reinterpret_cast<const void*>(sa_lds_kernel<true, true>), lds))) return rc;
+                hipLaunchKernelGGL((sa_lds_kernel<true, true>), dim3(wgs), dim3(64 * nw), lds, s, p);
+                return check_launch("sa_lds_kernel");
+            }
             hipLaunchKernelGGL(sa_compact_zero_kernel, dim3(1), dim3(64), 0, s, p.cws);
             if ((rc = check_launch("sa_compact_zero_kernel"))) return rc;
             hipLaunchKernelGGL(sa_compact_kernel<true>, dim3((total_centres + 31) / 32), dim3(256), 0, s, d->xyz, d->idx, d->N, d->M,
                                SacTable{p.cws, total_centres});
             if ((rc = check_launch("sa_compact_kernel"))) return rc;
-            if (wgs > 256 * PTT_SAL_WGS) wgs = 256 * PTT_SAL_WGS;
             if ((rc = set_lds_limit(reinterpret_cast<const void*>(sa_lds_kernel<true>), lds))) return rc;
             hipLaunchKernelGGL(sa_lds_kernel<true>, dim3(wgs), dim3(64 * nw), lds, s, p);
             return check_launch("sa_lds_kernel");
@@ -2178,14 +2239,24 @@
                 return fail(PTT_EWORKSPACE, "ptt_sa_fused_fwd_f32: compact_ws needs %zu bytes, 16-byte aligned (got %zu)",
                             ptt_sa_compact_workspace(d->B, d->M), d->compact_ws_bytes);
             p.cws = static_cast<int32_t*>(d->compact_ws);
+            const int lds = (2 * SAS_TILE + 64 * 4 + 64) * (int)sizeof(float);
+            if (c1) {
+                hipLaunchKernelGGL(sa_compact_zero6_kernel, dim3(1), dim3(64), 0, s, p.cws);
+                if ((rc = check_launch("sa_compact_zero6_kernel"))) return rc;
+                hipLaunchKernelGGL((sa_compact_kernel<false, true>), dim3((total_centres + 31) / 32), dim3(256), 0, s, d->xyz, d->idx,
+                                   d->N, d->M, SacTable{p.cws, total_centres});
+                if ((rc = check_launch("sa_compact_kernel"))) return rc;
+                if ((rc = set_lds_limit(reinterpret_cast<const void*>(sa_stream_compact_kernel<true>), lds))) return rc;
+                hipLaunchKernelGGL(sa_stream_compact_kernel<true>, dim3(p.tiles < 512 ? p.tiles : 512), dim3(256), lds, s, p);
+                return check_launch("sa_stream_compact_kernel");
+            }
             hipLaunchKernelGGL(sa_compact_zero_kernel, dim3(1), dim3(64), 0, s, p.cws);
             if ((rc = check_launch("sa_compact_zero_kernel"))) return rc;
             hipLaunchKernelGGL(sa_compact_kernel<false>, dim3((total_centres + 31) / 32), dim3(256), 0, s, d->xyz, d->idx, d->N, d->M,
                                SacTable{p.cws, total_centres});
             if ((rc = check_launch("sa_compact_kernel"))) return rc;
-            const int lds = (2 * SAS_TILE + 64 * 4 + 64) * (int)sizeof(float);
-            if ((rc = set_lds_limit(reinterpret_cast<const void*>(sa_stream_compact_kernel), lds))) return rc;
-            hipLaunchKernelGGL(sa_stream_compact_kernel, dim3(p.tiles < 512 ? p.tiles : 512), dim3(256), lds, s, p);
+            if ((rc = set_lds_limit(reinterpret_cast<const void*>(sa_stream_compact_kernel<false>), lds))) return rc;
+            hipLaunchKernelGGL(sa_stream_compact_kernel<false>, dim3(p.tiles < 512 ? p.tiles : 512), dim3(256), lds, s, p);
             return check_launch("sa_stream_compact_kernel");
         }
         const int lds = (2 * SAS_TILE + 4 * 16 * 4) * (int)sizeof(float);
diff --git a/ptt_amd/models/backbones_3d/pointnet2/pointnet2_modules.py b/ptt_amd/models/backbones_3d/pointnet2/pointnet2_modules.py
--- a/ptt_amd/models/backbones_3d/pointnet2/pointnet2_modules.py
+++ b/ptt_amd/models/backbones_3d/pointnet2/pointnet2_modules.py
@@ -95,13 +95,13 @@
         return layers, hoist
 
     def forward(self, xyz: torch.Tensor, features: torch.Tensor, npoint: int, inds: torch.Tensor = None, pre=None,
-                compact: bool = False):
+                compact: bool = False, compact_min_class: int = 0):
         self.centres_knn = None
         if self._fusable(xyz, features):
-            return self._forward_fused(xyz, features, npoint, inds, pre, compact)
+            return self._forward_fused(xyz, features, npoint, inds, pre, compact, compact_min_class)
         return self._forward_train(xyz, features, npoint, inds)
 
-    def _forward_fused(self, xyz, features, npoint, inds, pre, compact):
+    def _forward_fused(self, xyz, features, npoint, inds, pre, compact, compact_min_class=0):
         if (pre is None and inds is None and self.sample_method == 'fps' and xyz.shape[1] <= 256 and npoint <= 128
                 and xyz.shape[0] * npoint * self.nsample <= ops.ONE_FRAME_MAX_SA_ROWS and self.centres_knn_k <= npoint):
             xyz = xyz.contiguous()
@@ -126,6 +126,9 @@
         else:
             new_xyz, inds64, idx = ops.centres_ball_query(xyz, inds.contiguous(), npoint, self.radius, self.nsample)
         layers, hoist = self._fused_params(xyz.device)
+        many = xyz.shape[0] * npoint >= STREAM_COMPACT_MIN_BALLS
+        large = many and xyz.shape[1] <= STREAM_COMPACT_MAX_POINTS
+        classes = {'compact_min_class': int(compact_min_class)} if (compact_min_class and many) else {}
         if hoist is not None and features is not None:
             wf_packed, wx, c0, relu0 = hoist
             rows = features.transpose(1, 2)
@@ -143,12 +146,11 @@
                 return new_xyz, pooled.transpose(1, 2), inds64
             new_features = ops.sa_fused_forward(xyz, new_xyz, idx, None, layers[1:], self.radius, True,
                                                 self.normalize_xyz, point_major_out=True, l0=(term, wx, relu0),
-                                                compact=(bool(compact) and B * M >= STREAM_COMPACT_MIN_BALLS
-                                                         and xyz.shape[1] <= STREAM_COMPACT_MAX_POINTS))
+                                                compact=bool(compact) and large, **(classes if (compact and large) else {}))
         else:
             new_features = ops.sa_fused_forward(xyz, new_xyz, idx, features, layers, self.radius,
                                                 self.use_xyz, self.normalize_xyz, point_major_out=True,
-                                                compact=features is None)
+                                                compact=features is None, **(classes if features is None else {}))
         return new_xyz, new_features, inds64
 
     def _forward_train(self, xyz, features, npoint, inds):
diff --git a/ptt_amd/models/backbones_3d/pointnet2_backbone.py b/ptt_amd/models/backbones_3d/pointnet2_backbone.py
--- a/ptt_amd/models/backbones_3d/pointnet2_backbone.py
+++ b/ptt_amd/models/backbones_3d/pointnet2_backbone.py
@@ -29,6 +29,7 @@
         self._cov_cache = ParamCache()
         self.seed_knn = 16
         self.overlap_branches = True
+        self.compact_policy = 'last_search'
         self._side_stream = None
 
     @staticmethod
@@ -53,7 +54,7 @@
         out = ops.linear(rows, wpacked, w.shape[0], None, bias)
         return out.transpose(1, 2)
 
-    def branch_forward(self, pts, npoints: List, inds0=None, want_knn=0, compact_levels=()):
+    def branch_forward(self, pts, npoints: List, inds0=None, want_knn=0, compact_levels=(), compact_min_class=0):
         xyz, features = self._break_up_pc(pts)
         sa = self.model_cfg.SA_CONFIG
         one_frame = (not self.training and xyz.is_cuda and features is None and len(self.SA_modules) == 3
@@ -79,9 +80,12 @@
             xyz, features, inds2 = self.SA_modules[2](xyz=xyz, features=features, npoint=npoints[2],
                                                       pre=(levels[2][0], levels[2][1], seq[2]))
         else:
-            xyz, features, inds0 = self.SA_modules[0](xyz=xyz, features=features, npoint=npoints[0], inds=inds0)
-            xyz, features, inds1 = self.SA_modules[1](xyz=xyz, features=features, npoint=npoints[1], compact=1 in compact_levels)
-            xyz, features, inds2 = self.SA_modules[2](xyz=xyz, features=features, npoint=npoints[2], compact=2 in compact_levels)
+            mc = compact_min_class
+            xyz, features, inds0 = self.SA_modules[0](xyz=xyz, features=features, npoint=npoints[0], inds=inds0, compact_min_class=mc)
+            xyz, features, inds1 = self.SA_modules[1](xyz=xyz, features=features, npoint=npoints[1], compact=1 in compact_levels,
+                                                      compact_min_class=mc)
+            xyz, features, inds2 = self.SA_modules[2](xyz=xyz, features=features, npoint=npoints[2], compact=2 in compact_levels,
+                                                      compact_min_class=mc)
         point_features = self._cov_final(features)
         assert inds1.dtype == inds2.dtype == torch.int64, 'index type must be int64, not {}'.format(inds2.dtype)
         if all(m.sample_method in ('rs', 'sequence') for m in self.SA_modules[1:]) and inds0.shape[1] >= npoints[2]:
@@ -102,18 +106,24 @@
     def forward_branches(self, search_points, template_points, inds=None):
         sa = self.model_cfg.SA_CONFIG
         i_s, i_t = inds if inds is not None else (None, None)
-        last = (len(self.SA_modules) - 1,) if (search_points.is_cuda and not self.training) else ()
+        if self.compact_policy not in ('last_search', 'all'):
+            raise ValueError("compact_policy must be 'last_search' or 'all', not %r" % (self.compact_policy,))
+        fused = search_points.is_cuda and not self.training
+        last = (len(self.SA_modules) - 1,) if fused else ()
+        every = dict(compact_levels=(1, 2), compact_min_class=1) if (fused and self.compact_policy == 'all') else None
+        search_kw = every or dict(compact_levels=last)
+        templ_kw = every or {}
         if not (self.overlap_branches and search_points.is_cuda and not self.training):
-            r = self.branch_forward(search_points, sa.NPOINTS_SEARCH, i_s, want_knn=self.seed_knn, compact_levels=last)
-            t_seeds, t_feats, t_inds = self.branch_forward(template_points, sa.NPOINTS_TEMPLATE, i_t)
+            r = self.branch_forward(search_points, sa.NPOINTS_SEARCH, i_s, want_knn=self.seed_knn, **search_kw)
+            t_seeds, t_feats, t_inds = self.branch_forward(template_points, sa.NPOINTS_TEMPLATE, i_t, **templ_kw)
         else:
             if self._side_stream is None or self._side_stream.device != search_points.device:
                 self._side_stream = torch.cuda.Stream(device=search_points.device)
             main = torch.cuda.current_stream(search_points.device)
             side = graph_policy.branch(main, self._side_stream)
             with torch.cuda.stream(side):
-                t_seeds, t_feats, t_inds = self.branch_forward(template_points, sa.NPOINTS_TEMPLATE, i_t)
-            r = self.branch_forward(search_points, sa.NPOINTS_SEARCH, i_s, want_knn=self.seed_knn, compact_levels=last)
+                t_seeds, t_feats, t_inds = self.branch_forward(template_points, sa.NPOINTS_TEMPLATE, i_t, **templ_kw)
+            r = self.branch_forward(search_points, sa.NPOINTS_SEARCH, i_s, want_knn=self.seed_knn, **search_kw)
             graph_policy.join(main, side)
             if side is not main:
                 for t in (t_seeds, t_feats, t_inds, template_points):
diff --git a/ptt_amd/models/trackers/ptt.py b/ptt_amd/models/trackers/ptt.py
--- a/ptt_amd/models/trackers/ptt.py
+++ b/ptt_amd/models/trackers/ptt.py
@@ -8,6 +8,8 @@
     def __init__(self, model_cfg, num_class, dataset):
         super().__init__(model_cfg=model_cfg, num_class=num_class, dataset=dataset)
         self.module_list = self.build_networks()
+        if hasattr(getattr(self, 'backbone_3d', None), 'compact_policy'):
+            self.backbone_3d.compact_policy = 'all'
 
     def forward(self, batch_dict):
         for module in self.module_list:
diff --git a/ptt_amd/ops.py b/ptt_amd/ops.py
--- a/ptt_amd/ops.py
+++ b/ptt_amd/ops.py
@@ -379,7 +379,7 @@
 
 
 def sa_fused_forward(xyz, new_xyz, idx, features, layers, radius, use_xyz=True, normalize_xyz=False,
-                     point_major_out=True, l0=None, compact=False):
+                     point_major_out=True, l0=None, compact=False, compact_min_class=0):
     _chk(xyz, "xyz", torch.float32, 3)
     _chk(new_xyz, "new_xyz", torch.float32, 3)
     _chk(idx, "idx", torch.int32, 3)
@@ -429,6 +429,7 @@
     elif compact:
         ws, (_, d.compact_ws_bytes) = _workspace("ptt_sa_compact_workspace", xyz.device, B, M)
         d.compact_ws = ws.data_ptr()
+    d.compact_min_class = int(compact_min_class)
     _launch("ptt_sa_fused_fwd_f32", xyz.device, ctypes.byref(d), timed='ptt_sa_fused_fwd_f32')
     return out
 
```

After: 17380, median of 3. No clear change (+0.1%).
